# weiguangzhao/PBNet

Hardware: AMD Instinct MI355X
Metric: scenes/sec fwd+cluster (ScanNet ~150k pts/scene) (higher is better)
Workload: dtype bf16

## Files before the change

### include/pbnet_hip.h

```cpp
#ifndef PBNET_HIP_H
#define PBNET_HIP_H

#include <stddef.h>
#include <stdint.h>

#ifdef __cplusplus
extern "C" {
#endif

typedef void* pbn_stream_t;

enum {
    PBN_OK = 0,
    PBN_ERR_ARG = -1,
    PBN_ERR_WORKSPACE = -2,
    PBN_ERR_HIP = -3,
    PBN_ERR_RANGE = -4,
    PBN_ERR_UNSUPPORTED = -5
};

enum { PBN_F32 = 0, PBN_BF16 = 1, PBN_F16 = 2 };

#define PBN_MAX_SCENES 8

const char* pbn_version(void);
int pbn_last_hip_error(void);

size_t pbn_cluster_workspace_bytes(int n_points, int n_segments, int general_sem);

int pbn_binary_cluster(const float* off_xyz, const float* org_xyz, const int32_t* sem, const int32_t* seg_len,
                       int n_points, int n_segments, float radius, int min_pts, float para_f, int nv_flag,
                       int general_sem , int32_t* cluster_id, int32_t* cluster_num, int32_t* den, float* centers,
                       int32_t* clt_sem, int32_t* n_clusters, int32_t* member_start, int32_t* member_idx,
                       void* workspace, size_t workspace_bytes, pbn_stream_t stream);

int pbn_get_iou(const int32_t* proposals_idx, const int32_t* proposals_offset, const int64_t* instance_labels,
                const int32_t* instance_pointnum, float* proposals_iou, int n_instance, int n_proposal,
                pbn_stream_t stream);

int pbn_cal_iou_and_masklabel(const int32_t* proposals_idx, const int32_t* proposals_offset,
                              const int64_t* instance_labels, const int32_t* instance_pointnum,
                              float* proposals_iou, int n_instance, int n_proposal,
                              const float* mask_scores_sigmoid, float* mask_label, int mode, pbn_stream_t stream);


int pbn_hash_capacity(int n);
size_t pbn_coords_workspace_bytes(int n_max);

int pbn_coords_unique(const int32_t* coords, const int32_t* n_dev, int n_max, uint64_t* table_keys, int32_t* table_vals,
                      int capacity, int32_t* unique_index, int32_t* inverse, int32_t* unique_coords, int32_t* n_unique,
                      void* workspace, size_t workspace_bytes, pbn_stream_t stream);

int pbn_coords_stride(const int32_t* fine_coords, const int32_t* n_fine_dev, int n_fine_max, int stride_out,
                      uint64_t* table_keys, int32_t* table_vals, int capacity, int32_t* coarse_coords,
                      int32_t* parent_row, int32_t* child_k, int32_t* nbr_down, int32_t* n_coarse, void* workspace,
                      size_t workspace_bytes, pbn_stream_t stream);

int pbn_kernel_map(const int32_t* out_coords, const int32_t* n_out_dev, int n_out_max, const int32_t* offsets,
                   int n_offsets, const uint64_t* table_keys, const int32_t* table_vals, int capacity, int32_t* nbr,
                   pbn_stream_t stream);

int pbn_kernel_map_cube(const int32_t* out_coords, const int32_t* n_out_dev, int n_out_max, int kernel_size,
                        int tensor_stride, int x_fastest, const uint64_t* table_keys, const int32_t* table_vals,
                        int capacity, int32_t* nbr, pbn_stream_t stream);

int pbn_up_table(const int32_t* parent_row, const int32_t* child_k, const int32_t* n_fine_dev, int n_fine_max,
                 int32_t* nbr_up, pbn_stream_t stream);

int pbn_spconv_forward(const void* in_feat, int ld_in, int n_in, const int32_t* nbr, int n_offsets, const int32_t* row_perm,
                       const int32_t* n_out_dev, int n_out, const void* w_packed, int vecs_per_offset, int n_steps,
                       int cout_padded, const float* scale, const float* shift, const void* residual, int ld_res,
                       int relu, void* out_feat, int ld_out, int dtype, int rows_per_wave, void* workspace,
                       size_t workspace_bytes, pbn_stream_t stream);

int pbn_spconv_forward_dual(const void* in_feat, int ld_in, int n_in, const int32_t* nbr, int n_offsets,
                            const int32_t* n_out_dev, int n_out, const void* w_packed, int vecs_per_offset, int n_steps,
                            int cout_padded, const float* scale, const float* shift, const void* residual, int ld_res,
                            int relu, void* out_feat, int ld_out, int dtype, int rows_per_wave, void* workspace,
                            size_t workspace_bytes, const void* in2_feat, int ld_in2, int n_in2, int vecs_second,
                            pbn_stream_t stream);

int pbn_spconv_family(int n_out, int n_offsets, int vecs_per_offset, int n_steps, int cout_padded, int dtype, int has_map);

int pbn_gather_rows(const void* in, int ld_in_bytes, const int64_t* idx, int n, int row_bytes, void* out,
                    int ld_out_bytes, pbn_stream_t stream);

size_t pbn_segment_pool_workspace_bytes(int n_seg, int channels);
int pbn_segment_pool(const void* feats, int ld, int channels, int dtype, const int32_t* seg_start, int n_seg,
                     float* out_max, float* out_avg, void* workspace, size_t workspace_bytes, pbn_stream_t stream);

int pbn_local_scene_rows(const int32_t* ent_row_start, const int32_t* ent_member_start, const int32_t* ent_scene,
                         const float* ent_weight, int n_ent, int n_rows, const int32_t* member_idx,
                         const int64_t* ins_ind, const float* xyz, float inv_voxel, const void* point_feat, int ld_feat,
                         int channels, const void* sem_score, int ld_sem, const int64_t* sem_pred, int dtype,
                         int64_t* point_idx, int64_t* row_scene, int32_t* coords, void* feat_out, int ld_out,
                         pbn_stream_t stream);
int pbn_gather_pad_rows(const void* in, int ld_in_bytes, int row_bytes, const int64_t* idx, int n, void* out,
                        int ld_out_bytes, pbn_stream_t stream);

int pbn_pack_weight(const float* src, int n_offsets, int dim_a, int dim_b, int flip, int transpose, int dtype,
                    int vecs_per_offset, int n_steps, int cout_padded, void* out, pbn_stream_t stream);

typedef struct pbn_pack_job {
    const float* src;
    void* out;
    int32_t n_offsets, dim_a, dim_b, flip, transpose, cin, cout, cin_p, cout_p, n_steps;
    int32_t reserved[2];
} pbn_pack_job;
int pbn_pack_weights_batch(const pbn_pack_job* jobs, int n_jobs, int max_vectors, int dtype, pbn_stream_t stream);

int pbn_gather_rulebook_rows(const void* in, int ld_in_bytes, int row_bytes, const int32_t* nbr, int n_offsets, int k0,
                             int kc, int n, void* out, pbn_stream_t stream);

size_t pbn_bn_workspace_bytes(int channels);
int pbn_bn_train_forward(const void* x, int ld_x, int n, int channels, int dtype, const float* weight, const float* bias,
                         float eps, float momentum, float* running_mean, float* running_var, void* y, int ld_y,
                         float* save_mean, float* save_invstd, void* workspace, size_t workspace_bytes, pbn_stream_t stream);
int pbn_bn_train_backward(const void* x, int ld_x, const void* dy, int ld_dy, int n, int channels, int dtype,
                          const float* weight, const float* save_mean, const float* save_invstd, void* dx, int ld_dx,
                          float* dweight, float* dbias, void* workspace, size_t workspace_bytes, pbn_stream_t stream);

int pbn_bn_act_train_forward(const void* x, int ld_x, int n, int channels, int dtype, const float* weight, const float* bias,
                             float eps, float momentum, float* running_mean, float* running_var, const void* residual,
                             int ld_res, int relu, void* y, int ld_y, float* save_mean, float* save_invstd, void* workspace,
                             size_t workspace_bytes, pbn_stream_t stream);
int pbn_bn_act_train_backward(const void* x, int ld_x, const void* dy, int ld_dy, const void* y, int ld_y, int n, int channels,
                              int dtype, const float* weight, const float* save_mean, const float* save_invstd, void* dx,
                              int ld_dx, void* dres, int ld_dres, float* dweight, float* dbias, void* workspace,
                              size_t workspace_bytes, pbn_stream_t stream);

int pbn_rulebook_pair_blocks(int n);
int pbn_rulebook_pair_counts(const int32_t* nbr, int n, int n_offsets, int32_t* table, int32_t* totals, pbn_stream_t stream);
int pbn_rulebook_pair_fill(const int32_t* nbr, int n, int n_offsets, const int32_t* table, const int32_t* seg_start, int seg,
                           int n_segments, int32_t* in_idx, int32_t* out_idx, int64_t* seg_offset, pbn_stream_t stream);

int pbn_rulebook_pair_fill_dev(const int32_t* nbr, int n, int n_offsets, const int32_t* table, const int32_t* totals,
                               int segment, int32_t* seg_begin, int32_t* in_idx, int32_t* out_idx, int64_t* seg_offset,
                               pbn_stream_t stream);

typedef struct {
    const int32_t* nbr;
    int32_t n, n_offsets;
    int32_t* table;
    int32_t* totals;
    int32_t* seg_begin;
    int32_t* in_idx;
    int32_t* out_idx;
    int64_t* seg_offset;
} pbn_pair_job;
int pbn_rulebook_pairs_multi(const pbn_pair_job* jobs, int n_jobs, int segment, pbn_stream_t stream);

size_t pbn_spconv_wgrad_workspace_bytes(int n_offsets, int cin, int cout);
int pbn_spconv_wgrad(const void* x, int ld_x, const void* g, int ld_g, int dtype, const int32_t* in_idx,
                     const int32_t* out_idx, const int32_t* seg_begin, const int32_t* pair_counts, int segment,
                     int n_pairs_total, int n_offsets, int cin, int cout, float* dw, void* workspace, size_t workspace_bytes,
                     pbn_stream_t stream);
int pbn_spconv_wgrad_checked(const void* x, int ld_x, long long n_x_rows, const void* g, int ld_g, long long n_g_rows, int dtype,
                             const int32_t* in_idx, const int32_t* out_idx, const int32_t* seg_begin, const int32_t* pair_counts,
                             int lists_padded, int segment, int n_pairs_total, int n_offsets, int cin, int cout, float* dw,
                             void* workspace, size_t workspace_bytes, pbn_stream_t stream);
typedef struct {
    int32_t form, wa, wb, small_level, strips, co_groups, splits;
    int64_t grid;
} pbn_wgrad_plan;
int pbn_spconv_wgrad_plan(int dtype, int ld_x, int ld_g, int aligned16, int identity, int n_offsets, int n_pairs_total, int cin,
                          int cout, int has_workspace, size_t workspace_bytes, pbn_wgrad_plan* out);

enum {
    PBN_CNT_POINTS = 0, PBN_CNT_CLUSTERS = 1, PBN_CNT_ENTRIES = 2, PBN_CNT_ROWS = 3, PBN_CNT_SCENES = 4,
    PBN_CNT_PROPOSAL_ROWS = 5, PBN_CNT_PROPOSALS = 6, PBN_CNT_OVERFLOW = 7, PBN_CNT_WORDS = 16
};
enum {
    PBN_OVF_POINTS = 1, PBN_OVF_CLUSTERS = 2, PBN_OVF_ENTRIES = 4, PBN_OVF_ROWS = 8, PBN_OVF_SEGMENT = 16,
    PBN_OVF_BATCH = 32, PBN_OVF_LEVEL = 64,
    PBN_OVF_CDIST = 128
};
int pbn_class_gate(const int32_t* table, const float* thr05, int n_classes, int nb, int m_cap, int n_points,
                   int32_t* class_base, int32_t* seg_len, int32_t* counts, pbn_stream_t stream);
size_t pbn_local_plan_workspace_bytes(int c_cap);
int pbn_local_plan(const int32_t* cluster_num, int n_segments, int nb, const int32_t* member_start, const float* centers,
                   const int32_t* n_clusters, const float* thr02, const int32_t* kmax, int c_cap, int e_cap, int r_cap,
                   int32_t* ent_row_start, int32_t* ent_member_start, int32_t* ent_scene, float* ent_weight,
                   int32_t* counts, void* workspace, size_t workspace_bytes, pbn_stream_t stream);
int pbn_proposal_offsets(const int32_t* per_scene, int s_cap, int64_t* proposals_offset, int64_t* alive_ids,
                         int32_t* dense_of, int32_t* counts, pbn_stream_t stream);
int pbn_batch_starts(const int32_t* coords, const int32_t* n_dev, int n_cap, int n_segments, int32_t* seg_start,
                     pbn_stream_t stream);
int pbn_local_scene_rows_dev(const int32_t* ent_row_start, const int32_t* ent_member_start, const int32_t* ent_scene,
                             const float* ent_weight, int n_ent_cap, int n_rows_cap, const int32_t* n_ent_dev,
                             const int32_t* n_rows_dev, const int32_t* member_idx, const int64_t* ins_ind, const float* xyz,
                             float inv_voxel, const void* point_feat, int ld_feat, int channels, const void* sem_score,
                             int ld_sem, const int64_t* sem_pred, int dtype, int64_t* point_idx, int64_t* row_scene,
                             int32_t* coords, void* feat_out, int ld_out, pbn_stream_t stream);
int pbn_gather_pad_rows_dev(const void* in, int ld_in_bytes, int row_bytes, const int64_t* idx, const int64_t* idx2,
                            int n_cap, const int32_t* n_dev, void* out, int ld_out_bytes, pbn_stream_t stream);
int pbn_mlp_rows_dev(const void* in, int ld_in, int in_rows, int channels, const int64_t* idx_a, const int64_t* idx_b, int n_cap,
                     const int32_t* n_dev, const float* w1, const float* scale, const float* shift, const float* slope,
                     int hidden, const float* w2, const float* b2, int n_out, int sigmoid, void* out, int ld_out, int dtype,
                     pbn_stream_t stream);
int pbn_mask_count_dev(const void* mask_score, int ld, float thd, const int64_t* row_scene, int n_cap, const int32_t* n_dev,
                       int n_scenes_cap, int dtype, int32_t* per_scene, int32_t* block_cnt, pbn_stream_t stream);
int pbn_proposal_rows_dev(const void* mask_score, int ld, float thd, const int64_t* row_scene, const int64_t* point_idx,
                          int n_cap, const int32_t* n_dev, const int32_t* dense_of, const int32_t* block_cnt,
                          const float* xyz, float scale, float inv_voxel, const void* point_feat, int ld_feat, int channels,
                          int dtype, int64_t* proposals_idx, void* proposals_ms, int32_t* coords, void* feat_out,
                          pbn_stream_t stream);

int pbn_mlp_rows(const void* in, int ld_in, int channels, const int64_t* idx_a, const int64_t* idx_b, int n,
                 const float* w1, const float* scale, const float* shift, const float* slope, int hidden, const float* w2,
                 const float* b2, int n_out, int sigmoid, void* out, int ld_out, int dtype, pbn_stream_t stream);

int pbn_select_blocks(int n);
int pbn_sem_argmax_table(const void* score, int ld, int n_cls, const int32_t* batch, int nb, int n, int dtype,
                         int64_t* sem_pred, void* sem_prob, int32_t* table, int32_t* block_hist, pbn_stream_t stream);
int pbn_select_points(const int64_t* sem_pred, int n, int n_cls, const int32_t* class_base, const int32_t* block_hist,
                      const float* xyz, const void* offset, int ld_off, int dtype, int64_t* ins_ind, float* ins_orig,
                      float* ins_off, int32_t* ins_sem, pbn_stream_t stream);

int pbn_mask_count(const void* mask_score, int ld, float thd, const int64_t* row_scene, int n, int n_scenes, int dtype,
                   int32_t* per_scene, int32_t* block_cnt, pbn_stream_t stream);
int pbn_proposal_rows(const void* mask_score, int ld, float thd, const int64_t* row_scene, const int64_t* point_idx, int n,
                      const int32_t* dense_of, const int32_t* block_cnt, const float* xyz, float scale, float inv_voxel,
                      const void* point_feat, int ld_feat, int channels, int dtype, int64_t* proposals_idx,
                      void* proposals_ms, int32_t* coords, void* feat_out, pbn_stream_t stream);

int pbn_post_words(int n_fold);
int pbn_proposal_bitmask(const int64_t* proposals_idx, int n_entries, int n_fold, int n_prop, uint32_t* masks,
                         int32_t* counts, pbn_stream_t stream);
int pbn_mask_iou(const uint32_t* masks, const int32_t* rows, int n_rows, int n_fold, const int32_t* counts, float* iou,
                 pbn_stream_t stream);
int pbn_superpoint_refine(const uint32_t* masks, const int32_t* pick, int n_pick, int n_fold, const int64_t* superpoint,
                          int n_sp, int64_t* seg, int32_t* hist, int64_t* sp_label, int64_t* seg_refined,
                          uint32_t* masks_out, int32_t* counts_out, pbn_stream_t stream);
int pbn_bitmask_to_dense(const uint32_t* masks, const int32_t* rows, int n_rows, int n_fold, int32_t* dense,
                         pbn_stream_t stream);

int pbn_post_max_proposals(void);
int pbn_post_select(const float* clt_score, const int32_t* counts, int n_prop, float score_t, int npoint_t, int32_t* rows,
                    int32_t* n_rows, int32_t* status, pbn_stream_t stream);
int pbn_mask_iou_dev(const uint32_t* masks, const int32_t* rows, const int32_t* n_rows, int n_prop, int n_fold,
                     const int32_t* counts, float* iou, pbn_stream_t stream);
int pbn_post_nms(const float* clt_score, const int32_t* rows, const int32_t* n_rows, int n_prop, const float* iou, float nms_t,
                 int32_t* pick, int32_t* pick_rows, int32_t* n_pick, pbn_stream_t stream);
int pbn_superpoint_refine_dev(const uint32_t* masks, const int32_t* pick_rows, const int32_t* n_pick, int n_prop, int n_fold,
                              const int64_t* superpoint, int n_sp_cap, int64_t* seg, int32_t* hist, int64_t* sp_label,
                              int64_t* seg_refined, uint32_t* masks_out, int32_t* counts_out, int32_t* status,
                              pbn_stream_t stream);
int pbn_post_compact(const int32_t* counts2, const int32_t* pick_rows, const int32_t* n_pick, int n_prop, int n_fold,
                     const float* clt_score, const int64_t* proposals_idx, int n_entries, const void* proposals_offset,
                     int offset_i64, const void* pred_sem, int sem_i64, int64_t n_sem, const int64_t* label_table, int n_labels,
                     const uint32_t* masks2, int32_t* keep, float* scores_out, int64_t* semantic_id_out, int32_t* clusters,
                     int32_t* n_keep, int32_t* status, pbn_stream_t stream);

typedef struct pbn_scene_table {
    int32_t n_scenes;
    int32_t point_start[PBN_MAX_SCENES + 1];
    int32_t sp_start[PBN_MAX_SCENES + 1];
} pbn_scene_table;
typedef struct pbn_post_batch_layout {
    int64_t masks, counts, prop_scene, score, rows, pick_rows, n_rows, n_pick, iou, votes, sp_label, seg, seg_refined, counts2,
        renumber, total_bytes;
} pbn_post_batch_layout;
size_t pbn_post_batch_workspace_bytes(int n_prop, int n_points_total, int n_scenes, int n_sp_total, pbn_post_batch_layout* layout);
int pbn_post_batch(const int64_t* proposals_idx, int n_entries, const void* proposals_offset, int offset_i64, int n_prop,
                   const void* clt_score, int score_dtype, const void* pred_sem, int sem_i64, int n_points_total,
                   pbn_scene_table scenes, const int64_t* superpoint, float score_t, int npoint_t, float nms_t,
                   const int64_t* label_table, int n_labels, int32_t* point_instance, float* scores, int64_t* semantic_id,
                   int32_t* npoints, int32_t* scalars, void* workspace, size_t workspace_bytes, pbn_stream_t stream);

typedef struct pbn_tta_table {
    int32_t n_scenes;
    int32_t copies;
    int32_t point_start[PBN_MAX_SCENES + 1];
    int32_t sp_start[PBN_MAX_SCENES + 1];
} pbn_tta_table;
int pbn_post_batch_tta(const int64_t* proposals_idx, int n_entries, const void* proposals_offset, int offset_i64, int n_prop,
                       const void* clt_score, int score_dtype, const void* pred_sem, int sem_i64, int n_points_merged,
                       pbn_tta_table units, const int64_t* superpoint, float score_t, int npoint_t, float nms_t,
                       const int64_t* label_table, int n_labels, int32_t* point_instance, float* scores, int64_t* semantic_id,
                       int32_t* npoints, int32_t* scalars, void* workspace, size_t workspace_bytes, pbn_stream_t stream);

size_t pbn_scene_summary_workspace_bytes(int n_prop, int n_cls);
int pbn_scene_summary_lds_instances(int n_cls);
int pbn_scene_summary(const void* sem_score, int ld, int n_cls, int score_dtype, int n_points_merged, pbn_tta_table units,
                      const int32_t* point_instance, const int32_t* post_scalars, int n_prop, const float* xyz,
                      const int64_t* label_table, int n_labels, int32_t* sem_fold, int64_t* class_vote, int32_t* class_points,
                      float* box, float* centroid, int32_t* status, void* workspace, size_t workspace_bytes, pbn_stream_t stream);

int pbn_instance_overlap(const int32_t* masks, int n_pred, int n_pts, const int32_t* gt_index, int n_gt, int32_t* inter,
                         pbn_stream_t stream);

#define PBN_AP_RECORD_MAGIC 0x41504c47
#define PBN_AP_RECORD_HEADER 8
#define PBN_AP_STATUS_ID_RANGE 4
#define PBN_AP_STATUS_ID_COUNT 8
#define PBN_AP_STATUS_LABEL_RANGE 16
#define PBN_AP_STATUS_INSTANCE_CAP 32
#define PBN_AP_STATUS_SEMANTIC_RANGE 64
int pbn_gt_encode_dev(const void* sem, int sem_i64, const void* ins, int ins_i64, int n_pts, const int32_t* label_table,
                      int n_labels, int32_t* first, int n_inst_cap, int32_t* ids, int32_t* status, pbn_stream_t stream);
int pbn_gt_index_dev(const void* ids, int ids_i64, int n_pts, int32_t* table, int id_cap, int32_t* uid, int32_t* gt_vert,
                     int u_cap, int32_t* n_gt, int32_t* gt_index, int32_t* status, pbn_stream_t stream);
int pbn_instance_overlap_dev(const int32_t* clusters, const int32_t* n_keep, int p_cap, int n_pts, const int32_t* gt_index,
                             const int32_t* n_gt, int u_cap, int32_t* inter, pbn_stream_t stream);
int pbn_ap_record_append(int32_t* state, int32_t* log, int64_t log_words, int scene_tag, const int32_t* n_keep, int p_cap,
                         const int32_t* n_gt, int u_cap, int n_pts, const int32_t* post_status, int32_t* assoc_status,
                         const int32_t* uid, const int32_t* gt_vert, const int64_t* semantic_id, const float* conf,
                         const int32_t* inter, pbn_stream_t stream);

typedef struct pbn_ap_scene_tags {
    int32_t tag[PBN_MAX_SCENES];
} pbn_ap_scene_tags;
size_t pbn_ap_assoc_batch_workspace_bytes(int n_points_total, int n_scenes, int u_cap, int id_cap, int n_inst_cap);
int pbn_ap_assoc_batch_lds_counters(void);
int pbn_ap_assoc_batch(pbn_tta_table units, const int32_t* point_instance, const int32_t* post_scalars, const float* scores,
                       const int64_t* semantic_id, int n_prop, const void* ids, int ids_i64, const void* sem, int sem_i64,
                       const void* ins, int ins_i64, const int32_t* label_table, int n_labels, int u_cap, int id_cap,
                       int n_inst_cap, pbn_ap_scene_tags tags, int32_t* state, int32_t* log, int64_t log_words, void* workspace,
                       size_t workspace_bytes, pbn_stream_t stream);

#define PBN_AP_MAX_CLASSES 32
#define PBN_AP_MAX_OVERLAPS 16
#define PBN_AP_TABLE_SCALARS 16
typedef struct pbn_ap_class_ids {
    int32_t n;
    int32_t id[PBN_AP_MAX_CLASSES];
} pbn_ap_class_ids;
typedef struct pbn_ap_overlaps {
    int32_t n;
    int32_t _pad;
    double th[PBN_AP_MAX_OVERLAPS];
} pbn_ap_overlaps;
size_t pbn_ap_table_workspace_bytes(int rec_cap, int64_t entry_cap);
int pbn_ap_table_lds_entries(void);
int pbn_ap_table_reset(void* workspace, size_t workspace_bytes, int rec_cap, int64_t entry_cap, pbn_stream_t stream);
int pbn_ap_table_add_log(void* workspace, size_t workspace_bytes, int rec_cap, int64_t entry_cap, const int32_t* log_state,
                         const int32_t* log, int64_t log_words, int tag_base, pbn_ap_class_ids classes, pbn_ap_overlaps overlaps,
                         int min_region, pbn_stream_t stream);
int pbn_ap_table_finish(void* workspace, size_t workspace_bytes, int rec_cap, int64_t entry_cap, int n_classes, int n_overlaps,
                        float* ap, int32_t* cells, int32_t* flags, int32_t* directory, int32_t* scalars, pbn_stream_t stream);

typedef struct {
    int64_t counts, unique_index, inverse;
    int64_t keys[5], vals[5], coords[5], k3[5];
    int64_t parent_row[4], child_k[4], nbr_down[4], up[4];
    int64_t k5, workspace, workspace_bytes;
    int32_t capacity[5];
    int32_t _pad;
} pbn_coords_layout;

size_t pbn_coords_arena_bytes(int n, int want_k5, pbn_coords_layout* layout);
int pbn_coords_build(const int32_t* coords, const int32_t* n_dev, int n, int want_k5, int x_fastest, void* arena,
                     size_t arena_bytes, const pbn_coords_layout* layout, pbn_stream_t stream);

typedef struct {
    pbn_coords_layout pyramid;
    int64_t n_unique, unique_index, inverse, perm, inv_perm, ucoords;
    int64_t tmp_keys, tmp_vals, uidx32, inv32, sort_keys, sort_vals, sort_temp, sort_temp_bytes;
} pbn_prepare_layout;

size_t pbn_coords_prepare_bytes(int n, int want_k5, pbn_prepare_layout* layout);
int pbn_coords_prepare_dev(const int32_t* coords, const int32_t* n_dev, int n_cap, int want_k5, int x_fastest, void* arena,
                           size_t arena_bytes, const pbn_prepare_layout* layout, pbn_stream_t stream);
int pbn_coords_prepare(const int32_t* coords, int n, int want_k5, int x_fastest, void* arena, size_t arena_bytes,
                       const pbn_prepare_layout* layout, pbn_stream_t stream);
int pbn_coords_prepare_hash(const int32_t* coords, const int32_t* n_dev, int n_cap, int want_k5, int x_fastest, void* arena,
                            size_t arena_bytes, const pbn_prepare_layout* layout, pbn_stream_t stream);

int pbn_morton_keys(const int32_t* coords, const int32_t* n_dev, int n_max, int64_t* keys, pbn_stream_t stream);

typedef struct {
    int32_t map_kind, level_in, level_out;
    int32_t in_buf, in_col, res_buf, res_col, out_buf, out_col;
    int32_t vpo, n_steps, cout_p, relu;
    int32_t in2_buf;
    int32_t in2_col, vpo2;
    const void* w;
    const float* scale;
    const float* shift;
} pbn_unet_op;

typedef struct {
    int32_t level, width;
} pbn_unet_buf;

size_t pbn_unet_arena_bytes(const pbn_unet_buf* bufs, int n_bufs, const int32_t* n_rows, int dtype, int64_t* buf_offsets);
int pbn_unet_forward_dev(const pbn_unet_op* ops, int n_ops, const pbn_unet_buf* bufs, int n_bufs, const int32_t* n_rows_cap,
                         const int32_t* n_rows_dev, const int32_t* rows_expected, const void* input, int ld_input,
                         const int32_t* const* k3, const int32_t* k5, const int32_t* const* down, const int32_t* const* up,
                         void* arena, size_t arena_bytes, int dtype, void* splitk_ws, size_t splitk_bytes, pbn_stream_t stream);
int pbn_unet_forward(const pbn_unet_op* ops, int n_ops, const pbn_unet_buf* bufs, int n_bufs, const int32_t* n_rows,
                     const void* input, int ld_input, const int32_t* const* k3, const int32_t* k5,
                     const int32_t* const* down, const int32_t* const* up, void* arena, size_t arena_bytes, int dtype,
                     void* splitk_ws, size_t splitk_bytes, pbn_stream_t stream);

int pbn_unet_forward_timed(const pbn_unet_op* ops, int n_ops, const pbn_unet_buf* bufs, int n_bufs, const int32_t* n_rows,
                           const void* input, int ld_input, const int32_t* const* k3, const int32_t* k5,
                           const int32_t* const* down, const int32_t* const* up, void* arena, size_t arena_bytes,
                           int dtype, void* splitk_ws, size_t splitk_bytes, pbn_stream_t stream, float* op_ms);

typedef struct {
    int32_t map_kind, level_in, level_out;
    int32_t in_buf, in_col, pre_buf, res_buf, res_col, out_buf, out_col;
    int32_t relu, cin, cout;
    int32_t vpo, n_steps, cout_p;
    int32_t vpo_d, n_steps_d, cout_p_d;
    int32_t want_dx, dx_accumulate, _pad;
    const void* w;
    const void* w_d;
    const float* gamma;
    const float* beta;
    float* running_mean;
    float* running_var;
    float eps, momentum;
    int64_t stat_off, dw_off, dgamma_off, dbeta_off;
} pbn_train_op;

typedef struct {
    const int32_t* in_idx;
    const int32_t* out_idx;
    const int32_t* seg_begin;
    const int32_t* counts;
    int32_t segment, n_pairs_estimate;
} pbn_pair_lists;

int pbn_unet_train_forward(const pbn_train_op* ops, int n_ops, const pbn_unet_buf* bufs, int n_bufs, const int32_t* n_rows,
                           const void* input, int ld_input, const int32_t* const* k3, const int32_t* k5,
                           const int32_t* const* down, const int32_t* const* up, void* act_arena, size_t arena_bytes,
                           float* stats, int dtype, void* splitk_ws, size_t splitk_bytes, void* bn_ws, size_t bn_ws_bytes,
                           pbn_stream_t stream);
int pbn_unet_train_backward(const pbn_train_op* ops, int n_ops, const pbn_unet_buf* bufs, int n_bufs, const int32_t* n_rows,
                            const void* input, int ld_input, const int32_t* const* k3, const int32_t* k5,
                            const int32_t* const* down, const int32_t* const* up, const pbn_pair_lists* pairs,
                            const void* act_arena, void* grad_arena, size_t arena_bytes, const float* stats,
                            float* param_grads, void* dinput, int ld_dinput, int dtype, void* splitk_ws, size_t splitk_bytes,
                            void* bn_ws, size_t bn_ws_bytes, void* wgrad_ws, size_t wgrad_ws_bytes, pbn_stream_t stream);

int pbn_aug_chunks(int n_rows);
size_t pbn_aug_workspace_bytes(int n_segments);
int pbn_aug_affine(const float* xyz, const int32_t* unit_off, int n_units, int max_unit_rows, const int32_t* pre_min,
                   const double* mats, const double* scale, const int32_t* has_scale, double* out, double* ext,
                   void* workspace, pbn_stream_t stream);
int pbn_aug_elastic(double* xyz, const int32_t* unit_off, int n_units, int max_unit_rows, const int32_t* desc, int n_el,
                    int total_cells, float* noise, float* tmp, int gran, double mag, double* ext, void* workspace,
                    pbn_stream_t stream);
int pbn_aug_sub_min(double* xyz, const int32_t* unit_off, int n_units, int max_unit_rows, const int32_t* flags,
                    const double* ext, pbn_stream_t stream);
int pbn_aug_crop(const double* xyz, const int32_t* scene_off, int n_scenes, int max_scene_rows, const int32_t* mode,
                 const double* triples, const int32_t* n_triples, const double* levels, int max_crop_p, int min_crop_p,
                 int32_t* counts, int32_t* state, double* ext_pre, double* ext_post, void* workspace, pbn_stream_t stream);
int pbn_aug_compact(const double* xyz, const float* rgb, const float* nl, const int64_t* sem, const int32_t* ins,
                    const double* shift, const int32_t* ins_shift, const int32_t* unit_off, int n_units,
                    const int32_t* scene_off, int n_scenes, const int32_t* mode, const double* triples, const double* levels,
                    const int32_t* state, const double* ext_pre, const double* ext_post, const int32_t* label_off,
                    int32_t* label_map, int32_t* present, int32_t* scene_i32, int32_t* scan, double* xyz_out,
                    float* feat_out, int64_t* sem_out, int32_t* label_out, int32_t* scene_info, int n_rows, int n_labels,
                    pbn_stream_t stream);
int pbn_aug_instances(const double* xyz, const int32_t* label, const int32_t* out_start, int n_scenes,
                      const int32_t* inst_start, const int32_t* inst_off, int n_inst, int n_rows, int32_t* pointnum,
                      float* stats, float* inst_info, int64_t* ins, pbn_stream_t stream);
int pbn_aug_quantize(const double* xyz, const int32_t* out_start, int n_scenes, int n_rows, double voxel_size,
                     int32_t* coords, float* xyz_f32, pbn_stream_t stream);

enum { PBN_MESH_NORMALS = 0, PBN_MESH_SEGMENT = 1, PBN_MESH_SEGMENT_POINT = 2 };
size_t pbn_mesh_workspace_bytes(int mode, int n_vertices, int n_elems);
int pbn_mesh_vertex_normals(const float* xyz, int n_vertices, const void* faces, int faces_i64, int n_faces, float* nl,
                            int32_t* status, void* workspace, size_t workspace_bytes, pbn_stream_t stream);
int pbn_mesh_segment(const float* xyz, int n_vertices, const void* faces, int faces_i64, int n_faces, float k_thresh,
                     int seg_min_verts, int64_t* sup, float* nl, void* workspace, size_t workspace_bytes, float* times_ms,
                     pbn_stream_t stream);
int pbn_mesh_segment_point(const float* xyz, const float* normals, int n_points, const void* edges, int edges_i64, int n_edges,
                           float k_thresh, int seg_min_verts, int64_t* sup, void* workspace, size_t workspace_bytes,
                           pbn_stream_t stream);

int pbn_sem_confusion(const void* pred, int pred_i64, const void* target, int target_i64, int64_t n, int n_class,
                      int ignore_index, int64_t* acc3k, int64_t* conf_kk, pbn_stream_t stream);
int pbn_mask_accuracy(const void* pred_mask, int dtype, const void* gt_mask, int gt_i64, int64_t n, float threshold,
                      int64_t* row8, pbn_stream_t stream);

size_t pbn_losses_workspace_bytes(int64_t n_points, int64_t n_rows, int64_t n_prop);
int pbn_losses_forward(const void* sem_score, int sem_dtype, int sem_ld, const int64_t* sem_label, const void* offset_pred,
                       int offset_dtype, const float* inst_info, const float* xyz, const int64_t* ins_label, int64_t n_points,
                       int n_class, const void* pred_mask, int mask_dtype, int64_t* gt_mask, uint8_t* mask_weight,
                       int64_t n_rows, const float* iou, int n_inst, const void* clt_scores, int clt_dtype, int64_t n_prop,
                       double fg_thresh, double bg_thresh, float* gt_scores, float* terms, int64_t* counts, double* state,
                       void* workspace, size_t workspace_bytes, pbn_stream_t stream);
int pbn_losses_backward(const void* sem_score, int sem_dtype, int sem_ld, const int64_t* sem_label, const void* offset_pred,
                        int offset_dtype, const float* inst_info, const float* xyz, const int64_t* ins_label, int64_t n_points,
                        int n_class, const void* pred_mask, int mask_dtype, const int64_t* gt_mask, const uint8_t* mask_weight,
                        int64_t n_rows, const void* clt_scores, int clt_dtype, const float* gt_scores, int64_t n_prop,
                        const double* state, const float* grad_loss, void* g_sem, void* g_offset, void* g_mask, void* g_clt,
                        pbn_stream_t stream);

#define PBN_OPTIM_CHUNK 4096
typedef struct pbn_optim_chunk_rec {
    void* param;
    const void* grad;
    void* state0;
    void* state1;
    int32_t n;
    int32_t vec;
} pbn_optim_chunk_rec;
int pbn_optim_chunk(void);
int pbn_optim_adam(const void* table, int n_chunks, float lr, float beta1, float one_minus_beta1, float beta2,
                   float one_minus_beta2, float eps, float weight_decay, float step_size, float bc2_sqrt, int decoupled,
                   pbn_stream_t stream);
int pbn_optim_sgd(const void* table, int n_chunks, float lr, float momentum, float weight_decay, int first,
                  pbn_stream_t stream);
int pbn_loss_meter_update(const float* terms, const double* weights, double* acc, int k, pbn_stream_t stream);

#ifdef __cplusplus
}
#endif
#endif
```

### pbnet_amd/MinkowskiEngine/core.py

```python
import ctypes

import torch

from .. import _native as N
from . import conventions as CV


def _i32(n, dev, fill=None):
    if fill is None:
        return torch.empty(n, dtype=torch.int32, device=dev)
    return torch.full((n,), fill, dtype=torch.int32, device=dev)


_OFFSETS = {}
_RANGE_ERROR = ("coordinates cannot be indexed: batch must be in [0,65534], x/y/z in [-32768,32767], and the bounding box of one "
                "call must fit 44 Z-order key bits (3 x bits of the largest extent + bits of the batch range); also raised when a "
                "coordinate table was found full or corrupted")


def _device_offsets(kernel_size, stride, device):
    key = (int(kernel_size), int(stride), device)
    t = _OFFSETS.get(key)
    if t is None:
        t = CV.kernel_offsets(kernel_size, stride).to(device)
        _OFFSETS[key] = t
    return t


class _Level(object):
    __slots__ = ("stride", "coords", "n", "n_dev", "keys", "vals", "capacity", "parent_row", "child_k", "nbr_down")


class _Pyramid(object):
    _STRIDES = (1, 2, 4, 8, 16)

    def __init__(self, coords, n_dev, n_cap, _prepared=None):
        lib = N.lib()
        if _prepared is not None:
            self.arena, self.layout = _prepared
            self.device = self.arena.device
        else:
            self.device = coords.device
            self.layout = N.CoordsLayout()
            nbytes = lib.pbn_coords_arena_bytes(n_cap, 1, ctypes.byref(self.layout))
            self.arena = torch.empty(nbytes, dtype=torch.uint8, device=coords.device)
            rc = lib.pbn_coords_build(N.ptr(coords), None if n_dev is None else N.ptr(n_dev), n_cap, 1,
                                      int(CV.X_FASTEST), N.ptr(self.arena), nbytes, ctypes.byref(self.layout),
                                      N.current_stream())
            N.check(rc, "pbn_coords_build")
        self.counts_dev = self.view(self.layout.counts, 5, torch.int32)
        self.n = None

    def view(self, offset, count, dtype, shape=None):
        nbytes = count * torch.empty(0, dtype=dtype).element_size()
        t = self.arena[offset:offset + nbytes].view(dtype)
        return t if shape is None else t.view(shape)

    def ptr(self, offset):
        return self.arena.data_ptr() + offset

    def set_counts(self, counts):
        if min(counts) < 0:
            raise ValueError(_RANGE_ERROR)
        self.n = [int(c) for c in counts]

    def finalize(self):
        if self.n is None:
            self.set_counts(self.counts_dev.tolist())

    def level_index(self, stride):
        return self._STRIDES.index(stride)

    def coordinates(self, stride):
        self.finalize()
        l = self.level_index(stride)
        return self.view(self.layout.coords[l], self.n[l] * 4, torch.int32, (self.n[l], 4))

    def _map_view(self, key, make):
        views = self.__dict__.setdefault("_views", {})
        if key not in views:
            views[key] = make()
        return views[key]

    def kernel_map(self, stride, kernel_size):
        self.finalize()
        l = self.level_index(stride)
        if kernel_size == 3:
            return self._map_view(("k3", l), lambda: self.view(self.layout.k3[l], self.n[l] * 27, torch.int32, (self.n[l], 27)))
        assert kernel_size == 5 and stride == 1
        return self._map_view(("k5",), lambda: self.view(self.layout.k5, self.n[0] * 125, torch.int32, (self.n[0], 125)))

    def down_map(self, stride_in):
        self.finalize()
        l = self.level_index(stride_in)
        return self._map_view(("down", l), lambda: self.view(self.layout.nbr_down[l], self.n[l + 1] * 8, torch.int32,
                                                             (self.n[l + 1], 8)))

    def up_map(self, stride_in):
        self.finalize()
        l = self.level_index(stride_in) - 1
        return self._map_view(("up", l), lambda: self.view(self.layout.up[l], self.n[l] * 8, torch.int32, (self.n[l], 8)))

    def native_tables(self):
        self.finalize()
        return table_arrays(self.ptr(0), self.layout)


def table_arrays(base, L):
    vp = ctypes.c_void_p
    return ((vp * 5)(*[base + L.k3[l] for l in range(5)]), vp(base + L.k5),
            (vp * 4)(*[base + L.nbr_down[l] for l in range(4)]), (vp * 4)(*[base + L.up[l] for l in range(4)]))


class SortedView(object):
    __slots__ = ("pyramid", "perm", "inv_perm")


class CoordinateManager(object):

    MAX_STRIDE = 16
    _STRIDES = (1, 2, 4, 8, 16)

    def __init__(self, coordinates, build_maps=True, prepare=None):
        N.require_cuda(coordinates)
        coords = coordinates.to(torch.int32).contiguous()
        assert coords.dim() == 2 and coords.shape[1] == 4, "coordinates must be [N,4] (batch, x, y, z)"
        dev = coords.device
        lib = N.lib()
        n = int(coords.shape[0])
        self.device = dev
        self.n_input = n
        self._maps = {}
        self._plain = None
        self._sorted = None
        self._final = False
        self.unique_index = self.inverse_mapping = self.is_identity = None
        self._n1 = None
        if prepare is None:
            prepare = ("plain" if torch.is_grad_enabled() else "sorted") if build_maps else "unique"
        self._native = None
        if prepare == "sorted" and n > 0:
            P = N.PrepareLayout()
            nbytes = lib.pbn_coords_prepare_bytes(n, 1, ctypes.byref(P))
            arena = torch.empty(nbytes, dtype=torch.uint8, device=dev)
            rc = lib.pbn_coords_prepare(N.ptr(coords), n, 1, int(CV.X_FASTEST), N.ptr(arena), nbytes, ctypes.byref(P),
                                        N.current_stream())
            N.check(rc, "pbn_coords_prepare")
            self._native = (arena, P)
            self._prepare_input = coords
            sv = SortedView()
            sv.pyramid = _Pyramid(None, None, n, _prepared=(arena, P.pyramid))
            sv.perm = sv.inv_perm = None
            self._sorted = sv
            self._count = sv.pyramid.view(P.n_unique, 1, torch.int32)
            self._ucoords = sv.pyramid.view(P.ucoords, max(n, 1) * 4, torch.int32, (max(n, 1), 4))
            return
        cap = lib.pbn_hash_capacity(n)
        keys = torch.empty(cap, dtype=torch.int64, device=dev)
        vals = _i32(cap, dev)
        self._count = _i32(1, dev)
        self._uidx, self._inv = _i32(max(n, 1), dev), _i32(max(n, 1), dev)
        self._ucoords = torch.empty(max(n, 1), 4, dtype=torch.int32, device=dev)
        wsb = lib.pbn_coords_workspace_bytes(n)
        ws = torch.empty(wsb, dtype=torch.uint8, device=dev)
        rc = lib.pbn_coords_unique(N.ptr(coords), None, n, N.ptr(keys), N.ptr(vals), cap, N.ptr(self._uidx),
                                   N.ptr(self._inv), N.ptr(self._ucoords), N.ptr(self._count), N.ptr(ws), wsb,
                                   N.current_stream())
        N.check(rc, "pbn_coords_unique")
        if prepare == "plain":
            self._build_plain()
        elif prepare == "sorted":
            self._build_sorted()

    def _build_plain(self):
        if self._plain is None:
            self._plain = _Pyramid(self._ucoords, self._count, self.n_input)
        return self._plain

    def _build_sorted(self):
        if self._sorted is None:
            n = self.n_input
            keys = torch.empty(max(n, 1), dtype=torch.int64, device=self.device)
            rc = N.lib().pbn_morton_keys(N.ptr(self._ucoords), N.ptr(self._count), n, N.ptr(keys), N.current_stream())
            N.check(rc, "pbn_morton_keys")
            perm = torch.sort(keys[:n], stable=True)[1]
            sv = SortedView()
            sv.perm = perm
            sv.pyramid = _Pyramid(self._ucoords[perm].contiguous(), self._count, n)
            sv.inv_perm = None
            self._sorted = sv
        return self._sorted

    def _finalize(self):
        if self._final:
            return
        if self._native is not None:
            arena, P = self._native
            pyr = self._sorted.pyramid
            counts = pyr.counts_dev.tolist()
            if min(counts) < 0 and self.__dict__.get("_prepare_input") is not None:
                coords = self._prepare_input
                rc = N.lib().pbn_coords_prepare_hash(N.ptr(coords), None, self.n_input, 1, int(CV.X_FASTEST), N.ptr(arena),
                                                     arena.numel(), ctypes.byref(P), N.current_stream())
                N.check(rc, "pbn_coords_prepare_hash")
                counts = pyr.counts_dev.tolist()
            self._prepare_input = None
            pyr.set_counts(counts)
            n1 = self._n1 = int(counts[0])
            n = self.n_input
            self.unique_index = pyr.view(P.unique_index, n, torch.int64)[:n1]
            self.inverse_mapping = pyr.view(P.inverse, n, torch.int64)
            self.is_identity = (n1 == n)
            self._sorted.perm = pyr.view(P.perm, n, torch.int64)[:n1]
            self._sorted.inv_perm = pyr.view(P.inv_perm, n, torch.int64)[:n1]
            self._final = True
            return
        pending = [p for p in (self._plain, self._sorted.pyramid if self._sorted else None) if p is not None and p.n is None]
        counts = torch.cat([self._count] + [p.counts_dev for p in pending]).tolist()
        if min(counts) < 0:
            raise ValueError(_RANGE_ERROR)
        self._n1 = int(counts[0])
        for i, p in enumerate(pending):
            p.set_counts(counts[1 + 5 * i:6 + 5 * i])
        n1 = self._n1
        self.unique_index = self._uidx[:n1].long()
        self.inverse_mapping = self._inv[:self.n_input].long()
        self.is_identity = (n1 == self.n_input)
        if self._sorted is not None:
            sv = self._sorted
            sv.perm = sv.perm[:n1]
            sv.inv_perm = torch.empty_like(sv.perm)
            sv.inv_perm[sv.perm] = torch.arange(n1, device=self.device)
        self._final = True

    def plain(self):
        self._finalize()
        if self._plain is None:
            self._build_plain()
        self._plain.finalize()
        return self._plain

    def sorted(self):
        self._finalize()
        if self._sorted is None:
            self._build_sorted()
            sv = self._sorted
            sv.pyramid.finalize()
            sv.perm = sv.perm[:self._n1]
            sv.inv_perm = torch.empty_like(sv.perm)
            sv.inv_perm[sv.perm] = torch.arange(self._n1, device=self.device)
        return self._sorted

    def num_rows(self, stride):
        self._finalize()
        if stride == 1:
            return self._n1
        pyr = self._plain if self._plain is not None else (self._sorted.pyramid if self._sorted else self.plain())
        pyr.finalize()
        return pyr.n[self._STRIDES.index(stride)]

    def row_counts(self):
        return [self.num_rows(s) for s in self._STRIDES]

    def coordinates(self, stride):
        self._finalize()
        if stride == 1:
            return self._ucoords[:self._n1]
        return self.plain().coordinates(stride)

    def kernel_map(self, stride, kernel_size):
        pyr = self.plain()
        if kernel_size == 3 or (kernel_size == 5 and stride == 1):
            return pyr.kernel_map(stride, kernel_size)
        key = ("k", stride, kernel_size)
        if key not in self._maps:
            l = pyr.level_index(stride)
            n = pyr.n[l]
            L = pyr.layout
            nbr = torch.empty(max(n, 1), kernel_size ** 3, dtype=torch.int32, device=self.device)
            rc = N.lib().pbn_kernel_map_cube(N.c_vp(pyr.ptr(L.coords[l])), None, n, kernel_size, stride,
                                             int(CV.X_FASTEST), N.c_vp(pyr.ptr(L.keys[l])), N.c_vp(pyr.ptr(L.vals[l])),
                                             L.capacity[l], N.ptr(nbr), N.current_stream())
            N.check(rc, "pbn_kernel_map_cube")
            self._maps[key] = nbr[:n]
        return self._maps[key]

    def down_map(self, stride_in):
        return self.plain().down_map(stride_in)

    def up_map(self, stride_in):
        return self.plain().up_map(stride_in)


class SparseTensor(object):

    def __init__(self, features, coordinates=None, tensor_stride=1, coordinate_manager=None, device=None,
                 quantization_mode=None, _slab=None):
        if device is not None:
            dev = torch.device(device) if not isinstance(device, int) else torch.device("cuda", device)
            features = features.to(dev)
            if coordinates is not None:
                coordinates = coordinates.to(dev)
        if coordinate_manager is None:
            assert coordinates is not None
            N.require_cuda(features, coordinates)
            cm = CoordinateManager(coordinates)
            cm.num_rows(1)
            if not cm.is_identity:
                features = features[cm.unique_index]
            coordinate_manager = cm
            tensor_stride = 1
        self._F = features
        self._stored = None
        self.coordinate_manager = coordinate_manager
        self.tensor_stride = int(tensor_stride)

    @classmethod
    def _from_stored_rows(cls, stored, row_index, coordinate_manager, tensor_stride=1):
        self = cls.__new__(cls)
        self._F = None
        self._stored = (stored, row_index)
        self.coordinate_manager = coordinate_manager
        self.tensor_stride = int(tensor_stride)
        return self

    def rows(self):
        if self._F is None:
            return self._stored
        return self._F, None

    @property
    def F(self):
        if self._F is None:
            stored, row_index = self._stored
            self._F = stored[row_index]
        return self._F

    @property
    def C(self):
        return self.coordinate_manager.coordinates(self.tensor_stride)

    @property
    def inverse_mapping(self):
        return self.coordinate_manager.inverse_mapping

    @property
    def device(self):
        return self.rows()[0].device

    @property
    def dtype(self):
        return self.rows()[0].dtype

    @property
    def shape(self):
# ... 18 lines not shown
```

### pbnet_amd/_native.py

```python
import ctypes
import os

import torch

_HERE = os.path.dirname(os.path.abspath(__file__))
LIB_PATH = os.environ.get("PBNET_HIP_LIB") or os.path.join(_HERE, "libpbnet_hip.so")

_lib = None

c_f32p = ctypes.c_void_p
c_i32p = ctypes.c_void_p
c_vp = ctypes.c_void_p
c_int = ctypes.c_int
c_float = ctypes.c_float
c_size = ctypes.c_size_t

c_i64 = ctypes.c_int64
c_i32 = ctypes.c_int32

DT = {torch.float32: 0, torch.bfloat16: 1, torch.float16: 2}


class CoordsLayout(ctypes.Structure):
    _fields_ = [("counts", c_i64), ("unique_index", c_i64), ("inverse", c_i64),
                ("keys", c_i64 * 5), ("vals", c_i64 * 5), ("coords", c_i64 * 5), ("k3", c_i64 * 5),
                ("parent_row", c_i64 * 4), ("child_k", c_i64 * 4), ("nbr_down", c_i64 * 4), ("up", c_i64 * 4),
                ("k5", c_i64), ("workspace", c_i64), ("workspace_bytes", c_i64),
                ("capacity", c_i32 * 5), ("_pad", c_i32)]


class PrepareLayout(ctypes.Structure):
    _fields_ = [("pyramid", CoordsLayout), ("n_unique", c_i64), ("unique_index", c_i64), ("inverse", c_i64),
                ("perm", c_i64), ("inv_perm", c_i64), ("ucoords", c_i64), ("tmp_keys", c_i64), ("tmp_vals", c_i64),
                ("uidx32", c_i64), ("inv32", c_i64), ("sort_keys", c_i64), ("sort_vals", c_i64), ("sort_temp", c_i64),
                ("sort_temp_bytes", c_i64)]


class UnetOp(ctypes.Structure):
    _fields_ = [("map_kind", c_i32), ("level_in", c_i32), ("level_out", c_i32),
                ("in_buf", c_i32), ("in_col", c_i32), ("res_buf", c_i32), ("res_col", c_i32), ("out_buf", c_i32),
                ("out_col", c_i32), ("vpo", c_i32), ("n_steps", c_i32), ("cout_p", c_i32), ("relu", c_i32),
                ("in2_buf", c_i32), ("in2_col", c_i32), ("vpo2", c_i32),
                ("w", ctypes.c_void_p), ("scale", ctypes.c_void_p), ("shift", ctypes.c_void_p)]


class WgradPlan(ctypes.Structure):
    _fields_ = [("form", c_i32), ("wa", c_i32), ("wb", c_i32), ("small_level", c_i32), ("strips", c_i32),
                ("co_groups", c_i32), ("splits", c_i32), ("grid", c_i64)]


class UnetBuf(ctypes.Structure):
    _fields_ = [("level", c_i32), ("width", c_i32)]


class TrainOp(ctypes.Structure):
    _fields_ = [("map_kind", c_i32), ("level_in", c_i32), ("level_out", c_i32),
                ("in_buf", c_i32), ("in_col", c_i32), ("pre_buf", c_i32), ("res_buf", c_i32), ("res_col", c_i32),
                ("out_buf", c_i32), ("out_col", c_i32), ("relu", c_i32), ("cin", c_i32), ("cout", c_i32),
                ("vpo", c_i32), ("n_steps", c_i32), ("cout_p", c_i32), ("vpo_d", c_i32), ("n_steps_d", c_i32),
                ("cout_p_d", c_i32), ("want_dx", c_i32), ("dx_accumulate", c_i32), ("_pad", c_i32),
                ("w", ctypes.c_void_p), ("w_d", ctypes.c_void_p), ("gamma", ctypes.c_void_p), ("beta", ctypes.c_void_p),
                ("running_mean", ctypes.c_void_p), ("running_var", ctypes.c_void_p), ("eps", ctypes.c_float),
                ("momentum", ctypes.c_float), ("stat_off", ctypes.c_int64), ("dw_off", ctypes.c_int64),
                ("dgamma_off", ctypes.c_int64), ("dbeta_off", ctypes.c_int64)]


class PairJob(ctypes.Structure):
    _fields_ = [("nbr", ctypes.c_void_p), ("n", c_i32), ("n_offsets", c_i32), ("table", ctypes.c_void_p),
                ("totals", ctypes.c_void_p), ("seg_begin", ctypes.c_void_p), ("in_idx", ctypes.c_void_p),
                ("out_idx", ctypes.c_void_p), ("seg_offset", ctypes.c_void_p)]


class PairLists(ctypes.Structure):
    _fields_ = [("in_idx", ctypes.c_void_p), ("out_idx", ctypes.c_void_p), ("seg_begin", ctypes.c_void_p),
                ("counts", ctypes.c_void_p), ("segment", c_i32), ("n_pairs_estimate", c_i32)]


MAX_SCENES = 8


class SceneTable(ctypes.Structure):
    _fields_ = [("n_scenes", c_i32), ("point_start", c_i32 * (MAX_SCENES + 1)), ("sp_start", c_i32 * (MAX_SCENES + 1))]


class TtaTable(ctypes.Structure):
    _fields_ = [("n_scenes", c_i32), ("copies", c_i32), ("point_start", c_i32 * (MAX_SCENES + 1)),
                ("sp_start", c_i32 * (MAX_SCENES + 1))]


class SceneTags(ctypes.Structure):
    _fields_ = [("tag", c_i32 * MAX_SCENES)]


AP_MAX_CLASSES, AP_MAX_OVERLAPS, AP_TABLE_SCALARS = 32, 16, 16


class ApClassIds(ctypes.Structure):
    _fields_ = [("n", c_i32), ("id", c_i32 * AP_MAX_CLASSES)]


class ApOverlaps(ctypes.Structure):
    _fields_ = [("n", c_i32), ("_pad", c_i32), ("th", ctypes.c_double * AP_MAX_OVERLAPS)]


class PostBatchLayout(ctypes.Structure):
    _fields_ = [(k, c_i64) for k in ("masks", "counts", "prop_scene", "score", "rows", "pick_rows", "n_rows", "n_pick", "iou",
                                     "votes", "sp_label", "seg", "seg_refined", "counts2", "renumber", "total_bytes")]


SIGNATURES = {
    "pbn_version": (ctypes.c_char_p, []),
    "pbn_last_hip_error": (c_int, []),
    "pbn_cluster_workspace_bytes": (c_size, [c_int, c_int, c_int]),
    "pbn_binary_cluster": (c_int, [c_f32p, c_f32p, c_i32p, c_i32p, c_int, c_int, c_float, c_int, c_float, c_int, c_int,
                                   c_i32p, c_i32p, c_i32p, c_f32p, c_i32p, c_i32p, c_i32p, c_i32p, c_vp, c_size, c_vp]),
    "pbn_get_iou": (c_int, [c_i32p, c_i32p, c_vp, c_i32p, c_f32p, c_int, c_int, c_vp]),
    "pbn_cal_iou_and_masklabel": (c_int, [c_i32p, c_i32p, c_vp, c_i32p, c_f32p, c_int, c_int, c_f32p, c_f32p, c_int,
                                          c_vp]),
    "pbn_hash_capacity": (c_int, [c_int]),
    "pbn_coords_workspace_bytes": (c_size, [c_int]),
    "pbn_coords_unique": (c_int, [c_i32p, c_i32p, c_int, c_vp, c_i32p, c_int, c_i32p, c_i32p, c_i32p, c_i32p, c_vp,
                                  c_size, c_vp]),
    "pbn_coords_stride": (c_int, [c_i32p, c_i32p, c_int, c_int, c_vp, c_i32p, c_int, c_i32p, c_i32p, c_i32p, c_i32p,
                                  c_i32p, c_vp, c_size, c_vp]),
    "pbn_kernel_map": (c_int, [c_i32p, c_i32p, c_int, c_i32p, c_int, c_vp, c_i32p, c_int, c_i32p, c_vp]),
    "pbn_up_table": (c_int, [c_i32p, c_i32p, c_i32p, c_int, c_i32p, c_vp]),
    "pbn_spconv_forward": (c_int, [c_vp, c_int, c_int, c_i32p, c_int, c_i32p, c_i32p, c_int, c_vp, c_int, c_int, c_int,
                                   c_f32p, c_f32p, c_vp, c_int, c_int, c_vp, c_int, c_int, c_int, c_vp, c_size, c_vp]),
    "pbn_spconv_forward_dual": (c_int, [c_vp, c_int, c_int, c_i32p, c_int, c_i32p, c_int, c_vp, c_int, c_int, c_int, c_f32p, c_f32p,
                                        c_vp, c_int, c_int, c_vp, c_int, c_int, c_int, c_vp, c_size, c_vp, c_int, c_int, c_int, c_vp]),
    "pbn_spconv_family": (c_int, [c_int, c_int, c_int, c_int, c_int, c_int, c_int]),
    "pbn_spconv_wgrad_workspace_bytes": (c_size, [c_int, c_int, c_int]),
    "pbn_spconv_wgrad": (c_int, [c_vp, c_int, c_vp, c_int, c_int, c_vp, c_vp, c_i32p, c_i32p, c_int, c_int, c_int, c_int, c_int,
                                 c_f32p, c_vp, c_size, c_vp]),
    "pbn_spconv_wgrad_checked": (c_int, [c_vp, c_int, ctypes.c_longlong, c_vp, c_int, ctypes.c_longlong, c_int, c_vp, c_vp, c_i32p,
                                         c_i32p, c_int, c_int, c_int, c_int, c_int, c_int, c_f32p, c_vp, c_size, c_vp]),
    "pbn_spconv_wgrad_plan": (c_int, [c_int, c_int, c_int, c_int, c_int, c_int, c_int, c_int, c_int, c_int, c_size,
                                      ctypes.POINTER(WgradPlan)]),
    "pbn_gather_rows": (c_int, [c_vp, c_int, c_vp, c_int, c_int, c_vp, c_int, c_vp]),
    "pbn_segment_pool_workspace_bytes": (c_size, [c_int, c_int]),
    "pbn_segment_pool": (c_int, [c_vp, c_int, c_int, c_int, c_i32p, c_int, c_f32p, c_f32p, c_vp, c_size, c_vp]),
    "pbn_local_scene_rows": (c_int, [c_i32p, c_i32p, c_i32p, c_f32p, c_int, c_int, c_i32p, c_vp, c_f32p, c_float, c_vp,
                                     c_int, c_int, c_vp, c_int, c_vp, c_int, c_vp, c_vp, c_i32p, c_vp, c_int, c_vp]),
    "pbn_gather_pad_rows": (c_int, [c_vp, c_int, c_int, c_vp, c_int, c_vp, c_int, c_vp]),
    "pbn_mlp_rows": (c_int, [c_vp, c_int, c_int, c_vp, c_vp, c_int, c_f32p, c_f32p, c_f32p, c_f32p, c_int, c_f32p, c_f32p,
                             c_int, c_int, c_vp, c_int, c_int, c_vp]),
    "pbn_select_blocks": (c_int, [c_int]),
    "pbn_sem_argmax_table": (c_int, [c_vp, c_int, c_int, c_i32p, c_int, c_int, c_int, c_vp, c_vp, c_i32p, c_i32p, c_vp]),
    "pbn_select_points": (c_int, [c_vp, c_int, c_int, c_i32p, c_i32p, c_f32p, c_vp, c_int, c_int, c_vp, c_f32p, c_f32p,
                                  c_i32p, c_vp]),
    "pbn_mask_count": (c_int, [c_vp, c_int, c_float, c_vp, c_int, c_int, c_int, c_i32p, c_i32p, c_vp]),
    "pbn_proposal_rows": (c_int, [c_vp, c_int, c_float, c_vp, c_vp, c_int, c_i32p, c_i32p, c_f32p, c_float, c_float, c_vp,
                                  c_int, c_int, c_int, c_vp, c_vp, c_i32p, c_vp, c_vp]),
    "pbn_post_words": (c_int, [c_int]),
    "pbn_proposal_bitmask": (c_int, [c_vp, c_int, c_int, c_int, c_vp, c_i32p, c_vp]),
    "pbn_mask_iou": (c_int, [c_vp, c_i32p, c_int, c_int, c_i32p, c_f32p, c_vp]),
    "pbn_superpoint_refine": (c_int, [c_vp, c_i32p, c_int, c_int, c_vp, c_int, c_vp, c_i32p, c_vp, c_vp, c_vp, c_i32p,
                                      c_vp]),
    "pbn_bitmask_to_dense": (c_int, [c_vp, c_i32p, c_int, c_int, c_i32p, c_vp]),
    "pbn_post_max_proposals": (c_int, []),
    "pbn_post_select": (c_int, [c_f32p, c_i32p, c_int, c_float, c_int, c_i32p, c_i32p, c_i32p, c_vp]),
    "pbn_mask_iou_dev": (c_int, [c_vp, c_i32p, c_i32p, c_int, c_int, c_i32p, c_f32p, c_vp]),
    "pbn_post_nms": (c_int, [c_f32p, c_i32p, c_i32p, c_int, c_f32p, c_float, c_i32p, c_i32p, c_i32p, c_vp]),
    "pbn_superpoint_refine_dev": (c_int, [c_vp, c_i32p, c_i32p, c_int, c_int, c_vp, c_int, c_vp, c_i32p, c_vp, c_vp, c_vp, c_i32p,
                                          c_i32p, c_vp]),
    "pbn_post_compact": (c_int, [c_i32p, c_i32p, c_i32p, c_int, c_int, c_f32p, c_vp, c_int, c_vp, c_int, c_vp, c_int, c_i64, c_vp,
                                 c_int, c_vp, c_i32p, c_f32p, c_vp, c_i32p, c_i32p, c_i32p, c_vp]),
    "pbn_post_batch_workspace_bytes": (c_size, [c_int, c_int, c_int, c_int, ctypes.POINTER(PostBatchLayout)]),
    "pbn_post_batch": (c_int, [c_vp, c_int, c_vp, c_int, c_int, c_vp, c_int, c_vp, c_int, c_int, SceneTable, c_vp, c_float, c_int,
                               c_float, c_vp, c_int, c_i32p, c_f32p, c_vp, c_i32p, c_i32p, c_vp, c_size, c_vp]),
    "pbn_post_batch_tta": (c_int, [c_vp, c_int, c_vp, c_int, c_int, c_vp, c_int, c_vp, c_int, c_int, TtaTable, c_vp, c_float, c_int,
                                   c_float, c_vp, c_int, c_i32p, c_f32p, c_vp, c_i32p, c_i32p, c_vp, c_size, c_vp]),
    "pbn_scene_summary_workspace_bytes": (c_size, [c_int, c_int]),
    "pbn_scene_summary_lds_instances": (c_int, [c_int]),
    "pbn_scene_summary": (c_int, [c_vp, c_int, c_int, c_int, c_int, TtaTable, c_i32p, c_i32p, c_int, c_f32p, c_vp, c_int, c_i32p,
                                  c_vp, c_i32p, c_f32p, c_f32p, c_i32p, c_vp, c_size, c_vp]),
    "pbn_instance_overlap": (c_int, [c_i32p, c_int, c_int, c_i32p, c_int, c_i32p, c_vp]),
    "pbn_gt_encode_dev": (c_int, [c_vp, c_int, c_vp, c_int, c_int, c_i32p, c_int, c_i32p, c_int, c_i32p, c_i32p, c_vp]),
    "pbn_gt_index_dev": (c_int, [c_vp, c_int, c_int, c_i32p, c_int, c_i32p, c_i32p, c_int, c_i32p, c_i32p, c_i32p, c_vp]),
    "pbn_instance_overlap_dev": (c_int, [c_i32p, c_i32p, c_int, c_int, c_i32p, c_i32p, c_int, c_i32p, c_vp]),
    "pbn_ap_record_append": (c_int, [c_i32p, c_i32p, c_i64, c_int, c_i32p, c_int, c_i32p, c_int, c_int, c_i32p, c_i32p, c_i32p,
                                     c_i32p, c_vp, c_f32p, c_i32p, c_vp]),
    "pbn_ap_assoc_batch_workspace_bytes": (c_size, [c_int, c_int, c_int, c_int, c_int]),
    "pbn_ap_assoc_batch_lds_counters": (c_int, []),
    "pbn_ap_assoc_batch": (c_int, [TtaTable, c_i32p, c_i32p, c_f32p, c_vp, c_int, c_vp, c_int, c_vp, c_int, c_vp, c_int, c_i32p,
                                   c_int, c_int, c_int, c_int, SceneTags, c_i32p, c_i32p, c_i64, c_vp, c_size, c_vp]),
    "pbn_ap_table_workspace_bytes": (c_size, [c_int, c_i64]),
    "pbn_ap_table_lds_entries": (c_int, []),
    "pbn_ap_table_reset": (c_int, [c_vp, c_size, c_int, c_i64, c_vp]),
    "pbn_ap_table_add_log": (c_int, [c_vp, c_size, c_int, c_i64, c_i32p, c_i32p, c_i64, c_int, ApClassIds, ApOverlaps, c_int,
                                     c_vp]),
    "pbn_ap_table_finish": (c_int, [c_vp, c_size, c_int, c_i64, c_int, c_int, c_f32p, c_i32p, c_i32p, c_i32p, c_i32p, c_vp]),
    "pbn_rulebook_pair_blocks": (c_int, [c_int]),
    "pbn_bn_workspace_bytes": (c_size, [c_int]),
    "pbn_bn_train_forward": (c_int, [c_vp, c_int, c_int, c_int, c_int, c_f32p, c_f32p, ctypes.c_float, ctypes.c_float, c_f32p,
                                     c_f32p, c_vp, c_int, c_f32p, c_f32p, c_vp, c_size, c_vp]),
    "pbn_bn_train_backward": (c_int, [c_vp, c_int, c_vp, c_int, c_int, c_int, c_int, c_f32p, c_f32p, c_f32p, c_vp, c_int,
                                      c_f32p, c_f32p, c_vp, c_size, c_vp]),
    "pbn_bn_act_train_forward": (c_int, [c_vp, c_int, c_int, c_int, c_int, c_f32p, c_f32p, ctypes.c_float, ctypes.c_float,
                                         c_f32p, c_f32p, c_vp, c_int, c_int, c_vp, c_int, c_f32p, c_f32p, c_vp, c_size, c_vp]),
    "pbn_bn_act_train_backward": (c_int, [c_vp, c_int, c_vp, c_int, c_vp, c_int, c_int, c_int, c_int, c_f32p, c_f32p, c_f32p,
                                          c_vp, c_int, c_vp, c_int, c_f32p, c_f32p, c_vp, c_size, c_vp]),
    "pbn_rulebook_pair_counts": (c_int, [c_i32p, c_int, c_int, c_i32p, c_i32p, c_vp]),
    "pbn_rulebook_pair_fill_dev": (c_int, [c_i32p, c_int, c_int, c_i32p, c_i32p, c_int, c_i32p, c_vp, c_vp, c_vp, c_vp]),
    "pbn_rulebook_pair_fill": (c_int, [c_i32p, c_int, c_int, c_i32p, c_i32p, c_int, c_int, c_vp, c_vp, c_vp, c_vp]),
    "pbn_gather_rulebook_rows": (c_int, [c_vp, c_int, c_int, c_i32p, c_int, c_int, c_int, c_int, c_vp, c_vp]),
    "pbn_pack_weights_batch": (c_int, [c_vp, c_int, c_int, c_int, c_vp]),
    "pbn_pack_weight": (c_int, [c_f32p, c_int, c_int, c_int, c_int, c_int, c_int, c_int, c_int, c_int, c_vp, c_vp]),
    "pbn_kernel_map_cube": (c_int, [c_i32p, c_i32p, c_int, c_int, c_int, c_int, c_vp, c_i32p, c_int, c_i32p, c_vp]),
    "pbn_coords_arena_bytes": (c_size, [c_int, c_int, ctypes.POINTER(CoordsLayout)]),
    "pbn_coords_build": (c_int, [c_i32p, c_i32p, c_int, c_int, c_int, c_vp, c_size, ctypes.POINTER(CoordsLayout), c_vp]),
    "pbn_coords_prepare_bytes": (c_size, [c_int, c_int, ctypes.POINTER(PrepareLayout)]),
    "pbn_coords_prepare": (c_int, [c_i32p, c_int, c_int, c_int, c_vp, c_size, ctypes.POINTER(PrepareLayout), c_vp]),
    "pbn_coords_prepare_dev": (c_int, [c_i32p, c_i32p, c_int, c_int, c_int, c_vp, c_size, ctypes.POINTER(PrepareLayout), c_vp]),
    "pbn_coords_prepare_hash": (c_int, [c_i32p, c_i32p, c_int, c_int, c_int, c_vp, c_size, ctypes.POINTER(PrepareLayout), c_vp]),
    "pbn_unet_forward_dev": (c_int, [ctypes.POINTER(UnetOp), c_int, ctypes.POINTER(UnetBuf), c_int, ctypes.POINTER(c_i32),
                                     c_i32p, ctypes.POINTER(c_i32), c_vp, c_int, ctypes.POINTER(ctypes.c_void_p), c_vp,
                                     ctypes.POINTER(ctypes.c_void_p), ctypes.POINTER(ctypes.c_void_p), c_vp, c_size, c_int,
                                     c_vp, c_size, c_vp]),
    "pbn_class_gate": (c_int, [c_i32p, c_f32p, c_int, c_int, c_int, c_int, c_i32p, c_i32p, c_i32p, c_vp]),
    "pbn_local_plan_workspace_bytes": (c_size, [c_int]),
    "pbn_local_plan": (c_int, [c_i32p, c_int, c_int, c_i32p, c_f32p, c_i32p, c_f32p, c_i32p, c_int, c_int, c_int, c_i32p,
                               c_i32p, c_i32p, c_f32p, c_i32p, c_vp, c_size, c_vp]),
    "pbn_proposal_offsets": (c_int, [c_i32p, c_int, c_vp, c_vp, c_i32p, c_i32p, c_vp]),
    "pbn_batch_starts": (c_int, [c_i32p, c_i32p, c_int, c_int, c_i32p, c_vp]),
    "pbn_local_scene_rows_dev": (c_int, [c_i32p, c_i32p, c_i32p, c_f32p, c_int, c_int, c_i32p, c_i32p, c_i32p, c_vp, c_f32p,
                                         c_float, c_vp, c_int, c_int, c_vp, c_int, c_vp, c_int, c_vp, c_vp, c_i32p, c_vp,
                                         c_int, c_vp]),
    "pbn_gather_pad_rows_dev": (c_int, [c_vp, c_int, c_int, c_vp, c_vp, c_int, c_i32p, c_vp, c_int, c_vp]),
    "pbn_mlp_rows_dev": (c_int, [c_vp, c_int, c_int, c_int, c_vp, c_vp, c_int, c_i32p, c_f32p, c_f32p, c_f32p, c_f32p, c_int,
                                 c_f32p, c_f32p, c_int, c_int, c_vp, c_int, c_int, c_vp]),
    "pbn_mask_count_dev": (c_int, [c_vp, c_int, c_float, c_vp, c_int, c_i32p, c_int, c_int, c_i32p, c_i32p, c_vp]),
    "pbn_proposal_rows_dev": (c_int, [c_vp, c_int, c_float, c_vp, c_vp, c_int, c_i32p, c_i32p, c_i32p, c_f32p, c_float,
                                      c_float, c_vp, c_int, c_int, c_int, c_vp, c_vp, c_i32p, c_vp, c_vp]),
    "pbn_morton_keys": (c_int, [c_i32p, c_i32p, c_int, c_vp, c_vp]),
    "pbn_unet_arena_bytes": (c_size, [ctypes.POINTER(UnetBuf), c_int, ctypes.POINTER(c_i32), c_int,
                                      ctypes.POINTER(c_i64)]),
    "pbn_unet_forward": (c_int, [ctypes.POINTER(UnetOp), c_int, ctypes.POINTER(UnetBuf), c_int, ctypes.POINTER(c_i32),
                                 c_vp, c_int, ctypes.POINTER(ctypes.c_void_p), c_vp, ctypes.POINTER(ctypes.c_void_p),
                                 ctypes.POINTER(ctypes.c_void_p), c_vp, c_size, c_int, c_vp, c_size, c_vp]),
    "pbn_rulebook_pairs_multi": (c_int, [ctypes.POINTER(PairJob), c_int, c_int, c_vp]),
    "pbn_unet_train_forward": (c_int, [ctypes.POINTER(TrainOp), c_int, ctypes.POINTER(UnetBuf), c_int, ctypes.POINTER(c_i32),
                                       c_vp, c_int, ctypes.POINTER(ctypes.c_void_p), c_vp, ctypes.POINTER(ctypes.c_void_p),
                                       ctypes.POINTER(ctypes.c_void_p), c_vp, c_size, c_vp, c_int, c_vp, c_size, c_vp, c_size,
                                       c_vp]),
    "pbn_unet_train_backward": (c_int, [ctypes.POINTER(TrainOp), c_int, ctypes.POINTER(UnetBuf), c_int, ctypes.POINTER(c_i32),
                                        c_vp, c_int, ctypes.POINTER(ctypes.c_void_p), c_vp, ctypes.POINTER(ctypes.c_void_p),
                                        ctypes.POINTER(ctypes.c_void_p), ctypes.POINTER(PairLists), c_vp, c_vp, c_size, c_vp,
                                        c_vp, c_vp, c_int, c_int, c_vp, c_size, c_vp, c_size, c_vp, c_size, c_vp]),
    "pbn_unet_forward_timed": (c_int, [ctypes.POINTER(UnetOp), c_int, ctypes.POINTER(UnetBuf), c_int,
                                       ctypes.POINTER(c_i32), c_vp, c_int, ctypes.POINTER(ctypes.c_void_p), c_vp,
                                       ctypes.POINTER(ctypes.c_void_p), ctypes.POINTER(ctypes.c_void_p), c_vp, c_size,
                                       c_int, c_vp, c_size, c_vp, ctypes.POINTER(ctypes.c_float)]),
    "pbn_aug_chunks": (c_int, [c_int]),
    "pbn_aug_workspace_bytes": (c_size, [c_int]),
    "pbn_aug_affine": (c_int, [c_f32p, c_i32p, c_int, c_int, c_i32p, c_vp, c_vp, c_i32p, c_vp, c_vp, c_vp, c_vp]),
    "pbn_aug_elastic": (c_int, [c_vp, c_i32p, c_int, c_int, c_i32p, c_int, c_int, c_f32p, c_f32p, c_int, ctypes.c_double, c_vp,
                                c_vp, c_vp]),
    "pbn_aug_sub_min": (c_int, [c_vp, c_i32p, c_int, c_int, c_i32p, c_vp, c_vp]),
    "pbn_aug_crop": (c_int, [c_vp, c_i32p, c_int, c_int, c_i32p, c_vp, c_i32p, c_vp, c_int, c_int, c_i32p, c_i32p, c_vp, c_vp,
                             c_vp, c_vp]),
    "pbn_aug_compact": (c_int, [c_vp, c_f32p, c_f32p, c_vp, c_i32p, c_vp, c_i32p, c_i32p, c_int, c_i32p, c_int, c_i32p, c_vp,
                                c_vp, c_i32p, c_vp, c_vp, c_i32p, c_i32p, c_i32p, c_i32p, c_i32p, c_vp, c_f32p, c_vp, c_i32p,
                                c_i32p, c_int, c_int, c_vp]),
    "pbn_aug_instances": (c_int, [c_vp, c_i32p, c_i32p, c_int, c_i32p, c_i32p, c_int, c_int, c_i32p, c_f32p, c_f32p, c_vp,
                                  c_vp]),
    "pbn_aug_quantize": (c_int, [c_vp, c_i32p, c_int, c_int, ctypes.c_double, c_i32p, c_f32p, c_vp]),
    "pbn_mesh_workspace_bytes": (c_size, [c_int, c_int, c_int]),
    "pbn_mesh_vertex_normals": (c_int, [c_f32p, c_int, c_vp, c_int, c_int, c_f32p, c_i32p, c_vp, c_size, c_vp]),
    "pbn_mesh_segment": (c_int, [c_f32p, c_int, c_vp, c_int, c_int, c_float, c_int, c_vp, c_f32p, c_vp, c_size,
                                 ctypes.POINTER(ctypes.c_float), c_vp]),
    "pbn_mesh_segment_point": (c_int, [c_f32p, c_f32p, c_int, c_vp, c_int, c_int, c_float, c_int, c_vp, c_vp, c_size, c_vp]),
    "pbn_sem_confusion": (c_int, [c_vp, c_int, c_vp, c_int, c_i64, c_int, c_int, c_vp, c_vp, c_vp]),
    "pbn_mask_accuracy": (c_int, [c_vp, c_int, c_vp, c_int, c_i64, c_float, c_vp, c_vp]),
    "pbn_losses_workspace_bytes": (c_size, [c_i64, c_i64, c_i64]),
    "pbn_losses_forward": (c_int, [c_vp, c_int, c_int, c_vp, c_vp, c_int, c_f32p, c_f32p, c_vp, c_i64, c_int, c_vp, c_int, c_vp,
                                   c_vp, c_i64, c_f32p, c_int, c_vp, c_int, c_i64, ctypes.c_double, ctypes.c_double, c_f32p,
                                   c_f32p, c_vp, c_vp, c_vp, c_size, c_vp]),
    "pbn_losses_backward": (c_int, [c_vp, c_int, c_int, c_vp, c_vp, c_int, c_f32p, c_f32p, c_vp, c_i64, c_int, c_vp, c_int, c_vp,
                                    c_vp, c_i64, c_vp, c_int, c_f32p, c_i64, c_vp, c_f32p, c_vp, c_vp, c_vp, c_vp, c_vp]),
    "pbn_optim_chunk": (c_int, []),
    "pbn_optim_adam": (c_int, [c_vp, c_int, c_float, c_float, c_float, c_float, c_float, c_float, c_float, c_float, c_float,
                               c_int, c_vp]),
# ... 58 lines not shown
```

### pbnet_amd/csrc/executor.hip

```cpp
#include <cstdlib>
#include "pbn_common.h"
#include "spconv_common.h"
#include "unet_plan.h"

using namespace pbn;

static inline size_t a256(size_t x) { return align_up(x, 256); }

extern "C" size_t pbn_coords_arena_bytes(int n, int want_k5, pbn_coords_layout* L) {
    if (n < 0 || !L) return 0;
    const size_t N = (size_t)(n > 0 ? n : 1);
    const int cap = pbn_hash_capacity(n);
    size_t off = 0;
    auto take = [&](size_t bytes) { size_t o = off; off = a256(off + bytes); return (int64_t)o; };
    L->counts = take(16 * sizeof(int));
    for (int l = 0; l < 5; ++l) { L->capacity[l] = cap; L->keys[l] = take((size_t)cap * 8); }
    for (int l = 0; l < 4; ++l) L->nbr_down[l] = take(N * 8 * 4);
    for (int l = 0; l < 5; ++l) L->vals[l] = take((size_t)cap * 4);
    const int64_t fill_end = (int64_t)off;
    (void)fill_end;
    L->unique_index = take(N * 4);
    L->inverse = take(N * 4);
    for (int l = 0; l < 5; ++l) {
        L->coords[l] = take(N * 16);
// ... 5 lines not shown
        L->up[l] = take(N * 8 * 4);
    }
    L->k5 = want_k5 ? take(N * 125 * 4) : -1;
    L->workspace = take(pbn_coords_workspace_bytes(n));
    L->workspace_bytes = (int64_t)pbn_coords_workspace_bytes(n);
    return off;
}

extern "C" int pbn_coords_build(const int32_t* coords, const int32_t* n_dev, int n, int want_k5, int x_fastest, void* arena,
                                size_t arena_bytes, const pbn_coords_layout* L, pbn_stream_t stream) {
    if (n < 0 || !arena || !L) return PBN_ERR_ARG;
    pbn_coords_layout chk;
    if (pbn_coords_arena_bytes(n, want_k5, &chk) > arena_bytes) return PBN_ERR_WORKSPACE;
    char* A = (char*)arena;
    auto I = [&](int64_t o) { return (int32_t*)(A + o); };
    int32_t* counts = I(L->counts);
    void* ws = A + L->workspace;
    const size_t wsb = (size_t)L->workspace_bytes;
    hipStream_t st = (hipStream_t)stream;
    {
        const FillRange fr[3] = {{A + L->counts, 16 * sizeof(int), 0}, {A + L->keys[0], (size_t)(L->vals[0] - L->keys[0]), 0xff},
                                 {A + L->vals[0], (size_t)(L->unique_index - L->vals[0]), 0x7f}};
        const int frc = fill_ranges(fr, 3, st);
        if (frc != PBN_OK) return frc;
    }
    int rc = coords_unique_impl(coords, n_dev, n, (uint64_t*)(A + L->keys[0]), I(L->vals[0]), L->capacity[0],
                                I(L->unique_index), I(L->inverse), I(L->coords[0]), counts + 0, ws, wsb, counts + 8, false,
                                st);
    if (rc != PBN_OK) return rc;
    return coords_build_upper(n, want_k5, x_fastest, arena, L, st);
}

int pbn::coords_build_upper(int n, int want_k5, int x_fastest, void* arena, const pbn_coords_layout* L, hipStream_t st) {
    char* A = (char*)arena;
    auto I = [&](int64_t o) { return (int32_t*)(A + o); };
    int32_t* counts = I(L->counts);
    void* ws = A + L->workspace;
    const size_t wsb = (size_t)L->workspace_bytes;
    int rc = PBN_OK;
    for (int l = 0; l < 4; ++l) {
        rc = coords_stride_impl(I(L->coords[l]), counts + l, n, 2 << l, (uint64_t*)(A + L->keys[l + 1]), I(L->vals[l + 1]),
                                L->capacity[l + 1], I(L->coords[l + 1]), I(L->parent_row[l]), I(L->child_k[l]),
                                I(L->nbr_down[l]), I(L->up[l]), counts + l + 1, ws, wsb, counts + 8, false, st);
        if (rc != PBN_OK) return rc;
    }
    {
        MapJobs jb;
        jb.n_jobs = 0; jb.n_max = n; jb.x_fastest = x_fastest;
        long long total = 0;
        auto add = [&](int l, int ksize, int32_t* out) {
            const int j = jb.n_jobs++;
            jb.coords[j] = I(L->coords[l]); jb.n_dev[j] = counts + l; jb.keys[j] = (const unsigned long long*)(A + L->keys[l]);
            jb.vals[j] = I(L->vals[l]); jb.nbr[j] = out; jb.mask[j] = (unsigned)L->capacity[l] - 1; jb.ksize[j] = ksize;
            jb.stride[j] = 1 << l;
            total += (long long)n * ksize * ksize * ksize;
        };
        for (int l = 0; l < 5; ++l) add(l, 3, I(L->k3[l]));
        if (want_k5) add(0, 5, I(L->k5));
        rc = kernel_maps_multi(jb, total, st);
        if (rc != PBN_OK) return rc;
    }
    return PBN_OK;
}

extern "C" size_t pbn_coords_prepare_bytes(int n, int want_k5, pbn_prepare_layout* P) {
    if (n < 0 || !P) return 0;
    const size_t N = (size_t)(n > 0 ? n : 1);
    const size_t pyr = pbn_coords_arena_bytes(n, want_k5, &P->pyramid);
    if (!pyr) return 0;
    size_t off = a256(pyr);
    auto take = [&](size_t bytes) { size_t o = off; off = a256(off + bytes); return (int64_t)o; };
    const int cap = pbn_hash_capacity(n);
    P->n_unique = take(16 * sizeof(int));
    P->tmp_keys = take((size_t)cap * 8);
    P->tmp_vals = take((size_t)cap * 4);
    P->unique_index = take(N * 8);
    P->inverse = take(N * 8);
    P->perm = take(N * 8);
    P->inv_perm = take(N * 8);
    P->ucoords = take(N * 16);
    P->uidx32 = take(N * 4);
    P->inv32 = take(N * 4);
    P->sort_keys = take(2 * N * 8);
    P->sort_vals = take(2 * N * 4);
    {
        const size_t a = sort_pairs_temp_bytes(n), b = pyramid_scratch_bytes(n);
        P->sort_temp_bytes = (int64_t)(a > b ? a : b);
    }
    P->sort_temp = take((size_t)P->sort_temp_bytes);
    return off;
}

static int coords_prepare_impl(const int32_t* coords, const int32_t* n_dev, int n, int want_k5, int x_fastest, void* arena,
                               size_t arena_bytes, const pbn_prepare_layout* P, pbn_stream_t stream, bool force_hash = false) {
    if (n < 0 || !arena || !P) return PBN_ERR_ARG;
    pbn_prepare_layout chk;
    if (pbn_coords_prepare_bytes(n, want_k5, &chk) > arena_bytes) return PBN_ERR_WORKSPACE;
    hipStream_t st = (hipStream_t)stream;
    static const int hash_env = getenv("PBN_PREPARE_HASH") ? atoi(getenv("PBN_PREPARE_HASH")) : 0;
    if (!hash_env && !force_hash) return coords_prepare_sorted(coords, n_dev, n, want_k5, x_fastest, arena, P, st);
    char* A = (char*)arena;
    const pbn_coords_layout* L = &P->pyramid;
    auto I = [&](int64_t o) { return (int32_t*)(A + o); };
    const size_t N = (size_t)(n > 0 ? n : 1);
    {
        const FillRange fr[6] = {{A + P->n_unique, 16 * sizeof(int), 0},
                                 {A + P->tmp_keys, (size_t)(P->tmp_vals - P->tmp_keys), 0xff},
                                 {A + P->tmp_vals, (size_t)(P->unique_index - P->tmp_vals), 0x7f},
                                 {A + L->counts, 16 * sizeof(int), 0},
                                 {A + L->keys[0], (size_t)(L->vals[0] - L->keys[0]), 0xff},
                                 {A + L->vals[0], (size_t)(L->unique_index - L->vals[0]), 0x7f}};
        const int frc = fill_ranges(fr, 6, st);
        if (frc != PBN_OK) return frc;
    }
    if (n == 0) return PBN_OK;
    if (!coords) return PBN_ERR_ARG;
    int32_t* n_unique = I(P->n_unique);
    int rc = coords_unique_impl(coords, n_dev, n, (uint64_t*)(A + P->tmp_keys), I(P->tmp_vals), pbn_hash_capacity(n),
                                I(P->uidx32), I(P->inv32), I(P->ucoords), n_unique, A + L->workspace,
                                (size_t)L->workspace_bytes, n_unique + 8, false, st);
    if (rc != PBN_OK) return rc;
    uint64_t* keys = (uint64_t*)(A + P->sort_keys);
    int32_t* vals = I(P->sort_vals);
    rc = coords_morton_iota(I(P->ucoords), n_unique, n, keys, vals, st);
    if (rc != PBN_OK) return rc;
    rc = sort_pairs_u64_i32(keys, keys + N, vals, vals + N, n, A + P->sort_temp, (size_t)P->sort_temp_bytes, st);
    if (rc != PBN_OK) return rc;
    rc = coords_apply_perm(I(P->ucoords), vals + N, I(P->uidx32), I(P->inv32), n, I(L->coords[0]),
                           (int64_t*)(A + P->perm), (int64_t*)(A + P->inv_perm), (int64_t*)(A + P->unique_index),
                           (int64_t*)(A + P->inverse), st);
    if (rc != PBN_OK) return rc;
    rc = coords_insert_identity(I(L->coords[0]), n_unique, n, (uint64_t*)(A + L->keys[0]), I(L->vals[0]), L->capacity[0],
                                I(L->coords[0]), I(L->counts), I(L->counts) + 8, st);
    if (rc != PBN_OK) return rc;
    return coords_build_upper(n, want_k5, x_fastest, arena, L, st);
}

extern "C" int pbn_coords_prepare(const int32_t* coords, int n, int want_k5, int x_fastest, void* arena, size_t arena_bytes,
                                  const pbn_prepare_layout* P, pbn_stream_t stream) {
    return coords_prepare_impl(coords, nullptr, n, want_k5, x_fastest, arena, arena_bytes, P, stream);
}

extern "C" int pbn_coords_prepare_dev(const int32_t* coords, const int32_t* n_dev, int n_cap, int want_k5, int x_fastest,
                                      void* arena, size_t arena_bytes, const pbn_prepare_layout* P, pbn_stream_t stream) {
    if (!n_dev) return PBN_ERR_ARG;
    return coords_prepare_impl(coords, n_dev, n_cap, want_k5, x_fastest, arena, arena_bytes, P, stream);
}

extern "C" int pbn_coords_prepare_hash(const int32_t* coords, const int32_t* n_dev, int n_cap, int want_k5, int x_fastest,
                                       void* arena, size_t arena_bytes, const pbn_prepare_layout* P, pbn_stream_t stream) {
    return coords_prepare_impl(coords, n_dev, n_cap, want_k5, x_fastest, arena, arena_bytes, P, stream, true);
}

extern "C" size_t pbn_unet_arena_bytes(const pbn_unet_buf* bufs, int n_bufs, const int32_t* n_rows, int dtype,
                                       int64_t* buf_offsets) {
    if (!bufs || !n_rows || n_bufs < 1) return 0;
    size_t off = 0;
    for (int b = 0; b < n_bufs; ++b) {
        if (b == 0) { if (buf_offsets) buf_offsets[0] = -1; continue; }
        const size_t bytes = (size_t)n_rows[bufs[b].level] * bufs[b].width * esize(dtype);
        if (buf_offsets) buf_offsets[b] = (int64_t)off;
        off = a256(off + (bytes ? bytes : 16));
    }
    return off;
}

static NextWeights next_weights(const pbn_unet_op& q, int n_bufs, const MapTables& T, const int32_t* n_rows, const PlanArena& B,
                                int dtype, int mode) {
    if (!op_index_ok(q.in_buf, q.res_buf, q.out_buf, q.level_in, q.level_out, n_bufs) || !q.w) return {};
    const OpTables m = op_tables(q.map_kind, q.level_in, q.level_out, T);
    const ConvArgs nx = shape_args(n_rows[q.level_out], m.K, q.vpo, q.n_steps, q.cout_p, m.fwd != nullptr,
                                   (unsigned)((unsigned long long)q.n_steps * (q.cout_p / 16) * 1024ull),
                                   (unsigned)((unsigned long long)n_rows[q.level_in] * B.ld(q.in_buf) * esize(dtype)));
    LaunchDesc d;
    describe_launch(nx, dtype, &d);
    return {q.w, q.n_steps, q.cout_p / 16, d.wave_family ? d.nt : 0, (mode == 1 && d.wmajor) ? d.groups : 0};
}

static int unet_forward_impl(const pbn_unet_op* ops, int n_ops, const pbn_unet_buf* bufs, int n_bufs,
                             const int32_t* n_rows, const void* input, int ld_input, const int32_t* const* k3,
                             const int32_t* k5, const int32_t* const* down, const int32_t* const* up, void* arena,
                             size_t arena_bytes, int dtype, void* splitk_ws, size_t splitk_bytes, pbn_stream_t stream,
                             hipEvent_t* events, const int32_t* n_rows_dev = nullptr, const int32_t* rows_expected = nullptr) {
    if (!ops || !bufs || !n_rows || !input || !arena || n_ops < 1 || n_bufs < 2 || n_bufs > 512) return PBN_ERR_ARG;
    int64_t offs[512];
    if (pbn_unet_arena_bytes(bufs, n_bufs, n_rows, dtype, offs) > arena_bytes) return PBN_ERR_WORKSPACE;
    static const int pf_env = getenv("PBN_CONV_PREFETCH") ? atoi(getenv("PBN_CONV_PREFETCH")) : 0;
    const PlanArena B(arena, offs, bufs, input, ld_input, esize(dtype));
    const MapTables T{k3, k5, down, up};
    for (int i = 0; i < n_ops; ++i) {
        const pbn_unet_op& o = ops[i];
        if (!op_index_ok(o.in_buf, o.res_buf, o.out_buf, o.level_in, o.level_out, n_bufs)) return PBN_ERR_ARG;
        const OpTables m = op_tables(o.map_kind, o.level_in, o.level_out, T);
        if (!m.ok) return PBN_ERR_ARG;
        const bool dual = o.in2_buf >= 0;
        ConvHints hints;
        if (rows_expected && n_rows_dev) hints.rows_expected = rows_expected[o.level_out];
        if (pf_env && i + 1 < n_ops) hints.next = next_weights(ops[i + 1], n_bufs, T, n_rows, B, dtype, pf_env);
        if (events) PBN_HIP_CHECK(hipEventRecord(events[2 * i], (hipStream_t)stream));
        if (o.in2_buf >= n_bufs) return PBN_ERR_ARG;
        const int rc = spconv_launch({.in_feat = B.at(o.in_buf, o.in_col), .ld_in = B.ld(o.in_buf), .n_in = n_rows[o.level_in],
                                      .nbr = m.fwd, .n_offsets = m.K,
                                      .n_out_dev = n_rows_dev ? n_rows_dev + o.level_out : nullptr, .n_out = n_rows[o.level_out],
                                      .w_packed = o.w, .vecs_per_offset = o.vpo, .n_steps = o.n_steps, .cout_padded = o.cout_p,
                                      .scale = o.scale, .shift = o.shift,
                                      .residual = o.res_buf >= 0 ? B.at(o.res_buf, o.res_col) : nullptr,
                                      .ld_res = o.res_buf >= 0 ? B.ld(o.res_buf) : 0, .relu = o.relu,
                                      .out_feat = B.at(o.out_buf, o.out_col), .ld_out = B.ld(o.out_buf), .dtype = dtype,
                                      .workspace = splitk_ws, .workspace_bytes = splitk_bytes,
                                      .in2_feat = dual ? B.at(o.in2_buf, o.in2_col) : nullptr, .ld_in2 = dual ? B.ld(o.in2_buf) : 0,
                                      .n_in2 = dual ? n_rows[o.level_out] : 0, .vecs_second = dual ? o.vpo2 : 0},
                                     hints, (hipStream_t)stream);
        if (rc != PBN_OK) return rc;
        if (events) PBN_HIP_CHECK(hipEventRecord(events[2 * i + 1], (hipStream_t)stream));
    }
    return PBN_OK;
}

extern "C" int pbn_unet_forward(const pbn_unet_op* ops, int n_ops, const pbn_unet_buf* bufs, int n_bufs,
                                const int32_t* n_rows, const void* input, int ld_input, const int32_t* const* k3,
                                const int32_t* k5, const int32_t* const* down, const int32_t* const* up, void* arena,
                                size_t arena_bytes, int dtype, void* splitk_ws, size_t splitk_bytes, pbn_stream_t stream) {
    return unet_forward_impl(ops, n_ops, bufs, n_bufs, n_rows, input, ld_input, k3, k5, down, up, arena, arena_bytes, dtype,
                             splitk_ws, splitk_bytes, stream, nullptr);
}

extern "C" int pbn_unet_forward_dev(const pbn_unet_op* ops, int n_ops, const pbn_unet_buf* bufs, int n_bufs,
                                    const int32_t* n_rows_cap, const int32_t* n_rows_dev, const int32_t* rows_expected,
                                    const void* input, int ld_input, const int32_t* const* k3, const int32_t* k5,
                                    const int32_t* const* down, const int32_t* const* up, void* arena, size_t arena_bytes,
                                    int dtype, void* splitk_ws, size_t splitk_bytes, pbn_stream_t stream) {
    if (!n_rows_dev) return PBN_ERR_ARG;
    return unet_forward_impl(ops, n_ops, bufs, n_bufs, n_rows_cap, input, ld_input, k3, k5, down, up, arena, arena_bytes, dtype,
                             splitk_ws, splitk_bytes, stream, nullptr, n_rows_dev, rows_expected);
}

extern "C" int pbn_unet_forward_timed(const pbn_unet_op* ops, int n_ops, const pbn_unet_buf* bufs, int n_bufs,
                                      const int32_t* n_rows, const void* input, int ld_input, const int32_t* const* k3,
                                      const int32_t* k5, const int32_t* const* down, const int32_t* const* up,
                                      void* arena, size_t arena_bytes, int dtype, void* splitk_ws, size_t splitk_bytes,
                                      pbn_stream_t stream, float* op_ms) {
    if (!op_ms || n_ops < 1 || n_ops > 4096) return PBN_ERR_ARG;
    hipEvent_t* ev = new hipEvent_t[2 * (size_t)n_ops];
    int made = 0, rc = PBN_OK;
    for (; made < 2 * n_ops; ++made)
        if (hipEventCreate(&ev[made]) != hipSuccess) { rc = PBN_ERR_HIP; break; }
    if (rc == PBN_OK)
        rc = unet_forward_impl(ops, n_ops, bufs, n_bufs, n_rows, input, ld_input, k3, k5, down, up, arena, arena_bytes,
                               dtype, splitk_ws, splitk_bytes, stream, ev);
    if (rc == PBN_OK && hipStreamSynchronize((hipStream_t)stream) != hipSuccess) rc = PBN_ERR_HIP;
    if (rc == PBN_OK)
        for (int i = 0; i < n_ops; ++i)
            if (hipEventElapsedTime(&op_ms[i], ev[2 * i], ev[2 * i + 1]) != hipSuccess) { rc = PBN_ERR_HIP; break; }
    for (int i = 0; i < made; ++i) (void)hipEventDestroy(ev[i]);
    delete[] ev;
    return rc;
}
```

### pbnet_amd/csrc/pbn_common.h

```cpp
#pragma once
#include <hip/hip_runtime.h>
#include <stdint.h>
#include "../../include/pbnet_hip.h"

namespace pbn {

constexpr int WAVE = 64;
constexpr int SEL_MAX_CLASSES = 32;

extern thread_local int g_last_hip_error;

#define PBN_HIP_CHECK(expr)                                  \
    do {                                                     \
        hipError_t _e = (expr);                              \
        if (_e != hipSuccess) {                              \
            pbn::g_last_hip_error = (int)_e;                 \
            return PBN_ERR_HIP;                              \
        }                                                    \
    } while (0)

#define PBN_LAUNCH_CHECK() PBN_HIP_CHECK(hipGetLastError())

static inline int cdiv(long long a, long long b) { return (int)((a + b - 1) / b); }
static inline size_t align_up(size_t x, size_t a) { return (x + a - 1) / a * a; }

struct Carver {
    char* base;
    size_t off;
    size_t cap;
    bool ok;
    Carver(void* p, size_t bytes) : base((char*)p), off(0), cap(bytes), ok(true) {}
    template <typename T>
    T* take(size_t n) {
        size_t start = align_up(off, 256);
        size_t end = start + n * sizeof(T);
        if (base != nullptr && end > cap) ok = false;
        off = end;
        return base ? (T*)(base + start) : (T*)nullptr;
    }
};

__device__ __forceinline__ int lane_id() { return (int)(threadIdx.x & 63); }

__device__ __forceinline__ int wave_reduce_add(int v) {
#pragma unroll
    for (int o = 32; o > 0; o >>= 1) v += __shfl_xor(v, o, 64);
    return v;
}

__device__ __forceinline__ uint32_t hash64(uint64_t k) {
    k ^= k >> 30;
    k *= 0xbf58476d1ce4e5b9ULL;
    k ^= k >> 27;
    k *= 0x94d049bb133111ebULL;
    k ^= k >> 31;
    return (uint32_t)k;
}

constexpr int SCAN_THREADS = 256;
constexpr int SCAN_ITEMS = 8;
constexpr int SCAN_TILE = SCAN_THREADS * SCAN_ITEMS;

static inline size_t scan_tmp_ints(long long n) { return (size_t)cdiv(n, SCAN_TILE) + 2; }

int scan_exclusive_i32(const int* in, int* out, int n, int* tmp, int* total, hipStream_t stream);
size_t scan_chained_state_words(long long n);
int scan_exclusive_i32_chained(const int* in, int* out, int n, unsigned long long* state_zeroed, int* total, int* status,
                               hipStream_t stream);

struct MapJobs {
    const int* coords[6]; const int* n_dev[6]; const unsigned long long* keys[6]; const int* vals[6]; int* nbr[6];
    unsigned mask[6]; int ksize[6], stride[6];
    int n_jobs, n_max, x_fastest;
};
int kernel_maps_multi(const MapJobs& jobs, long long total_max, hipStream_t stream);

struct FillRange { void* p; size_t bytes; unsigned char value; };
int fill_ranges(const FillRange* ranges, int n, hipStream_t stream);
static inline int fill_bytes(void* p, unsigned char value, size_t bytes, hipStream_t stream) {
    const FillRange r{p, bytes, value};
    return fill_ranges(&r, 1, stream);
}

int coords_unique_impl(const int32_t* coords, const int32_t* n_dev, int n_max, uint64_t* table_keys, int32_t* table_vals,
                       int capacity, int32_t* unique_index, int32_t* inverse, int32_t* unique_coords, int32_t* n_unique,
                       void* workspace, size_t workspace_bytes, int32_t* status, bool clear, hipStream_t stream);
int coords_stride_impl(const int32_t* fine_coords, const int32_t* n_fine_dev, int n_fine_max, int stride_out,
                       uint64_t* table_keys, int32_t* table_vals, int capacity, int32_t* coarse_coords,
                       int32_t* parent_row, int32_t* child_k, int32_t* nbr_down, int32_t* nbr_up, int32_t* n_coarse,
                       void* workspace, size_t workspace_bytes, int32_t* status, bool clear, hipStream_t stream);

int coords_insert_identity(const int32_t* coords, const int32_t* n_dev, int n_max, uint64_t* keys, int32_t* vals,
                           int capacity, int32_t* out_coords, int32_t* n_out, int32_t* status, hipStream_t stream);
int coords_morton_iota(const int32_t* coords, const int32_t* n_dev, int n_max, uint64_t* keys, int32_t* iota,
                       hipStream_t stream);
int coords_apply_perm(const int32_t* ucoords, const int32_t* perm32, const int32_t* uidx32, const int32_t* inv32, int n_max,
                      int32_t* sorted_coords, int64_t* perm64, int64_t* inv_perm64, int64_t* uidx64, int64_t* inv64,
                      hipStream_t stream);
int coords_build_upper(int n, int want_k5, int x_fastest, void* arena, const pbn_coords_layout* L, hipStream_t stream);
int coords_number_first(const int32_t* slot_of_row, const int32_t* table_vals, const int32_t* n_dev, int n_max, int32_t* scan_tmp,
                        int32_t* newid, int32_t* first_row, int32_t* n_out, const int32_t* status, hipStream_t stream);
size_t pyramid_scratch_bytes(int n);
int coords_prepare_sorted(const int32_t* coords, const int32_t* n_dev, int n, int want_k5, int x_fastest, void* arena,
                          const pbn_prepare_layout* P, hipStream_t stream);
constexpr int RADIX_U32_DIGIT_BITS = 11, RADIX_U32_PASSES = 3;
size_t radix_sort_u32_scratch_bytes(int n);
int radix_sort_u32(unsigned long long* keys_a, unsigned long long* keys_b, int32_t* vals_a, int32_t* vals_b, int n,
                   const unsigned* ghist, int32_t* status, void* scratch, size_t scratch_bytes, hipStream_t stream);
size_t sort_pairs_temp_bytes(int n);
int sort_pairs_u64_i32(const uint64_t* keys_in, uint64_t* keys_out, const int32_t* vals_in, int32_t* vals_out, int n,
                       void* temp, size_t temp_bytes, hipStream_t stream);

}
```

### pbnet_amd/csrc/pyramid.hip

```cpp
#include "coords_dev.h"

namespace pbn {
namespace {

typedef unsigned long long u64;

constexpr int RADIX_BITS = 11, RADIX = 1 << RADIX_BITS, MAX_PASSES = 4;
#ifndef PBN_SORT_ITEMS
#define PBN_SORT_ITEMS 8
#endif
constexpr int SORT_ITEMS = PBN_SORT_ITEMS, SORT_TILE = TPB * SORT_ITEMS;
constexpr int PYR_ITEMS = 4, PYR_TILE = TPB * PYR_ITEMS;
constexpr unsigned SPIN_LIMIT = 1u << 24;
constexpr size_t SORT_LDS_BYTES = (size_t)SORT_TILE * 12 + (size_t)(TPB / 64 + 2) * RADIX * 4;

enum { PL_BMIN = 0, PL_XMIN, PL_YMIN, PL_ZMIN, PL_BMAX, PL_XMAX, PL_YMAX, PL_ZMAX, PL_TICKET0 = 8, PL_TICKET_PYR = 12,
       PL_ERROR = 13, PL_STAMPS = 16, PL_WORDS = 64 };
constexpr int PBN_STATUS_KEY_BITS = 4;
constexpr int PBN_STATUS_SPIN = 8;

struct KeyPlan { int b0, x0, y0, z0, e, nbits; };
__device__ __forceinline__ KeyPlan key_plan(const int* __restrict__ plan) {
    KeyPlan k;
    k.b0 = plan[PL_BMIN];
// ... 346 lines not shown
}

__global__ __launch_bounds__(TPB) void k_pyramid(const u64* __restrict__ keys_a, const u64* __restrict__ keys_b,
                                                const int* __restrict__ vals_a, const int* __restrict__ vals_b,
                                                const int* __restrict__ ucoords, const int* n_dev, int n_max,
                                                int* __restrict__ plan, int* __restrict__ status,
                                                u64* __restrict__ state, const PyrOut o) {
    __shared__ int s_wtot[TPB / 64][4];
    __shared__ int s_ex[4];
    __shared__ int s_blk;
    const int n = real_n(n_dev, n_max);
    const int tid = threadIdx.x, lane = tid & 63, wave = tid >> 6;
    if (tid == 0) s_blk = atomicAdd(&plan[PL_TICKET_PYR], 1);
    __syncthreads();
    const int blk = s_blk;
    const bool bad = *status != 0;
    if (blk == 0 && tid == 0 && (n <= 0 || bad)) {
        for (int l = 0; l < 5; ++l) o.counts[l] = bad ? -1 : 0;
    }
    if (n <= 0 || bad) return;
    const int base = blk * PYR_TILE;
    if (base >= n) return;
    const KeyPlan kp = key_plan(plan);
    const int passes = sort_plan(kp.nbits).passes;
    const u64* keys = (passes & 1) ? keys_b : keys_a;
    const int* vals = (passes & 1) ? vals_b : vals_a;

    int r[PYR_ITEMS], rp = 0;
    int4 c[PYR_ITEMS];
    u64 key[PYR_ITEMS];
#pragma unroll
    for (int k = 0; k < PYR_ITEMS; ++k) {
        const int i = base + k * TPB + tid;
        r[k] = i < n ? vals[i] : 0;
        key[k] = i < n ? keys[i] : 0ull;
    }
    const int ip = base + wave * 64 - 1;
    int rpk[PYR_ITEMS];
#pragma unroll
    for (int k = 0; k < PYR_ITEMS; ++k) rpk[k] = (lane == 0 && ip + k * TPB >= 0 && ip + k * TPB < n) ? vals[ip + k * TPB] : -1;
    (void)rp;
#pragma unroll
    for (int k = 0; k < PYR_ITEMS; ++k) c[k] = reinterpret_cast<const int4*>(ucoords)[r[k]];
    int4 cp[PYR_ITEMS];
#pragma unroll
    for (int k = 0; k < PYR_ITEMS; ++k)
        cp[k] = rpk[k] >= 0 ? reinterpret_cast<const int4*>(ucoords)[rpk[k]] : make_int4(-1, 0, 0, 0);
    int f[PYR_ITEMS], wid[PYR_ITEMS][4], carry[4] = {0, 0, 0, 0};
#pragma unroll
    for (int k = 0; k < PYR_ITEMS; ++k) {
        const int i = base + k * TPB + tid;
        int4 p;
        p.x = __shfl_up(c[k].x, 1, 64); p.y = __shfl_up(c[k].y, 1, 64); p.z = __shfl_up(c[k].z, 1, 64); p.w = __shfl_up(c[k].w, 1, 64);
        if (lane == 0) p = cp[k];
        f[k] = 0;
        int inc[4];
#pragma unroll
        for (int l = 1; l <= 4; ++l) {
            const bool first = i < n && (i == 0 || p.x != c[k].x || (p.y >> l) != (c[k].y >> l) || (p.z >> l) != (c[k].z >> l) ||
                                         (p.w >> l) != (c[k].w >> l));
            f[k] |= first ? (1 << (l - 1)) : 0;
            inc[l - 1] = wave_incl_scan_i(first ? 1 : 0);
            if (lane == 63) s_wtot[wave][l - 1] = inc[l - 1];
        }
        __syncthreads();
#pragma unroll
        for (int l = 0; l < 4; ++l) {
            int woff = 0, tot = 0;
            for (int w = 0; w < TPB / 64; ++w) { const int t = s_wtot[w][l]; if (w < wave) woff += t; tot += t; }
            wid[k][l] = carry[l] + woff + inc[l];
            carry[l] += tot;
        }
        __syncthreads();
    }
    const int* tot = carry;
    if (wave == 0) {
        u64* mine = state + (size_t)blk * 2;
        if (lane == 0) {
            const u64 fl = blk == 0 ? 2ull : 1ull;
            st_state(mine + 0, fl << 62 | (u64)(unsigned)tot[0] << 31 | (u64)(unsigned)tot[1]);
            st_state(mine + 1, fl << 62 | (u64)(unsigned)tot[2] << 31 | (u64)(unsigned)tot[3]);
        }
        int ex[4] = {0, 0, 0, 0};
        unsigned spins = 0;
        int p = blk - 1;
        while (p >= 0) {
            const int pp = p - lane;
            u64 a = 0, b = 0;
            if (pp >= 0) { a = ld_state(state + (size_t)pp * 2); b = ld_state(state + (size_t)pp * 2 + 1); }
            const bool ready = pp < 0 || ((a >> 62) != 0 && (a >> 62) == (b >> 62));
            const u64 not_ready = __ballot(!ready);
            const u64 is_prefix = __ballot(pp >= 0 && ready && (a >> 62) == 2);
            int upto = not_ready ? __ffsll((long long)not_ready) - 1 : 64;
            int stop = 64;
            if (is_prefix) { const int fp = __ffsll((long long)is_prefix) - 1; if (fp < upto) { stop = fp; upto = fp + 1; } }
            const bool take = lane < upto && pp >= 0;
            int v[4] = {take ? (int)((a >> 31) & 0x7fffffffu) : 0, take ? (int)(a & 0x7fffffffu) : 0,
                        take ? (int)((b >> 31) & 0x7fffffffu) : 0, take ? (int)(b & 0x7fffffffu) : 0};
#pragma unroll
            for (int l = 0; l < 4; ++l) ex[l] += wave_reduce_add(v[l]);
            if (stop < 64) break;
            if (upto == 0) {
                if (++spins > SPIN_LIMIT) { if (lane == 0) atomicOr(status, PBN_STATUS_SPIN); break; }
                __builtin_amdgcn_s_sleep(1);
            }
            p -= upto;
        }
        if (lane == 0) {
            if (blk > 0) {
                st_state(mine + 0, 2ull << 62 | (u64)(unsigned)(ex[0] + tot[0]) << 31 | (u64)(unsigned)(ex[1] + tot[1]));
                st_state(mine + 1, 2ull << 62 | (u64)(unsigned)(ex[2] + tot[2]) << 31 | (u64)(unsigned)(ex[3] + tot[3]));
            }
            for (int l = 0; l < 4; ++l) s_ex[l] = ex[l];
            if (base + PYR_TILE >= n) {
                o.counts[0] = n;
                for (int l = 0; l < 4; ++l) o.counts[l + 1] = ex[l] + tot[l];
            }
        }
    }
    __syncthreads();
#pragma unroll
    for (int k = 0; k < PYR_ITEMS; ++k) {
        const int i = base + k * TPB + tid;
        if (i >= n) continue;
        int id[4];
#pragma unroll
        for (int l = 0; l < 4; ++l) id[l] = s_ex[l] + wid[k][l] - 1;
        const int4 cc = c[k];
        reinterpret_cast<int4*>(o.coords[0])[i] = cc;
        o.perm[i] = r[k];
        o.inv_perm[r[k]] = i;
        int row = i;
#pragma unroll
        for (int l = 1; l <= 4; ++l) {
            const bool mine = l == 1 || ((f[k] >> (l - 2)) & 1);
            if (mine) {
                const int kk = ((cc.y >> (l - 1)) & 1) + 2 * ((cc.z >> (l - 1)) & 1) + 4 * ((cc.w >> (l - 1)) & 1);
                const int par = id[l - 1];
                o.parent_row[l - 1][row] = par;
                o.child_k[l - 1][row] = kk;
                o.nbr_down[l - 1][(size_t)par * 8 + kk] = row;
                write_up_row(o.up[l - 1], row, kk, par);
            }
            if ((f[k] >> (l - 1)) & 1) {
                const int m = ~((1 << l) - 1);
                reinterpret_cast<int4*>(o.coords[l])[id[l - 1]] = make_int4(cc.x, cc.y & m, cc.z & m, cc.w & m);
                if (l >= 2) o.lkeys[l - 2][id[l - 1]] = key[k] >> (3 * l);
            }
            row = id[l - 1];
        }
    }
}

__device__ __forceinline__ void cube_offset(int k, int ksize, int x_fastest, int& dx, int& dy, int& dz) {
    const int c0 = (ksize & 1) ? ksize / 2 : 0;
    const int a = k % ksize - c0, b = (k / ksize) % ksize - c0, c = k / (ksize * ksize) - c0;
    dx = x_fastest ? a : c; dy = b; dz = x_fastest ? c : a;
}

struct TopJobs { const int* coords[3]; const u64* lkeys[3]; int* nbr[3]; const int* counts; int n_max, x_fastest; };
__global__ __launch_bounds__(TPB) void k_maps_top(const TopJobs jb, const int* __restrict__ plan) {
    const KeyPlan kp = key_plan(plan);
    long long first[4];
    first[0] = 0;
#pragma unroll
    for (int j = 0; j < 3; ++j) { const int c = jb.counts[2 + j]; first[j + 1] = first[j] + (long long)(c > 0 ? min(c, jb.n_max) : 0) * 27; }
    for (long long g = (long long)blockIdx.x * TPB + threadIdx.x; g < first[3]; g += (long long)gridDim.x * TPB) {
        const int j = (g >= first[1]) + (g >= first[2]);
        const int l = 2 + j;
        const long long e = g - first[j];
        const int row = (int)(e / 27), k = (int)(e % 27);
        int dx, dy, dz;
        cube_offset(k, 3, jb.x_fastest, dx, dy, dz);
        const int4 cc = reinterpret_cast<const int4*>(jb.coords[j])[row];
        const int x = cc.y + (dx << l) - kp.x0, y = cc.z + (dy << l) - kp.y0, z = cc.w + (dz << l) - kp.z0;
        int res = -1;
        const int lim = 1 << kp.e;
        if (x >= 0 && y >= 0 && z >= 0 && x < lim && y < lim && z < lim) {
            const u64 want = (((u64)(unsigned)(cc.x - kp.b0) << (3 * kp.e)) | spread3((unsigned)x) | (spread3((unsigned)y) << 1) |
                              (spread3((unsigned)z) << 2)) >> (3 * l);
            const u64* keys = jb.lkeys[j];
            int lo = 0, hi = min(jb.counts[l], jb.n_max);
            while (lo < hi) {
                const int mid = (lo + hi) >> 1;
                if (keys[mid] < want) lo = mid + 1; else hi = mid;
            }
            if (lo < min(jb.counts[l], jb.n_max) && keys[lo] == want) res = lo;
        }
        jb.nbr[j][e] = res;
    }
}

struct DownJob {
    const int* nbr_down; const int* k3_up;
    const int* n_parents_dev; int* k3; int* k5; int n_max, x_fastest;
};
__global__ __launch_bounds__(TPB) void k_maps_down(const DownJob jb) {
    __shared__ int s_tab[TPB / 64][27 * 8];
    const int lane = threadIdx.x & 63, wave = threadIdx.x >> 6;
    const int n_par = real_n(jb.n_parents_dev, jb.n_max);
    int* tab = s_tab[wave];
    for (int par = blockIdx.x * (TPB / 64) + wave; par < n_par; par += gridDim.x * (TPB / 64)) {
        const int q = lane < 27 ? jb.k3_up[(size_t)par * 27 + lane] : -1;
#pragma unroll
        for (int e0 = 0; e0 < 27 * 8; e0 += 64) {
            const int e = e0 + lane;
            const int qq = __shfl(q, (e >> 3) < 27 ? (e >> 3) : 0, 64);
            if (e < 27 * 8) tab[e] = qq >= 0 ? jb.nbr_down[(size_t)qq * 8 + (e & 7)] : -1;
        }
        __builtin_amdgcn_fence(__ATOMIC_RELEASE, "wavefront");
        __builtin_amdgcn_wave_barrier();
        int first = -1, nchild = 0;
        unsigned cks = 0;
#pragma unroll
        for (int ck = 0; ck < 8; ++ck) {
            const int row = tab[13 * 8 + ck];
            if (row >= 0) { if (first < 0) first = row; cks |= (unsigned)ck << (3 * nchild); ++nchild; }
        }
        auto entry = [&](int j, int k, int ksize) -> int {
            const int ck = (int)(cks >> (3 * j)) & 7;
            int dx, dy, dz;
            cube_offset(k, ksize, jb.x_fastest, dx, dy, dz);
            const int tx = (ck & 1) + dx, ty = ((ck >> 1) & 1) + dy, tz = ((ck >> 2) & 1) + dz;
            const int px = tx >> 1, py = ty >> 1, pz = tz >> 1;
            const int kp3 = jb.x_fastest ? (px + 1) + 3 * (py + 1) + 9 * (pz + 1) : (pz + 1) + 3 * (py + 1) + 9 * (px + 1);
            return tab[kp3 * 8 + ((tx & 1) + 2 * (ty & 1) + 4 * (tz & 1))];
        };
        for (int e = lane; e < nchild * 27; e += 64) {
            const int j = e / 27;
            jb.k3[(size_t)first * 27 + e] = entry(j, e - j * 27, 3);
        }
        if (jb.k5)
            for (int e = lane; e < nchild * 125; e += 64) {
                const int j = e / 125;
                jb.k5[(size_t)first * 125 + e] = entry(j, e - j * 125, 5);
            }
        __builtin_amdgcn_wave_barrier();
    }
}

}

size_t pyramid_scratch_bytes(int n) {
    const size_t N = (size_t)(n > 0 ? n : 1);
    const size_t sort_blocks = (size_t)cdiv((long long)N, SORT_TILE), pyr_blocks = (size_t)cdiv((long long)N, PYR_TILE);
    size_t b = 0;
    b += align_up(PL_WORDS * sizeof(int), 256);
    b += align_up((size_t)MAX_PASSES * RADIX * sizeof(unsigned), 256);
    b += align_up((size_t)MAX_PASSES * sort_blocks * (RADIX / 2) * sizeof(u64), 256);
    b += align_up(pyr_blocks * 2 * sizeof(u64), 256);
    b += 3 * align_up(N * sizeof(u64), 256);
    return b + 256;
}

int coords_prepare_sorted(const int32_t* coords, const int32_t* n_dev, int n, int want_k5, int x_fastest, void* arena,
                          const pbn_prepare_layout* P, hipStream_t st) {
    char* A = (char*)arena;
    const pbn_coords_layout* L = &P->pyramid;
    auto I = [&](int64_t o) { return (int32_t*)(A + o); };
    const size_t N = (size_t)(n > 0 ? n : 1);
    const size_t sort_blocks = (size_t)cdiv((long long)N, SORT_TILE), pyr_blocks = (size_t)cdiv((long long)N, PYR_TILE);
    char* S = A + P->sort_temp;
    size_t off = 0;
    auto take = [&](size_t bytes) { char* p = S + off; off += align_up(bytes, 256); return p; };
    int* plan = (int*)take(PL_WORDS * sizeof(int));
    unsigned* ghist = (unsigned*)take((size_t)MAX_PASSES * RADIX * sizeof(unsigned));
    u64* sort_state = (u64*)take((size_t)MAX_PASSES * sort_blocks * (RADIX / 2) * sizeof(u64));
    u64* pyr_state = (u64*)take(pyr_blocks * 2 * sizeof(u64));
    u64* lkeys[3];
    for (int j = 0; j < 3; ++j) lkeys[j] = (u64*)take(N * sizeof(u64));
    if (off > (size_t)P->sort_temp_bytes) return PBN_ERR_WORKSPACE;
    int32_t* n_unique = I(P->n_unique);
    int32_t* status = n_unique + 8;
    int32_t* counts = I(L->counts);
    {
        const FillRange fr[] = {{A + P->n_unique, 16 * sizeof(int), 0},
                                {A + P->tmp_keys, (size_t)(P->tmp_vals - P->tmp_keys), 0xff},
                                {A + P->tmp_vals, (size_t)(P->unique_index - P->tmp_vals), 0x7f},
                                {A + L->counts, 16 * sizeof(int), 0},
                                {A + L->nbr_down[0], (size_t)(L->vals[0] - L->nbr_down[0]), 0xff},
                                {plan + PL_BMIN, 4 * sizeof(int), 0x7f},
                                {plan + PL_BMAX, 4 * sizeof(int), 0x80},
                                {plan + PL_TICKET0, (PL_WORDS - PL_TICKET0) * sizeof(int), 0},
                                {ghist, (size_t)((char*)lkeys[0] - (char*)ghist), 0}};
        const int frc = fill_ranges(fr, 9, st);
        if (frc != PBN_OK) return frc;
    }
    if (n == 0) return PBN_OK;
    if (!coords) return PBN_ERR_ARG;
    Carver cv(A + L->workspace, (size_t)L->workspace_bytes);
    int* slot_of_row = cv.take<int>(N);
    int* first_row = cv.take<int>(N);
    int* newid = cv.take<int>(N);
    int* scan_tmp = cv.take<int>(scan_tmp_ints((long long)N));
    if (!cv.ok) return PBN_ERR_WORKSPACE;
    const int cap = pbn_hash_capacity(n);
    const int gb = (int)(cdiv(n, TPB * 4) < 2048 ? cdiv(n, TPB * 4) : 2048);
    const int gi = (int)(cdiv(n, TPB) < 8192 ? cdiv(n, TPB) : 8192);
    hipLaunchKernelGGL(k_insert_bbox, dim3(gi), dim3(TPB), 0, st, coords, n_dev, n, (u64*)(A + P->tmp_keys), I(P->tmp_vals),
                       (unsigned)cap - 1, slot_of_row, status, plan);
    int rc = coords_number_first(slot_of_row, I(P->tmp_vals), n_dev, n, scan_tmp, newid, first_row, n_unique, status, st);
    if (rc != PBN_OK) return rc;
    u64* keys_a = (u64*)(A + P->sort_keys);
    u64* keys_b = keys_a + N;
    int* vals_a = I(P->sort_vals);
    int* vals_b = vals_a + N;
    hipLaunchKernelGGL(k_unique_keys, dim3(gb), dim3(TPB), 0, st, coords, slot_of_row, first_row, newid, n_dev, n, I(P->uidx32),
                       I(P->inv32), (long long*)(A + P->unique_index), (long long*)(A + P->inverse), I(P->ucoords), plan, status,
                       keys_a, vals_a, ghist);
    static const bool lds_attr = (hipFuncSetAttribute((const void*)k_sort_pass, hipFuncAttributeMaxDynamicSharedMemorySize,
                                                      (int)SORT_LDS_BYTES) == hipSuccess);
    if (!lds_attr) return PBN_ERR_HIP;
    for (int p = 0; p < MAX_PASSES; ++p)
        hipLaunchKernelGGL(k_sort_pass, dim3((unsigned)sort_blocks), dim3(TPB), SORT_LDS_BYTES, st, (p & 1) ? keys_b : keys_a,
                           (p & 1) ? keys_a : keys_b, (p & 1) ? vals_b : vals_a, (p & 1) ? vals_a : vals_b, n_unique, n, p, plan,
                           status, ghist, sort_state + (size_t)p * sort_blocks * (RADIX / 2));
    PyrOut o;
    for (int l = 0; l < 5; ++l) o.coords[l] = I(L->coords[l]);
    for (int l = 0; l < 4; ++l) {
        o.parent_row[l] = I(L->parent_row[l]); o.child_k[l] = I(L->child_k[l]); o.nbr_down[l] = I(L->nbr_down[l]);
        o.up[l] = I(L->up[l]);
    }
    for (int j = 0; j < 3; ++j) o.lkeys[j] = lkeys[j];
    o.counts = counts;
    o.perm = (long long*)(A + P->perm);
    o.inv_perm = (long long*)(A + P->inv_perm);
    hipLaunchKernelGGL(k_pyramid, dim3((unsigned)pyr_blocks), dim3(TPB), 0, st, keys_a, keys_b, vals_a, vals_b, I(P->ucoords),
                       n_unique, n, plan, status, pyr_state, o);
    {
        TopJobs tj;
        for (int j = 0; j < 3; ++j) { tj.coords[j] = I(L->coords[2 + j]); tj.lkeys[j] = lkeys[j]; tj.nbr[j] = I(L->k3[2 + j]); }
        tj.counts = counts; tj.n_max = n; tj.x_fastest = x_fastest;
        long long blocks = cdiv((long long)n * 27 / 4 + 1, TPB);
        if (blocks > 2048) blocks = 2048;
        hipLaunchKernelGGL(k_maps_top, dim3((unsigned)blocks), dim3(TPB), 0, st, tj, plan);
        for (int l = 1; l >= 0; --l) {
            DownJob dj;
            dj.nbr_down = I(L->nbr_down[l]); dj.k3_up = I(L->k3[l + 1]); dj.n_parents_dev = counts + l + 1; dj.k3 = I(L->k3[l]);
            dj.k5 = (l == 0 && want_k5) ? I(L->k5) : nullptr; dj.n_max = n; dj.x_fastest = x_fastest;
            long long bl = cdiv((long long)n, (TPB / 64) * 2);
            if (bl > 8192) bl = 8192;
            if (bl < 1) bl = 1;
            hipLaunchKernelGGL(k_maps_down, dim3((unsigned)bl), dim3(TPB), 0, st, dj);
        }
    }
    PBN_LAUNCH_CHECK();
    return PBN_OK;
}

static_assert(RADIX_U32_DIGIT_BITS == RADIX_BITS, "radix_sort_u32 runs sort_pass_body<8>: 11-bit digits");

size_t radix_sort_u32_scratch_bytes(int n) {
    const size_t sort_blocks = (size_t)cdiv(n > 0 ? n : 1, SORT_TILE);
    return align_up(PL_WORDS * sizeof(int), 256) + align_up((size_t)RADIX_U32_PASSES * sort_blocks * (RADIX / 2) * sizeof(u64), 256);
}

int radix_sort_u32(unsigned long long* keys_a, unsigned long long* keys_b, int32_t* vals_a, int32_t* vals_b, int n,
                   const unsigned* ghist, int32_t* status, void* scratch, size_t scratch_bytes, hipStream_t st) {
    if (n <= 0) return PBN_OK;
    if (scratch_bytes < radix_sort_u32_scratch_bytes(n)) return PBN_ERR_WORKSPACE;
    const size_t sort_blocks = (size_t)cdiv(n, SORT_TILE);
    int* words = (int*)scratch;
    u64* state = (u64*)((char*)scratch + align_up(PL_WORDS * sizeof(int), 256));
    const int frc = fill_bytes(scratch, 0, radix_sort_u32_scratch_bytes(n), st);
    if (frc != PBN_OK) return frc;
    static const bool lds_attr = (hipFuncSetAttribute((const void*)k_sort_pass_u32, hipFuncAttributeMaxDynamicSharedMemorySize,
                                                      (int)SORT_LDS_BYTES) == hipSuccess);
    if (!lds_attr) return PBN_ERR_HIP;
    for (int p = 0; p < RADIX_U32_PASSES; ++p)
        hipLaunchKernelGGL(k_sort_pass_u32, dim3((unsigned)sort_blocks), dim3(TPB), SORT_LDS_BYTES, st, (p & 1) ? keys_b : keys_a,
                           (p & 1) ? keys_a : keys_b, (p & 1) ? vals_b : vals_a, (p & 1) ? vals_a : vals_b, n, p, words, status,
                           ghist, state + (size_t)p * sort_blocks * (RADIX / 2));
    PBN_LAUNCH_CHECK();
    return PBN_OK;
}

}
```

### pbnet_amd/csrc/spconv.hip

```cpp
#include <cmath>
#include <cstdlib>
#include "spconv_common.h"

namespace pbn {
namespace {

constexpr int CGMAX = 4;


#define PBN_LDS_ADDR(p) ((unsigned)(uintptr_t)((__attribute__((address_space(3))) void*)(p)))

#ifdef PBN_CONV_TIMING
__device__ unsigned g_conv_timing[4 * 64 * 8 + 8];
#define PBN_STAMP(POS, I)                                                                                             \
    if (timed_ && lane == 0 && (POS) - g_lo < 64)                                                                     \
        s_time[(wave * 64 + ((POS) - g_lo)) * 8 + (I)] = (unsigned)__builtin_readcyclecounter();
#define PBN_TIMING_SKIP_DMA if (a.dbg & 64) continue
#else
#define PBN_STAMP(POS, I)
#define PBN_TIMING_SKIP_DMA
#endif

template <typename T, int NF, int NT, int RING, int NW = 4>
__global__ __launch_bounds__(NW * 64) void k_spconv(const ConvArgs a) {
// ... 332 lines not shown
__global__ __launch_bounds__(256) void k_spconv_reduce(const ConvArgs a) {
    const int ldp = a.ntiles_total * 16;
    const int vec_per_row = ldp >> 2;
    const int n = a.n_out_dev ? min(*a.n_out_dev, a.n_out) : a.n_out;
    const long long e = (long long)blockIdx.x * 256 + threadIdx.x;
    if (e >= (long long)n * vec_per_row) return;
    const int p = (int)(e / vec_per_row), c0 = (int)(e - (long long)p * vec_per_row) * 4;
    f32x4 v = f32x4{0.f, 0.f, 0.f, 0.f};
    for (int z = 0; z < a.ksplit; ++z) {
        const float4 t = *reinterpret_cast<const float4*>(a.partial + ((size_t)z * a.n_out_pad + p) * ldp + c0);
        v[0] += t.x; v[1] += t.y; v[2] += t.z; v[3] += t.w;
    }
    const int orow = a.row_perm ? a.row_perm[p] : p;
    if (a.scale) {
        const float4 sc = *reinterpret_cast<const float4*>(a.scale + c0);
        v[0] *= sc.x; v[1] *= sc.y; v[2] *= sc.z; v[3] *= sc.w;
    }
    if (a.shift) {
        const float4 sh = *reinterpret_cast<const float4*>(a.shift + c0);
        v[0] += sh.x; v[1] += sh.y; v[2] += sh.z; v[3] += sh.w;
    }
    if (a.residual) v += load4<T>(reinterpret_cast<const T*>(a.residual) + (size_t)orow * a.ld_res + c0);
    if (a.relu) {
        v[0] = fmaxf(v[0], 0.f); v[1] = fmaxf(v[1], 0.f); v[2] = fmaxf(v[2], 0.f); v[3] = fmaxf(v[3], 0.f);
    }
    store4<T>(reinterpret_cast<T*>(a.out) + (size_t)orow * a.ld_out + c0, v);
}

template <typename T, int NF, int NT, int RING, int NW = 4>
int launch_ring(ConvArgs a, int ngroups, float* workspace, size_t workspace_bytes, hipStream_t stream) {
    constexpr int TM = 16 * NW * NF;
    constexpr int CONV_TPB = NW * 64;
    const int KS = a.K | 1;
    a.cg = 1;
    if ((a.vpo & 3) == 0) {
        const int spo = a.vpo >> 2;
        for (int c = CGMAX; c >= 1; --c)
            if (spo % c == 0) { a.cg = c; break; }
    }
    const int n_groups = a.n_steps / a.cg;
    const size_t lds = (size_t)RING * a.cg * NT * 1024 +
                       sizeof(int) * ((size_t)TM * KS + ((a.K + 4) & ~3) + 3 * ((size_t)n_groups + 4) + 2 * NT * 16 + 4);
    if (lds > 160 * 1024) return PBN_ERR_UNSUPPORTED;
    auto kern = k_spconv<T, NF, NT, RING, NW>;
    if (lds > 64 * 1024)
        PBN_HIP_CHECK(hipFuncSetAttribute((const void*)kern, hipFuncAttributeMaxDynamicSharedMemorySize, (int)lds));
    const int tiles = cdiv(a.n_out, TM);
    a.ksplit = 1;
    a.partial = nullptr;
    a.n_out_pad = tiles * TM;
    const long long wgs = (long long)cdiv(a.n_sel, TM) * ngroups;
    static const float t_group = getenv("PBN_CONV_TGROUP") ? (float)atof(getenv("PBN_CONV_TGROUP")) : 1.5f;
    static const int max_wgs = getenv("PBN_CONV_SPLIT") ? atoi(getenv("PBN_CONV_SPLIT")) : 512;
    if (workspace && wgs < 256 && n_groups >= 8) {
        const float slab_us = 2.0f * (float)a.n_out_pad * (float)(a.ntiles_total * 16) * 4.0f / 3.0e6f;
        long long want = (long long)(sqrtf((float)n_groups * t_group / (slab_us > 0.05f ? slab_us : 0.05f)) + 0.5f);
        const long long by_steps = n_groups / 2;
        const long long by_ws = (long long)(workspace_bytes / ((size_t)a.n_out_pad * a.ntiles_total * 16 * sizeof(float)));
        const long long by_wgs = (RING == 3 ? 256 : max_wgs) / wgs;
        if (want > by_wgs) want = by_wgs;
        if (want > by_steps) want = by_steps;
        if (want > by_ws) want = by_ws;
        if (want > 32) want = 32;
        if (want > 1) { a.ksplit = (int)want; a.partial = workspace; }
    }
    hipLaunchKernelGGL(kern, dim3(tiles, ngroups, a.ksplit), dim3(CONV_TPB), lds, stream, a);
    if (a.ksplit > 1) {
        const long long total = (long long)a.n_out * (a.ntiles_total * 4);
        hipLaunchKernelGGL(k_spconv_reduce<T>, dim3(cdiv(total, 256)), dim3(256), 0, stream, a);
    }
    PBN_LAUNCH_CHECK();
    return PBN_OK;
}

template <typename T, int NF, int NT>
int launch_one(const ConvArgs& a, int ngroups, float* ws, size_t wsb, hipStream_t stream) {
    static const int ring_env = getenv("PBN_CONV_RING") ? atoi(getenv("PBN_CONV_RING")) : 2;
    static const long long w8_env = getenv("PBN_CONV_WAVES8") ? atoll(getenv("PBN_CONV_WAVES8")) : 0;
    if constexpr (NF == 2) {
        if (a.K <= 32 && (w8_env == 1 || (w8_env > 1 && a.n_out >= w8_env))) {
            const int rc = launch_ring<T, NF, NT, 2, 8>(a, ngroups, ws, wsb, stream);
            if (rc != PBN_ERR_UNSUPPORTED) return rc;
        }
    }
    if constexpr (NF == 1) {
        if (ring_env == 3 && a.n_out < 8192) {
            const int rc = launch_ring<T, NF, NT, 3>(a, ngroups, ws, wsb, stream);
            if (rc != PBN_ERR_UNSUPPORTED) return rc;
        }
    }
    return launch_ring<T, NF, NT, 2>(a, ngroups, ws, wsb, stream);
}

template <typename T, int NF>
int launch_nt(const ConvArgs& a, float* ws, size_t wsb, hipStream_t stream) {
    const int ntt = a.ntiles_total;
    if (ntt % 8 == 0) return launch_one<T, NF, 8>(a, ntt / 8, ws, wsb, stream);
    if (ntt % 6 == 0) return launch_one<T, NF, 6>(a, ntt / 6, ws, wsb, stream);
    if (ntt % 4 == 0) return launch_one<T, NF, 4>(a, ntt / 4, ws, wsb, stream);
    if (ntt % 2 == 0) return launch_one<T, NF, 2>(a, ntt / 2, ws, wsb, stream);
    return launch_one<T, NF, 1>(a, ntt, ws, wsb, stream);
}

template <typename T>
int launch_t(const ConvArgs& a, int rows_per_wave, float* ws, size_t wsb, hipStream_t stream) {
    if (rows_per_wave == 64) return launch_nt<T, 4>(a, ws, wsb, stream);
    if (rows_per_wave == 32) return launch_nt<T, 2>(a, ws, wsb, stream);
    return launch_nt<T, 1>(a, ws, wsb, stream);
}

__global__ __launch_bounds__(256) void k_gather_rows(const uint4* __restrict__ in, const long long* __restrict__ idx,
                                                    int n, int vec_per_row, int ld_in_vec, int ld_out_vec,
                                                    uint4* __restrict__ out) {
    const long long e = (long long)blockIdx.x * 256 + threadIdx.x;
    if (e >= (long long)n * vec_per_row) return;
    const int i = (int)(e / vec_per_row), v = (int)(e % vec_per_row);
    const long long r = idx[i];
    out[(size_t)i * ld_out_vec + v] = r >= 0 ? in[(size_t)r * ld_in_vec + v] : make_uint4(0u, 0u, 0u, 0u);
}

}
}

using namespace pbn;

namespace {

struct Family { int id; bool (*wanted)(const ConvArgs&, int dtype); int (*launch)(const ConvArgs&, int dtype, int cfg, hipStream_t); };

int launch_wave_auto(const ConvArgs& a, int dtype, int, hipStream_t stream) {
    static const int force_cfg = getenv("PBN_WAVE_CFG") ? atoi(getenv("PBN_WAVE_CFG")) : 0;
    return launch_wave(a, dtype, force_cfg, stream);
}

const Family FAMILIES[] = {
#ifdef PBN_EXPERIMENTS
    {3, pc_family_wanted, launch_pc},
#endif
    {2, rs_family_wanted, launch_rs},
    {1, wave_family_wanted, launch_wave_auto},
};

}

int pbn::spconv_launch(const ConvCall& c, const ConvHints& hints, hipStream_t stream) {
    if (c.n_out < 0 || c.n_in < 0 || c.n_offsets < 1 || c.vecs_per_offset < 1 || c.n_steps < 1 || c.cout_padded < 16 || (c.cout_padded & 15))
        return PBN_ERR_ARG;
    if (!(c.vecs_per_offset == 1 || c.vecs_per_offset == 2 || (c.vecs_per_offset & 3) == 0)) return PBN_ERR_ARG;
    const int n_main = (c.n_offsets * c.vecs_per_offset + 3) / 4;
    if (c.in2_feat) {
        if ((c.vecs_per_offset & 3) || c.vecs_second < 4 || (c.vecs_second & 3) || !c.nbr || c.row_perm || c.n_in2 < c.n_out) return PBN_ERR_ARG;
        if (c.n_steps < n_main + (c.vecs_second >> 2) || c.n_steps > n_main + (c.vecs_second >> 2) + 3) return PBN_ERR_ARG;
    } else if (c.n_steps != n_main) return PBN_ERR_ARG;
    if (!c.nbr && c.n_offsets != 1) return PBN_ERR_ARG;
    if (c.n_out == 0) return PBN_OK;
    if (!c.in_feat || !c.w_packed || !c.out_feat) return PBN_ERR_ARG;
    const int dtype = c.dtype, esz = dtype == PBN_F32 ? 4 : 2;
    if ((c.ld_in * esz) % 16 || (c.ld_out * esz) % 8 || (c.residual && (c.ld_res * esz) % 8)) return PBN_ERR_ARG;
    if (((uintptr_t)c.in_feat | (uintptr_t)c.w_packed) & 15) return PBN_ERR_ARG;
    if (c.in2_feat && ((c.ld_in2 * esz) % 16 || ((uintptr_t)c.in2_feat & 15))) return PBN_ERR_ARG;
    const unsigned long long in2_extent = c.in2_feat ? (unsigned long long)c.n_in2 * (unsigned long long)c.ld_in2 * (unsigned long long)esz : 0ull;
    if (in2_extent >= 0x80000000ull) return PBN_ERR_RANGE;
    const unsigned long long in_extent = (unsigned long long)c.n_in * (unsigned long long)c.ld_in * (unsigned long long)esz;
    const unsigned long long w_extent = (unsigned long long)c.n_steps * (unsigned long long)(c.cout_padded / 16) * 1024ull;
    if (in_extent >= 0x80000000ull || w_extent >= 0x80000000ull) return PBN_ERR_RANGE;
    if (!c.nbr && c.n_in < c.n_out) return PBN_ERR_ARG;
    ConvArgs a;
    a.in_bytes = (unsigned)in_extent; a.w_bytes = (unsigned)w_extent;
    a.in = c.in_feat; a.nbr = c.nbr; a.row_perm = c.row_perm; a.n_out_dev = c.n_out_dev; a.w = c.w_packed; a.scale = c.scale;
    a.shift = c.shift; a.residual = c.residual; a.out = c.out_feat; a.ld_in = c.ld_in; a.ld_res = c.ld_res; a.ld_out = c.ld_out;
    a.K = c.n_offsets; a.vpo = c.vecs_per_offset; a.n_steps = c.n_steps; a.ntiles_total = c.cout_padded / 16; a.n_out = c.n_out;
    a.relu = c.relu;
    a.n_sel = (hints.rows_expected > 0 && c.n_out_dev) ? (hints.rows_expected < c.n_out ? hints.rows_expected : c.n_out) : c.n_out;
    a.ksplit = 1; a.partial = nullptr; a.n_out_pad = 0; a.cg = 1; a.wmajor = 0;
    a.in2 = c.in2_feat; a.ld_in2 = c.ld_in2; a.vpo2 = c.vecs_second; a.n_main = n_main; a.in2_bytes = (unsigned)in2_extent;
    a.pf_w = hints.next.w; a.pf_steps = hints.next.steps; a.pf_ntt = hints.next.ntt; a.pf_nt = hints.next.nt; a.pf_groups = hints.next.groups;
    static const int dbg_env = getenv("PBN_CONV_DBG") ? atoi(getenv("PBN_CONV_DBG")) : 0;
    a.dbg = dbg_env;
    int rows_per_wave = c.rows_per_wave;
    if (rows_per_wave >= 10000) {
        const int cfg = rows_per_wave - 10000;
#ifdef PBN_EXPERIMENTS
        if ((cfg % 100000) / 1000 == 3) return launch_pc(a, dtype, (cfg / 100000) * 16, stream);
#endif
        return launch_rs(a, dtype, cfg, stream);
    }
    if (rows_per_wave >= 100) return launch_wave(a, dtype, rows_per_wave, stream);
    if (rows_per_wave == 0)
        for (const Family& f : FAMILIES)
            if (f.wanted(a, dtype)) {
                const int rc = f.launch(a, dtype, 0, stream);
                if (rc != PBN_ERR_UNSUPPORTED) return rc;
            }
    float* ws = reinterpret_cast<float*>(c.workspace);
    if (((uintptr_t)c.workspace) & 15) ws = nullptr;
    if (rows_per_wave != 16 && rows_per_wave != 32 && rows_per_wave != 64) rows_per_wave = (a.n_sel > 64) ? 32 : 16;
    switch (dtype) {
        case PBN_F32: return launch_t<float>(a, rows_per_wave, ws, c.workspace_bytes, stream);
        case PBN_BF16: return launch_t<__hip_bfloat16>(a, rows_per_wave, ws, c.workspace_bytes, stream);
        case PBN_F16: return launch_t<__half>(a, rows_per_wave, ws, c.workspace_bytes, stream);
        default: return PBN_ERR_ARG;
    }
}

extern "C" int pbn_spconv_forward(const void* in_feat, int ld_in, int n_in, const int32_t* nbr, int n_offsets,
                                  const int32_t* row_perm, const int32_t* n_out_dev, int n_out, const void* w_packed,
                                  int vecs_per_offset, int n_steps, int cout_padded, const float* scale,
                                  const float* shift, const void* residual, int ld_res, int relu, void* out_feat,
                                  int ld_out, int dtype, int rows_per_wave, void* workspace, size_t workspace_bytes,
                                  pbn_stream_t stream) {
    return spconv_launch({.in_feat = in_feat, .ld_in = ld_in, .n_in = n_in, .nbr = nbr, .n_offsets = n_offsets, .row_perm = row_perm,
                          .n_out_dev = n_out_dev, .n_out = n_out, .w_packed = w_packed, .vecs_per_offset = vecs_per_offset,
                          .n_steps = n_steps, .cout_padded = cout_padded, .scale = scale, .shift = shift, .residual = residual,
                          .ld_res = ld_res, .relu = relu, .out_feat = out_feat, .ld_out = ld_out, .dtype = dtype,
                          .rows_per_wave = rows_per_wave, .workspace = workspace, .workspace_bytes = workspace_bytes},
                         ConvHints{}, (hipStream_t)stream);
}

extern "C" int pbn_spconv_family(int n_out, int n_offsets, int vecs_per_offset, int n_steps, int cout_padded, int dtype, int has_map) {
    if (n_out < 0 || n_offsets < 1 || vecs_per_offset < 1 || n_steps < 1 || cout_padded < 16 || (cout_padded & 15)) return PBN_ERR_ARG;
    const ConvArgs a = shape_args(n_out, n_offsets, vecs_per_offset, n_steps, cout_padded, has_map != 0, 0, 0);
    for (const Family& f : FAMILIES)
        if (f.wanted(a, dtype)) return f.id;
    return 0;
}

extern "C" int pbn_spconv_forward_dual(const void* in_feat, int ld_in, int n_in, const int32_t* nbr, int n_offsets,
                                       const int32_t* n_out_dev, int n_out, const void* w_packed, int vecs_per_offset,
                                       int n_steps, int cout_padded, const float* scale, const float* shift,
                                       const void* residual, int ld_res, int relu, void* out_feat, int ld_out, int dtype,
                                       int rows_per_wave, void* workspace, size_t workspace_bytes, const void* in2_feat,
                                       int ld_in2, int n_in2, int vecs_second, pbn_stream_t stream) {
    if (!in2_feat) return PBN_ERR_ARG;
    return spconv_launch({.in_feat = in_feat, .ld_in = ld_in, .n_in = n_in, .nbr = nbr, .n_offsets = n_offsets, .n_out_dev = n_out_dev,
                          .n_out = n_out, .w_packed = w_packed, .vecs_per_offset = vecs_per_offset, .n_steps = n_steps,
                          .cout_padded = cout_padded, .scale = scale, .shift = shift, .residual = residual, .ld_res = ld_res,
                          .relu = relu, .out_feat = out_feat, .ld_out = ld_out, .dtype = dtype, .rows_per_wave = rows_per_wave,
                          .workspace = workspace, .workspace_bytes = workspace_bytes, .in2_feat = in2_feat, .ld_in2 = ld_in2,
                          .n_in2 = n_in2, .vecs_second = vecs_second},
                         ConvHints{}, (hipStream_t)stream);
}

#ifdef PBN_CONV_TIMING
extern "C" int pbn_conv_timing_read(unsigned* host) {
    PBN_HIP_CHECK(hipDeviceSynchronize());
    PBN_HIP_CHECK(hipMemcpyFromSymbol(host, HIP_SYMBOL(pbn::g_conv_timing), sizeof(unsigned) * (4 * 64 * 8 + 8)));
    return PBN_OK;
}
#endif

extern "C" int pbn_gather_rows(const void* in, int ld_in_bytes, const int64_t* idx, int n, int row_bytes, void* out,
                               int ld_out_bytes, pbn_stream_t stream_) {
    hipStream_t stream = (hipStream_t)stream_;
    if (n < 0 || row_bytes <= 0 || (row_bytes & 15) || (ld_in_bytes & 15) || (ld_out_bytes & 15)) return PBN_ERR_ARG;
    if (n == 0) return PBN_OK;
    if (!in || !idx || !out) return PBN_ERR_ARG;
    const int vpr = row_bytes / 16;
    const long long total = (long long)n * vpr;
    hipLaunchKernelGGL(k_gather_rows, dim3(cdiv(total, 256)), dim3(256), 0, stream, (const uint4*)in,
                       (const long long*)idx, n, vpr, ld_in_bytes / 16, ld_out_bytes / 16, (uint4*)out);
    PBN_LAUNCH_CHECK();
    return PBN_OK;
}
```

### pbnet_amd/csrc/spconv_common.h

```cpp
#pragma once
#include <hip/hip_bf16.h>
#include <hip/hip_fp16.h>
#include "pbn_common.h"

namespace pbn {

typedef float f32x4 __attribute__((ext_vector_type(4)));
typedef unsigned u32x4 __attribute__((ext_vector_type(4)));
typedef int i32x4 __attribute__((ext_vector_type(4)));
typedef __bf16 bf16x8 __attribute__((ext_vector_type(8)));
typedef _Float16 f16x8 __attribute__((ext_vector_type(8)));

struct ConvArgs {
    const void* in;
    const int* nbr;
    const int* row_perm;
    const int* n_out_dev;
    const void* w;
    const float* scale;
    const float* shift;
    const void* residual;
    void* out;
    int ld_in, ld_res, ld_out;
    unsigned in_bytes, w_bytes;
    int K, vpo, n_steps, ntiles_total;
    int n_out, relu;
    int n_sel;
    int ksplit;
    float* partial;
    int n_out_pad;
    int cg;
    int wmajor;
    int dbg;
    const void* in2;
    int ld_in2, vpo2, n_main;
    unsigned in2_bytes;
    const void* pf_w;
    int pf_steps, pf_ntt, pf_nt, pf_groups;
};

struct LaunchDesc { int wave_family, nt, groups, wmajor; };
struct NextWeights { const void* w; int steps, ntt, nt, groups; };
struct ConvCall {
    const void* in_feat; int ld_in; int n_in;
    const int32_t* nbr; int n_offsets;
    const int32_t* row_perm = nullptr; const int32_t* n_out_dev = nullptr; int n_out;
    const void* w_packed; int vecs_per_offset; int n_steps; int cout_padded;
    const float* scale = nullptr; const float* shift = nullptr; const void* residual = nullptr; int ld_res = 0; int relu = 0;
    void* out_feat; int ld_out; int dtype; int rows_per_wave = 0;
    void* workspace = nullptr; size_t workspace_bytes = 0;
    const void* in2_feat = nullptr; int ld_in2 = 0; int n_in2 = 0; int vecs_second = 0;
};
struct ConvHints { int rows_expected = 0; NextWeights next = {}; };
int spconv_launch(const ConvCall& c, const ConvHints& hints, hipStream_t stream);
inline ConvArgs shape_args(int n_sel, int K, int vpo, int n_steps, int cout_p, bool has_map, unsigned w_bytes, unsigned in_bytes) {
    static const int no_neighbour = -1;
    ConvArgs a{};
    a.nbr = has_map ? &no_neighbour : nullptr;
    a.K = K; a.vpo = vpo; a.n_steps = n_steps; a.ntiles_total = cout_p / 16; a.n_out = a.n_sel = n_sel;
    a.w_bytes = w_bytes; a.in_bytes = in_bytes;
    return a;
}

namespace {

template <typename T> struct Tr;
template <> struct Tr<float> { static constexpr int ELEMS = 4; };
template <> struct Tr<__hip_bfloat16> { static constexpr int ELEMS = 8; };
template <> struct Tr<__half> { static constexpr int ELEMS = 8; };

template <typename T>
__device__ __forceinline__ void mfma_step(const u32x4& w, const u32x4& x, f32x4& acc);

template <>
__device__ __forceinline__ void mfma_step<float>(const u32x4& w, const u32x4& x, f32x4& acc) {
    acc = __builtin_amdgcn_mfma_f32_16x16x4f32(__uint_as_float(w[0]), __uint_as_float(x[0]), acc, 0, 0, 0);
    acc = __builtin_amdgcn_mfma_f32_16x16x4f32(__uint_as_float(w[1]), __uint_as_float(x[1]), acc, 0, 0, 0);
    acc = __builtin_amdgcn_mfma_f32_16x16x4f32(__uint_as_float(w[2]), __uint_as_float(x[2]), acc, 0, 0, 0);
    acc = __builtin_amdgcn_mfma_f32_16x16x4f32(__uint_as_float(w[3]), __uint_as_float(x[3]), acc, 0, 0, 0);
}
template <>
__device__ __forceinline__ void mfma_step<__hip_bfloat16>(const u32x4& w, const u32x4& x, f32x4& acc) {
    acc = __builtin_amdgcn_mfma_f32_16x16x32_bf16(__builtin_bit_cast(bf16x8, w), __builtin_bit_cast(bf16x8, x), acc, 0, 0, 0);
}
template <>
__device__ __forceinline__ void mfma_step<__half>(const u32x4& w, const u32x4& x, f32x4& acc) {
    acc = __builtin_amdgcn_mfma_f32_16x16x32_f16(__builtin_bit_cast(f16x8, w), __builtin_bit_cast(f16x8, x), acc, 0, 0, 0);
}

template <typename T> __device__ __forceinline__ f32x4 load4(const T* p);
template <> __device__ __forceinline__ f32x4 load4<float>(const float* p) {
    const float4 v = *reinterpret_cast<const float4*>(p);
    return f32x4{v.x, v.y, v.z, v.w};
}
template <> __device__ __forceinline__ f32x4 load4<__hip_bfloat16>(const __hip_bfloat16* p) {
    const uint2 v = *reinterpret_cast<const uint2*>(p);
    return f32x4{__uint_as_float(v.x << 16), __uint_as_float(v.x & 0xffff0000u), __uint_as_float(v.y << 16),
                 __uint_as_float(v.y & 0xffff0000u)};
}
template <> __device__ __forceinline__ f32x4 load4<__half>(const __half* p) {
    const uint2 v = *reinterpret_cast<const uint2*>(p);
    const __half2 a = __builtin_bit_cast(__half2, v.x), b = __builtin_bit_cast(__half2, v.y);
    const float2 fa = __half22float2(a), fb = __half22float2(b);
    return f32x4{fa.x, fa.y, fb.x, fb.y};
}
__device__ __forceinline__ unsigned bf16_rne(float f) {
    unsigned u = __float_as_uint(f);
    if ((u & 0x7fffffffu) > 0x7f800000u) return (u >> 16) | 0x40u;
    return (u + 0x7fffu + ((u >> 16) & 1u)) >> 16;
}
template <typename T> __device__ __forceinline__ void store4(T* p, const f32x4& v);
template <> __device__ __forceinline__ void store4<float>(float* p, const f32x4& v) {
    *reinterpret_cast<float4*>(p) = make_float4(v[0], v[1], v[2], v[3]);
}
template <> __device__ __forceinline__ void store4<__hip_bfloat16>(__hip_bfloat16* p, const f32x4& v) {
    uint2 o;
    o.x = bf16_rne(v[0]) | (bf16_rne(v[1]) << 16);
    o.y = bf16_rne(v[2]) | (bf16_rne(v[3]) << 16);
    *reinterpret_cast<uint2*>(p) = o;
}
template <> __device__ __forceinline__ void store4<__half>(__half* p, const f32x4& v) {
    const __half2 a = __floats2half2_rn(v[0], v[1]), b = __floats2half2_rn(v[2], v[3]);
    uint2 o;
    o.x = __builtin_bit_cast(unsigned, a);
    o.y = __builtin_bit_cast(unsigned, b);
    *reinterpret_cast<uint2*>(p) = o;
}

__device__ __forceinline__ void prefetch_drain(u32x4& sink) { asm volatile("s_waitcnt vmcnt(0)" : "+v"(sink)); }
__device__ __forceinline__ u32x4 prefetch_next_weights(const ConvArgs& a, int block, int n_blocks, int tid, int tpb) {
    u32x4 sink = {0u, 0u, 0u, 0u};
    if (!a.pf_w) return sink;
    const int lane = tid & 63, wave = tid >> 6, waves = tpb >> 6;
    int owners = 1, xcd = 0, n_owned = a.pf_ntt / (a.pf_nt > 0 ? a.pf_nt : 1), g0 = 0, gstride = 1;
    if (a.pf_groups > 0) {
        xcd = block & 7;
        owners = 8;
        if (a.pf_groups >= 8) { g0 = xcd; gstride = 8; n_owned = (a.pf_groups - xcd + 7) >> 3; }
        else { g0 = xcd % a.pf_groups; gstride = a.pf_groups; n_owned = 1; }
    } else {
        n_owned = 1;
    }
    const int nt = a.pf_groups > 0 ? a.pf_nt : a.pf_ntt;
    const int rank = a.pf_groups > 0 ? (block >> 3) : block;
    const int nrank = a.pf_groups > 0 ? (n_blocks + 7 - xcd) >> 3 : n_blocks;
    const long long pieces = (long long)a.pf_steps * n_owned * nt;
    const long long per = (pieces + (nrank > 0 ? nrank : 1) - 1) / (nrank > 0 ? nrank : 1);
    const long long lo = (long long)rank * per, hi = lo + per < pieces ? lo + per : pieces;
    (void)owners;
    const unsigned char* base = reinterpret_cast<const unsigned char*>(a.pf_w);
    for (long long q = lo + wave; q < hi; q += waves) {
        const int s = (int)(q / (n_owned * nt));
        const int rem = (int)(q - (long long)s * (n_owned * nt));
        const int gi = rem / nt, t = rem - gi * nt;
        const int tile = (g0 + gi * gstride) * nt + t;
        const u32x4* src = reinterpret_cast<const u32x4*>(base + ((size_t)s * a.pf_ntt + tile) * 1024) + lane;
        asm volatile("global_load_dwordx4 %0, %1, off" : "+v"(sink) : "v"(src) : "memory");
    }
    return sink;
}

__device__ __forceinline__ int xcd_tile(int b, int nt) {
    const int q = nt >> 3, r = nt & 7, xcd = b & 7, idx = b >> 3;
    return (xcd < r ? xcd * (q + 1) : r * (q + 1) + (xcd - r) * q) + idx;
}

}

int launch_wave(const ConvArgs& a, int dtype, int force_cfg, hipStream_t stream);
bool wave_family_wanted(const ConvArgs& a, int dtype);
void describe_launch(const ConvArgs& a, int dtype, LaunchDesc* d);

bool rs_family_wanted(const ConvArgs& a, int dtype);
int launch_rs(const ConvArgs& a, int dtype, int cfg, hipStream_t stream);


#ifdef PBN_EXPERIMENTS
int launch_pc(const ConvArgs& a, int dtype, int rows, hipStream_t stream);
bool pc_family_wanted(const ConvArgs& a, int dtype);
#endif

}
```

### pbnet_amd/csrc/spconv_wave.hip

```cpp
#include <cstdlib>
#include <cstring>
#include "spconv_common.h"

namespace pbn {
namespace {

constexpr unsigned OOB = 0x80000000u;
constexpr unsigned UNIT_NONE = 0xffffu;

constexpr int MAX_DEPTH = 8;

#ifdef PBN_CONV_TIMING
constexpr int WT_BLOCKS = 1024;
__device__ unsigned long long g_wave_timing[WT_BLOCKS * 8 * 8 + 8];
#define PBN_WSTAMP(I)                                                                                                 \
    if (lane == 0 && wt_blk < WT_BLOCKS && wave < 8)                                                                  \
        g_wave_timing[(wt_blk * 8 + wave) * 8 + (I)] = (I) == 7 ? wall_clock64() : __builtin_readcyclecounter();
#else
#define PBN_WSTAMP(I)
#endif
#ifndef PBN_WAVE_DEPTH
#define PBN_WAVE_DEPTH 2
#endif
#ifndef PBN_WAVE_XCOAL
#define PBN_WAVE_XCOAL 1
#endif
constexpr int pipe_depth(int nf, int nt) {
    (void)nf; (void)nt;
    return PBN_WAVE_DEPTH;
}

template <int NF, int NT>
struct Stage {
    u32x4 w[NT];
    u32x4 x[NF];
};

__device__ __forceinline__ void buf_load_asm(u32x4& dst, const i32x4& rs, unsigned voff, unsigned soff) {
    asm volatile("buffer_load_dwordx4 %0, %1, %2, %3 offen" : "+v"(dst) : "v"(voff), "s"(rs), "s"(soff) : "memory");
}

template <typename T>
__device__ __forceinline__ void epilogue_store(const ConvArgs& a, f32x4 v, int orow, int c0) {
    if (a.scale) {
        const float4 sc = *reinterpret_cast<const float4*>(a.scale + c0);
        v[0] *= sc.x; v[1] *= sc.y; v[2] *= sc.z; v[3] *= sc.w;
    }
    if (a.shift) {
        const float4 sh = *reinterpret_cast<const float4*>(a.shift + c0);
        v[0] += sh.x; v[1] += sh.y; v[2] += sh.z; v[3] += sh.w;
    }
    if (a.residual) v += load4<T>(reinterpret_cast<const T*>(a.residual) + (size_t)orow * a.ld_res + c0);
    if (a.relu) {
        v[0] = fmaxf(v[0], 0.f); v[1] = fmaxf(v[1], 0.f); v[2] = fmaxf(v[2], 0.f); v[3] = fmaxf(v[3], 0.f);
    }
    store4<T>(reinterpret_cast<T*>(a.out) + (size_t)orow * a.ld_out + c0, v);
}

#ifndef PBN_WAVE_RED_KB
#define PBN_WAVE_RED_KB 64
#endif
constexpr int ksplit_round_tiles(int kw, int tm, int nt) {
    return (kw * tm * nt * 64 <= PBN_WAVE_RED_KB * 1024) ? nt : (nt < 2 ? nt : 2);
}
constexpr int ksplit_red_pitch(int ntb) { return ntb * 16 + 4; }

struct TileMap { int row_tile, group; bool valid; };
__device__ __forceinline__ TileMap map_block(const ConvArgs& a, int n_row_tiles, int n_groups) {
    TileMap m;
    const int b = blockIdx.x;
    if (!a.wmajor) {
        m.group = b / n_row_tiles;
        m.row_tile = xcd_tile(b - m.group * n_row_tiles, n_row_tiles);
        m.valid = m.group < n_groups;
        return m;
    }
    const int xcd = b & 7, idx = b >> 3;
    if (n_groups >= 8) {
        const int gl = idx / n_row_tiles;
        m.group = xcd + 8 * gl;
        m.row_tile = idx - gl * n_row_tiles;
        m.valid = m.group < n_groups;
    } else {
        const int share = 8 / n_groups;
        m.group = xcd % n_groups;
        m.row_tile = (xcd / n_groups) + share * idx;
        m.valid = m.row_tile < n_row_tiles;
    }
    return m;
}

template <typename T, int NF, int NT, int KW, bool KSPLIT, bool KLIST = false>
__global__ __launch_bounds__(KW * 64) void k_spconv_wave(const ConvArgs a) {
    static_assert(!KLIST || KSPLIT, "the shared step list is a K-split feature");
    static_assert(Tr<T>::ELEMS * sizeof(T) == 16, "one gather vector is 16 bytes");
    constexpr int RW = NF * 16;
    constexpr int TM = KSPLIT ? RW : KW * RW;
    constexpr int NTB = ksplit_round_tiles(KW, TM, NT);
    constexpr int TPB = KW * 64;
    constexpr int B = pipe_depth(NF, NT);
    extern __shared__ __attribute__((aligned(16))) unsigned char smem[];
    const int K = a.K;
    const int KS = K | 1;
    int* s_nbr = reinterpret_cast<int*>(smem);
    unsigned* s_units = reinterpret_cast<unsigned*>(s_nbr + ((TM * KS + 3) & ~3));
    const int units_pitch = (KSPLIT && !KLIST) ? 0 : a.n_steps + 2 * MAX_DEPTH + (KLIST ? 64 : 0);
    int* s_none = reinterpret_cast<int*>(s_units + ((KW * units_pitch + 3) & ~3));
    float* s_ss = reinterpret_cast<float*>(s_none + 4);
    float* s_red = s_ss + 2 * NT * 16;

    const int tid = threadIdx.x, lane = tid & 63;
    const int wave = __builtin_amdgcn_readfirstlane(tid >> 6);
#ifdef PBN_CONV_TIMING
    const int wt_blk = blockIdx.x;
    if (tid == 0 && wt_blk == 0) { g_wave_timing[WT_BLOCKS * 64] = gridDim.x; g_wave_timing[WT_BLOCKS * 64 + 1] = gridDim.y; }
#endif
    PBN_WSTAMP(7);
    PBN_WSTAMP(0);
    const int n_groups = a.ntiles_total / NT;
    u32x4 pf_sink = prefetch_next_weights(a, blockIdx.x, gridDim.x, tid, TPB);
    const int n_rows_now = a.n_out_dev ? min(*a.n_out_dev, a.n_out) : a.n_out;
    if (n_rows_now <= 0) { prefetch_drain(pf_sink); return; }
    const TileMap tm = map_block(a, (n_rows_now + TM - 1) / TM, n_groups);
    if (!tm.valid) { prefetch_drain(pf_sink); return; }
    const int row0 = tm.row_tile * TM;
    const int tile0 = tm.group * NT;
    const int g = lane >> 4, rl = lane & 15;

    const unsigned long long in_addr = (unsigned long long)a.in, w_addr = (unsigned long long)a.w;
    const i32x4 rs_in = {(int)(unsigned)in_addr, (int)(unsigned)(in_addr >> 32), (int)a.in_bytes, 0x00020000};
    const i32x4 rs_w = {(int)(unsigned)w_addr, (int)(unsigned)(w_addr >> 32), (int)a.w_bytes, 0x00020000};
    const unsigned ld_bytes = (unsigned)a.ld_in * (unsigned)sizeof(T);
    const unsigned long long in2_addr = (unsigned long long)a.in2;
    const i32x4 rs_in2 = {(int)(unsigned)in2_addr, (int)(unsigned)(in2_addr >> 32), (int)a.in2_bytes, 0x00020000};
    const unsigned ld2_bytes = (unsigned)a.ld_in2 * (unsigned)sizeof(T);
    const int n_main = a.in2 ? a.n_main : a.n_steps;
    const unsigned w_lane = (unsigned)lane * 16u;
    const unsigned w_tile0 = (unsigned)tile0 * 1024u;
    const unsigned w_step_bytes = (unsigned)a.ntiles_total * 1024u;
    const int vpo = a.vpo;
    const bool wide = (vpo & 3) == 0;
    const int spo = wide ? (vpo >> 2) : 1;
    const int vshift = (vpo == 2) ? 1 : 0;
    const float inv_vpo = 1.0f / (float)vpo;
    const int n_steps = a.n_steps;
    unsigned* my_units = s_units + wave * units_pitch;

    auto step_of = [&](int i) -> int {
        if constexpr (KLIST) return __builtin_amdgcn_readfirstlane((int)my_units[i * KW + wave]);
        else if constexpr (KSPLIT) return i * KW + wave;
        else return __builtin_amdgcn_readfirstlane((int)my_units[i]);
    };
    auto issue_w = [&](Stage<NF, NT>& st, int step) {
        const unsigned w_soff = (unsigned)(step < n_steps ? step : 0) * w_step_bytes + w_tile0;
#ifdef PBN_CONV_TIMING
        if (a.dbg & 2) return;
        const unsigned w_lane = (a.dbg & 16) ? OOB : (unsigned)lane * 16u;
#endif
#pragma unroll
        for (int t = 0; t < NT; ++t) buf_load_asm(st.w[t], rs_w, w_lane, w_soff + (unsigned)t * 1024u);
    };

    Stage<NF, NT> st[B];
#pragma unroll
    for (int s = 0; s < B; ++s) {
#pragma unroll
        for (int t = 0; t < NT; ++t) st[s].w[t] = u32x4{0u, 0u, 0u, 0u};
#pragma unroll
        for (int f = 0; f < NF; ++f) st[s].x[f] = u32x4{0u, 0u, 0u, 0u};
    }
    if constexpr (KSPLIT) {
        if (tid < NT * 32) {
            const int c = tile0 * 16 + (tid < NT * 16 ? tid : tid - NT * 16);
            const float* src = tid < NT * 16 ? a.scale : a.shift;
            s_ss[tid] = src ? src[c] : (tid < NT * 16 ? 1.0f : 0.0f);
        }
    }
    const int n = a.n_out_dev ? min(*a.n_out_dev, a.n_out) : a.n_out;
    if (row0 >= n) { prefetch_drain(pf_sink); return; }
    if (tid == 0) *s_none = -1;

    if (a.nbr && !a.row_perm && row0 + TM <= n && KS == K && ((TM * K) & 3) == 0) {
        const int4* src = reinterpret_cast<const int4*>(a.nbr + (size_t)row0 * K);
        int4* dst = reinterpret_cast<int4*>(s_nbr);
        for (int e = tid; e < (TM * K) >> 2; e += TPB) dst[e] = src[e];
    } else {
        const float inv_k = 1.0f / (float)K;
        for (int e = tid; e < TM * K; e += TPB) {
            const int r = (int)(((float)e + 0.5f) * inv_k), k = e - r * K;
            const int p = row0 + r;
            int v = -1;
            if (p < n) {
                const int row = a.row_perm ? a.row_perm[p] : p;
                v = a.nbr ? a.nbr[(size_t)row * K + k] : row;
            }
            s_nbr[r * KS + k] = v;
        }
    }
    prefetch_drain(pf_sink);
    __syncthreads();
    PBN_WSTAMP(1);

    const int wrow0 = KSPLIT ? 0 : wave * RW;
    int n_units;
    if constexpr (KSPLIT && !KLIST) {
        n_units = a.n_steps > wave ? (a.n_steps - wave + KW - 1) / KW : 0;
    } else {
        constexpr int SCAN = KSPLIT ? TM : RW;
        bool any0 = false, any1 = false;
        if (lane < K)
            for (int r = 0; r < SCAN; ++r) any0 |= s_nbr[(wrow0 + r) * KS + lane] >= 0;
        if (64 + lane < K)
            for (int r = 0; r < SCAN; ++r) any1 |= s_nbr[(wrow0 + r) * KS + 64 + lane] >= 0;
        const unsigned long long pop0 = __ballot(any0), pop1 = __ballot(any1);
        auto populated = [&](int k) -> bool { return ((k < 64 ? pop0 >> k : pop1 >> (k - 64)) & 1ull) != 0ull; };
        int base = 0;
        for (int s0 = 0; s0 < a.n_steps; s0 += 64) {
            const int s = s0 + lane;
            bool ok = false;
            int ko = 0;
            if (s < a.n_steps) {
                if (s >= n_main) {
                    ok = true;
                } else if (wide) {
                    ko = s / spo;
                    ok = populated(ko);
                } else {
                    ko = (s * 4) >> vshift;
                    const int span = 4 >> vshift;
                    for (int q = 0; q < span; ++q)
                        if (ko + q < K) ok |= populated(ko + q);
                }
            }
            const unsigned long long m = __ballot(ok);
            if (ok) my_units[base + __popcll(m & ((1ULL << lane) - 1ULL))] = (unsigned)s;
            base += __popcll(m);
        }
        constexpr int NSENT = (2 * B + 2) * (KLIST ? KW : 1);
        static_assert(NSENT <= 64, "one store per lane writes the sentinels");
        if (lane < NSENT) my_units[base + lane] = UNIT_NONE;
        if constexpr (KLIST) n_units = base > wave ? (base - wave + KW - 1) / KW : 0;
        else n_units = base;
        __builtin_amdgcn_fence(__ATOMIC_RELEASE, "wavefront");
        __builtin_amdgcn_wave_barrier();
    }
    PBN_WSTAMP(2);

    f32x4 acc[NF][NT];
#pragma unroll
    for (int f = 0; f < NF; ++f)
#pragma unroll
        for (int t = 0; t < NT; ++t) acc[f][t] = f32x4{0.f, 0.f, 0.f, 0.f};

    const int my_row = wrow0 + (PBN_WAVE_XCOAL ? (lane >> 2) : rl);
    const int my_chunk = PBN_WAVE_XCOAL ? (lane & 3) : g;
    const int xpose_addr = (4 * (lane & 15) + (lane >> 4)) * 4;
    struct Idx { int src[NF]; unsigned cvb; bool second; };
    auto fetch_idx = [&](int step) -> Idx {
        const int v = step * 4 + my_chunk;
        Idx ix;
        ix.second = __builtin_amdgcn_readfirstlane((int)(step >= n_main && step < n_steps)) != 0;
        if (ix.second) {
            const int cv = v - n_main * 4;
            ix.cvb = (unsigned)cv * 16u;
#pragma unroll
            for (int f = 0; f < NF; ++f) {
                const int p = row0 + my_row + f * 16;
                ix.src[f] = (p < n && cv < a.vpo2) ? p : -1;
            }
            return ix;
        }
        const int ko = (int)(((float)v + 0.5f) * inv_vpo);
        const bool live = step < n_steps && ko < K;
        ix.cvb = (unsigned)(v - ko * vpo) * 16u;
#pragma unroll
        for (int f = 0; f < NF; ++f) ix.src[f] = *(live ? s_nbr + (my_row + f * 16) * KS + ko : s_none);
        return ix;
    };
    auto issue_x = [&](Stage<NF, NT>& st, const Idx& ix) {
#ifdef PBN_CONV_TIMING
        if (a.dbg & 1) return;
#endif
        const i32x4 rs = {__builtin_amdgcn_readfirstlane(ix.second ? rs_in2[0] : rs_in[0]),
                          __builtin_amdgcn_readfirstlane(ix.second ? rs_in2[1] : rs_in[1]),
                          __builtin_amdgcn_readfirstlane(ix.second ? rs_in2[2] : rs_in[2]), 0x00020000};
        const unsigned ldb = ix.second ? ld2_bytes : ld_bytes;
#pragma unroll
        for (int f = 0; f < NF; ++f) {
            const unsigned voff = ix.src[f] >= 0 ? (unsigned)ix.src[f] * ldb + ix.cvb : OOB;
            buf_load_asm(st.x[f], rs, voff, 0u);
        }
    };
    auto compute = [&](const Stage<NF, NT>& st) {
#ifdef PBN_CONV_TIMING
        if (a.dbg & 4) return;
#endif
#if PBN_WAVE_XCOAL
        u32x4 xo[NF];
#pragma unroll
        for (int f = 0; f < NF; ++f)
#pragma unroll
            for (int d = 0; d < 4; ++d) xo[f][d] = (unsigned)__builtin_amdgcn_ds_bpermute(xpose_addr, (int)st.x[f][d]);
#pragma unroll
        for (int t = 0; t < NT; ++t)
#pragma unroll
            for (int f = 0; f < NF; ++f) mfma_step<T>(st.w[t], xo[f], acc[f][t]);
#else
#pragma unroll
        for (int t = 0; t < NT; ++t)
#pragma unroll
            for (int f = 0; f < NF; ++f) mfma_step<T>(st.w[t], st.x[f], acc[f][t]);
#endif
    };

    {
        constexpr int BEHIND = (B - 1) * (NT + NF);
        auto wait_unit = [&](Stage<NF, NT>& u) {
            asm volatile("s_waitcnt vmcnt(%1)" : "+v"(u.w[0]) : "n"(BEHIND));
#pragma unroll
            for (int t = 1; t < NT; ++t) asm volatile("" : "+v"(u.w[t]));
#pragma unroll
            for (int f = 0; f < NF; ++f) asm volatile("" : "+v"(u.x[f]));
        };
        int step = step_of(0);
        Idx ix = fetch_idx(step);
        int raw_next = 0;
        if constexpr (KLIST) raw_next = (int)my_units[KW + wave];
        else if constexpr (!KSPLIT) raw_next = (int)my_units[1];
        auto slot = [&](Stage<NF, NT>& u, int k) {
            issue_w(u, step);
            issue_x(u, ix);
            if constexpr (KLIST) {
                step = __builtin_amdgcn_readfirstlane(raw_next);
                raw_next = (int)my_units[(k + 2) * KW + wave];
            } else if constexpr (KSPLIT) {
                step = step_of(k + 1);
            } else {
                step = __builtin_amdgcn_readfirstlane(raw_next);
                raw_next = (int)my_units[k + 2];
            }
            ix = fetch_idx(step);
        };
#pragma unroll
        for (int s = 0; s < B; ++s) slot(st[s], s);
        PBN_WSTAMP(3);
        for (int i = 0; i < n_units; i += B) {
#pragma unroll
            for (int s = 0; s < B; ++s) {
                wait_unit(st[s]);
                compute(st[s]);
                __builtin_amdgcn_sched_barrier(0);
                slot(st[s], i + B + s);
                __builtin_amdgcn_sched_barrier(0);
            }
        }
        asm volatile("s_waitcnt vmcnt(0)" ::: "memory");
#pragma unroll
        for (int s = 0; s < B; ++s) {
#pragma unroll
            for (int t = 0; t < NT; ++t) asm volatile("" : "+v"(st[s].w[t]));
#pragma unroll
            for (int f = 0; f < NF; ++f) asm volatile("" : "+v"(st[s].x[f]));
        }
    }
    PBN_WSTAMP(4);

    if constexpr (!KSPLIT) {
#pragma unroll
        for (int f = 0; f < NF; ++f) {
            const int p = row0 + wave * RW + f * 16 + rl;
            if (p >= n) continue;
            const int orow = a.row_perm ? a.row_perm[p] : p;
#pragma unroll
            for (int t = 0; t < NT; ++t) epilogue_store<T>(a, acc[f][t], orow, (tile0 + t) * 16 + g * 4);
        }
    } else {
        constexpr int RP = NTB * 16;
        constexpr int RPP = ksplit_red_pitch(NTB);
        T* out = reinterpret_cast<T*>(a.out);
        const T* res = reinterpret_cast<const T*>(a.residual);
#pragma unroll
        for (int t0 = 0; t0 < NT; t0 += NTB) {
#pragma unroll
            for (int f = 0; f < NF; ++f)
#pragma unroll
                for (int tt = 0; tt < NTB; ++tt) {
                    const f32x4 v = acc[f][t0 + tt];
                    *reinterpret_cast<float4*>(s_red + ((size_t)(wave * TM + f * 16 + rl) * RPP + tt * 16 + g * 4)) =
                        make_float4(v[0], v[1], v[2], v[3]);
                }
            __syncthreads();
            if (t0 == 0) { PBN_WSTAMP(5); }
            for (int e = tid; e < TM * (RP / 4); e += TPB) {
                const int r = e / (RP / 4), q = e - r * (RP / 4);
                const int p = row0 + r;
                if (p >= n) continue;
                const int orow = a.row_perm ? a.row_perm[p] : p;
                const int cl = t0 * 16 + q * 4;
                f32x4 rv = f32x4{0.f, 0.f, 0.f, 0.f};
                if (res) rv = load4<T>(res + (size_t)orow * a.ld_res + tile0 * 16 + cl);
                f32x4 v = f32x4{0.f, 0.f, 0.f, 0.f};
#pragma unroll
                for (int w = 0; w < KW; ++w) {
                    const float4 s = *reinterpret_cast<const float4*>(s_red + ((size_t)(w * TM + r) * RPP + q * 4));
                    v[0] += s.x; v[1] += s.y; v[2] += s.z; v[3] += s.w;
                }
                if (a.scale) {
                    const float4 sc = *reinterpret_cast<const float4*>(s_ss + cl);
                    v[0] *= sc.x; v[1] *= sc.y; v[2] *= sc.z; v[3] *= sc.w;
                }
                if (a.shift) {
                    const float4 sh = *reinterpret_cast<const float4*>(s_ss + NT * 16 + cl);
                    v[0] += sh.x; v[1] += sh.y; v[2] += sh.z; v[3] += sh.w;
                }
                v += rv;
                if (a.relu) {
                    v[0] = fmaxf(v[0], 0.f); v[1] = fmaxf(v[1], 0.f); v[2] = fmaxf(v[2], 0.f); v[3] = fmaxf(v[3], 0.f);
                }
                store4<T>(out + (size_t)orow * a.ld_out + tile0 * 16 + cl, v);
            }
            if (t0 + NTB < NT) __syncthreads();
        }
    }
    PBN_WSTAMP(6);
}

template <typename T, int NF, int NT, int KW, bool KSPLIT, bool KLIST = false>
int launch_cfg(ConvArgs a, hipStream_t stream) {
    constexpr int RW = NF * 16;
    constexpr int TM = KSPLIT ? RW : KW * RW;
    constexpr int NTB = ksplit_round_tiles(KW, TM, NT);
    if (a.ntiles_total % NT) return PBN_ERR_UNSUPPORTED;
    const int KS = a.K | 1;
    size_t lds = sizeof(int) * (size_t)((TM * KS + 3) & ~3);
    if (KSPLIT) lds += 16 + sizeof(float) * ((size_t)2 * NT * 16 + (size_t)KW * TM * ksplit_red_pitch(NTB));
    if (!KSPLIT || KLIST) lds += (KSPLIT ? 0 : 16) + sizeof(unsigned) * (size_t)((KW * (a.n_steps + 2 * MAX_DEPTH + (KLIST ? 64 : 0)) + 3) & ~3);
    if (lds > 160 * 1024 || a.K > 128 || a.n_steps > 0xfffe) return PBN_ERR_UNSUPPORTED;
    auto kern = k_spconv_wave<T, NF, NT, KW, KSPLIT, KLIST>;
    if (lds > 64 * 1024)
        PBN_HIP_CHECK(hipFuncSetAttribute((const void*)kern, hipFuncAttributeMaxDynamicSharedMemorySize, (int)lds));
    const int row_tiles = cdiv(a.n_out, TM), groups = a.ntiles_total / NT;
    static const int wmajor_env = getenv("PBN_WAVE_WMAJOR") ? atoi(getenv("PBN_WAVE_WMAJOR")) : 2;
    const bool shape_ok = groups >= 8 ? (groups % 8 == 0) : (groups == 1 || groups == 2 || groups == 4);
    a.wmajor = (wmajor_env == 1 || (wmajor_env == 2 && a.w_bytes > a.in_bytes)) && shape_ok && groups > 1 ? 1 : 0;
    int blocks = row_tiles * groups;
    if (a.wmajor && groups < 8) blocks = 8 * cdiv(row_tiles, 8 / groups);
    hipLaunchKernelGGL(kern, dim3(blocks), dim3(KW * 64), lds, stream, a);
    PBN_LAUNCH_CHECK();
    return PBN_OK;
}

template <typename T>
int launch_by_cfg(const ConvArgs& a, int cfg, hipStream_t stream) {
    switch (cfg) {
        case 401: return launch_cfg<T, 4, 1, 4, false>(a, stream);
        case 402: return launch_cfg<T, 4, 2, 4, false>(a, stream);
        case 404: return launch_cfg<T, 4, 4, 4, false>(a, stream);
        case 406: return launch_cfg<T, 4, 6, 4, false>(a, stream);
        case 408: return launch_cfg<T, 4, 8, 4, false>(a, stream);
        case 204: return launch_cfg<T, 2, 4, 4, false>(a, stream);
        case 206: return launch_cfg<T, 2, 6, 4, false>(a, stream);
        case 208: return launch_cfg<T, 2, 8, 4, false>(a, stream);
        case 1401: return launch_cfg<T, 4, 1, 8, true>(a, stream);
        case 1402: return launch_cfg<T, 4, 2, 8, true>(a, stream);
        case 1404: return launch_cfg<T, 4, 4, 8, true>(a, stream);
        case 1201: return launch_cfg<T, 2, 1, 8, true>(a, stream);
        case 1202: return launch_cfg<T, 2, 2, 8, true>(a, stream);
        case 1204: return launch_cfg<T, 2, 4, 8, true>(a, stream);
        case 1208: return launch_cfg<T, 2, 8, 8, true>(a, stream);
        case 1408: return launch_cfg<T, 4, 8, 8, true>(a, stream);
        case 2202: return launch_cfg<T, 2, 2, 8, true, true>(a, stream);
        case 2201: return launch_cfg<T, 2, 1, 8, true, true>(a, stream);
        default: return PBN_ERR_UNSUPPORTED;
    }
}

int pick_cfg(const ConvArgs& a) {
    const int ntt = a.ntiles_total;
    const long long rows = a.n_sel;
    if (a.vpo <= 2 && a.K >= 64 && ntt % 2 == 0) return 1202;
    static const int klist = getenv("PBN_WAVE_KLIST") ? atoi(getenv("PBN_WAVE_KLIST")) : 0;
    if (a.vpo <= 8 && a.K >= 64 && ntt % 2 == 0) return (klist && a.vpo >= 8) ? 2202 : 1202;
    int best = 0;
    long long best_wgs = -1;
    for (int cfg : {1404, 1204, 1402, 1202, 1401, 1201}) {
        const int nf = (cfg / 100) % 10, nt = cfg % 100;
        if (ntt % nt) continue;
        const long long wgs = ((rows + nf * 16 - 1) / (nf * 16)) * (ntt / nt);
        if (wgs >= 180) return cfg;
        if (wgs > best_wgs) { best_wgs = wgs; best = cfg; }
    }
    return best ? best : 1201;
}

template <typename T>
int launch_t(const ConvArgs& a, int force_cfg, hipStream_t stream) {
    int cfg = force_cfg > 0 ? force_cfg : pick_cfg(a);
    int rc = launch_by_cfg<T>(a, cfg, stream);
    if (rc == PBN_ERR_UNSUPPORTED && force_cfg <= 0) {
        for (int alt : {1202, 1201, 204}) {
            rc = launch_by_cfg<T>(a, alt, stream);
            if (rc != PBN_ERR_UNSUPPORTED) break;
        }
    }
    return rc;
}

}

#ifdef PBN_CONV_TIMING
}
extern "C" int pbn_wave_timing_read(unsigned long long* host) {
    PBN_HIP_CHECK(hipDeviceSynchronize());
    PBN_HIP_CHECK(hipMemcpyFromSymbol(host, HIP_SYMBOL(pbn::g_wave_timing), sizeof(unsigned long long) * (pbn::WT_BLOCKS * 64 + 8)));
    return PBN_OK;
}
namespace pbn {
#endif

int launch_wave(const ConvArgs& a, int dtype, int force_cfg, hipStream_t stream) {
    switch (dtype) {
        case PBN_F32: return launch_t<float>(a, force_cfg, stream);
        case PBN_BF16: return launch_t<__hip_bfloat16>(a, force_cfg, stream);
        case PBN_F16: return launch_t<__half>(a, force_cfg, stream);
        default: return PBN_ERR_ARG;
    }
}

void describe_launch(const ConvArgs& a, int dtype, LaunchDesc* d) {
    d->wave_family = 0; d->nt = 0; d->groups = 0; d->wmajor = 0;
    if (!wave_family_wanted(a, dtype)) return;
    static const int force_cfg = getenv("PBN_WAVE_CFG") ? atoi(getenv("PBN_WAVE_CFG")) : 0;
    const int cfg = force_cfg > 0 ? force_cfg : pick_cfg(a);
    const int nt = cfg % 100;
    if (nt <= 0 || a.ntiles_total % nt) return;
    d->wave_family = 1;
    d->nt = nt;
    d->groups = a.ntiles_total / nt;
    const bool shape_ok = d->groups >= 8 ? (d->groups % 8 == 0) : (d->groups == 1 || d->groups == 2 || d->groups == 4);
    static const int wmajor_env = getenv("PBN_WAVE_WMAJOR") ? atoi(getenv("PBN_WAVE_WMAJOR")) : 2;
    d->wmajor = (cfg >= 1000 && (wmajor_env == 1 || (wmajor_env == 2 && a.w_bytes > a.in_bytes)) && shape_ok && d->groups > 1) ? 1 : 0;
}

bool wave_family_wanted(const ConvArgs& a, int dtype) {
    (void)dtype;
    static const int fam = getenv("PBN_CONV_FAMILY") ? atoi(getenv("PBN_CONV_FAMILY")) : 2;
    static const int max_rows = getenv("PBN_WAVE_MAX_ROWS") ? atoi(getenv("PBN_WAVE_MAX_ROWS")) : 30000;
    static const double max_macs = getenv("PBN_WAVE_MAX_GMACS") ? atof(getenv("PBN_WAVE_MAX_GMACS")) * 1e9 : 1.0e10;
    if (a.K > 128) return false;
    if (fam == 0) return false;
    if (fam == 1) return true;
    if (a.vpo <= 8 && a.K >= 64 && !a.row_perm) return true;
    const double elems_per_step = 4.0 * (dtype == PBN_F32 ? 4.0 : 8.0);
    const double dense = (double)a.n_sel * a.n_steps * elems_per_step * a.ntiles_total * 16.0;
    return a.n_sel < max_rows && dense <= max_macs;
}

}
```

### pbnet_amd/network/mink_unet.py

```python
import ctypes
import operator
import os

import torch
import torch.nn as nn

from .. import _native as N
from .. import stage_ops
from .. import MinkowskiEngine as ME
from ..MinkowskiEngine.conv import spconv_forward, pack_weight, _pad_vec, _vpo, _workspace
from ..MinkowskiEngine.modules.resnet_block import BasicBlock
from ..MinkowskiEngine.fused_train import conv_bn_act
from ..prof import section

SPECS = {
    "MinkUNet14A": ((1,) * 8, (32, 64, 128, 256, 128, 128, 96, 96)),
    "MinkUNet14B": ((1,) * 8, (32, 64, 128, 256, 128, 128, 128, 128)),
    "MinkUNet14C": ((1,) * 8, (32, 64, 128, 256, 192, 192, 128, 128)),
    "MinkUNet14D": ((1,) * 8, (32, 64, 128, 256, 384, 384, 384, 384)),
    "MinkUNet18A": ((2,) * 8, (32, 64, 128, 256, 128, 128, 96, 96)),
    "MinkUNet18B": ((2,) * 8, (32, 64, 128, 256, 128, 128, 128, 128)),
    "MinkUNet18D": ((2,) * 8, (32, 64, 128, 256, 384, 384, 384, 384)),
    "MinkUNet34A": ((2, 3, 4, 6, 2, 2, 2, 2), (32, 64, 128, 256, 256, 128, 64, 64)),
    "MinkUNet34B": ((2, 3, 4, 6, 2, 2, 2, 2), (32, 64, 128, 256, 256, 128, 64, 32)),
# ... 122 lines not shown

    def forward(self, x):
        if self.FUSE_EVAL and not self.training and not torch.is_grad_enabled():
            return self._forward_fused(x)
        return self._forward_modules(x)

    def _forward_modules(self, x):
        from .train_engine import forward_body
        body = forward_body(self, x)
        if body is not None:
            return self.final_sematic(body)
        out = conv_bn_act(self.conv0p1s1, self.bn0, x)
        skips = [out]
        for i in range(4):
            out = conv_bn_act(getattr(self, _DOWN[i]), getattr(self, _DOWN_BN[i]), out)
            out = getattr(self, "block%d" % (i + 1))(out)
            if i < 3:
                skips.append(out)
        for i in range(4):
            out = conv_bn_act(getattr(self, _UP[i]), getattr(self, _UP_BN[i]), out)
            out = ME.cat(out, skips[3 - i])
            out = getattr(self, "block%d" % (i + 5))(out)
        return self.final_sematic(out)

    def _fold(self, bn, cout_p):
        b = bn.bn
        key = (id(bn), b.weight._version, b.bias._version, b.running_mean._version, b.running_var._version, cout_p)
        hit = self._fold_cache.get(id(bn))
        if hit is None or hit[0] != key:
            scale = b.weight.detach().float() / torch.sqrt(b.running_var.float() + b.eps)
            shift = b.bias.detach().float() - b.running_mean.float() * scale
            hit = (key, _pad_vec(scale, cout_p, 1.0), _pad_vec(shift, cout_p, 0.0))
            self._fold_cache[id(bn)] = hit
        return hit[1], hit[2]

    def _cbr(self, conv, bn, feats, nbr, n_out, relu=True, residual=None, out=None):
        packed = conv._cache.get(conv.kernel, feats.dtype)
        scale, shift = self._fold(bn, packed[3])
        return spconv_forward(feats, nbr, n_out, packed, scale=scale, shift=shift, residual=residual, relu=relu, out=out)

    def _build_plan(self, dtype):
        keep, ops, bufs, true_io, folded_io = [], [], [(0, 0)], [], []

        def new_buf(level, width):
            bufs.append((level, width))
            return len(bufs) - 1

        def slab(level, up, skip):
            b = new_buf(level, up + skip)
            return (b, 0), (b, up), (b, 0)

        def emit(map_kind, lin, lout, src, res, out, packed, scale, shift, relu, src2=(-1, 0), vpo2=0):
            w, vpo, n_steps, cout_p = packed
            keep.extend([w, scale, shift])
            if out is None:
                out = (new_buf(lout, cout_p), 0)
            op = N.UnetOp()
            op.map_kind, op.level_in, op.level_out = map_kind, lin, lout
            op.in_buf, op.in_col = src
            op.res_buf, op.res_col = res if res is not None else (-1, 0)
            op.out_buf, op.out_col = out
            op.vpo, op.n_steps, op.cout_p, op.relu = vpo, n_steps, cout_p, int(relu)
            op.in2_buf, op.in2_col = src2
            op.vpo2 = vpo2
            op.w = w.data_ptr()
            op.scale = scale.data_ptr() if scale is not None else None
            op.shift = shift.data_ptr() if shift is not None else None
            ops.append(op)
            return out

        def add(conv, bn, map_kind, lin, lout, src, res, out, relu):
            packed = conv._cache.get(conv.kernel, dtype)
            if bn is not None:
                scale, shift = self._fold(bn, packed[3])
            else:
                scale = None
                shift = _pad_vec(conv.bias.detach(), packed[3], 0.0) if conv.bias is not None else None
            true_io.append((int(conv.kernel.shape[-2]), int(conv.kernel.shape[-1])))
            return emit(map_kind, lin, lout, src, res, out, packed, scale, shift, relu)

        def add_folded(blk, h, cur, l, out):
            conv2, convd = blk.conv2, blk.downsample[0]
            if not (self.FOLD_SHORTCUT and _vpo(int(conv2.kernel.shape[-2]), dtype) % 4 == 0
                    and _vpo(int(convd.kernel.shape[-2]), dtype) % 4 == 0 and self._fold_is_safe(blk, dtype)):
                return None
            cout = int(conv2.kernel.shape[-1])
            cout_p = (cout + 15) // 16 * 16
            s2, b2 = self._fold(blk.norm2, cout_p)
            sd, bd = self._fold(blk.downsample[1], cout_p)
            k2 = conv2.kernel.detach().float() * s2[:cout]
            kd = convd.kernel.detach().float()
            kd = (kd if kd.dim() == 3 else kd.unsqueeze(0)) * sd[:cout]
            w2, vpo, n_main, cp2 = pack_weight(k2, dtype)
            wd, vpo2, n2, cpd = pack_weight(kd, dtype)
            assert cp2 == cpd == cout_p and vpo % 4 == 0 and vpo2 % 4 == 0
            cg = _group_steps(vpo // 4)
            pad = (-n2) % cg
            parts = [w2, wd] + ([torch.zeros(pad, *wd.shape[1:], dtype=wd.dtype, device=wd.device)] if pad else [])
            w = torch.cat(parts, 0).contiguous()
            true_io.append((int(conv2.kernel.shape[-2]), cout))
            folded_io.append((len(ops), int(kd.shape[-2]), cout))
            return emit(1, l, l, h, None, out, (w, vpo, n_main + n2 + pad, cout_p), None, (b2 + bd).contiguous(), True, cur, vpo2)

        cur = walk_body(self, (0, 0), slab, add, add_folded)
        final = add(self.final_sematic, None, 0, 0, 0, cur, None, None, False)
        cin_p = self.conv0p1s1._cache.get(self.conv0p1s1.kernel, dtype)[1] * (16 // torch.empty(0, dtype=dtype).element_size())
        bufs[0] = (0, cin_p)
        ops_arr = (N.UnetOp * len(ops))(*ops)
        bufs_arr = (N.UnetBuf * len(bufs))(*[N.UnetBuf(lv, w) for lv, w in bufs])
        return dict(ops=ops_arr, n_ops=len(ops), bufs=bufs_arr, n_bufs=len(bufs), out_buf=final[0], cin_p=cin_p,
                    out_width=bufs[final[0]][1], keep=keep, true_io=true_io, folded_io=folded_io)

    def _forget_state_tensors(self):
        self.__dict__.pop("_state_tensors", None)
        self.__dict__.pop("_train_plans", None)
        self.__dict__.pop("_train_engine_ok", None)
        self.__dict__.pop("_train_engine_norms", None)
        self._plans.clear()

    def _apply(self, fn, *args, **kwargs):
        self._forget_state_tensors()
        return super()._apply(fn, *args, **kwargs)

    def _plan(self, dtype):
        tensors = self.__dict__.get("_state_tensors")
        if tensors is None:
            tensors = list(self.parameters()) + list(self.buffers())
            self.__dict__["_state_tensors"] = tensors
        ver = sum(map(_VERSION_OF, tensors))
        hit = self._plans.get(dtype)
        if hit is None or hit[0] != ver:
            hit = (ver, self._build_plan(dtype))
            self._plans[dtype] = hit
        return hit[1]

    def _output_rows(self, plan, arena, offs, n, dtype):
        out = arena_rows(arena, offs[plan["out_buf"]], n, plan["out_width"], dtype)
        cout = self.final_sematic.kernel.shape[-1]
        return out if out.shape[1] == cout else out[:, :cout]

    def _forward_fused(self, x):
        cm = x.coordinate_manager
        assert x.tensor_stride == 1
        sv = cm.sorted() if self.MORTON else None
        pyr = sv.pyramid if sv is not None else cm.plain()
        dt, dev = x.F.dtype, x.F.device
        plan = self._plan(dt)
        feats = input_slab(x.F, plan["cin_p"], None if sv is None else sv.perm)
        rows = list(pyr.n)
        arena, nbytes, offs, n_rows = alloc_arena(plan["bufs"], plan["n_bufs"], rows, dt, dev)
        lib = N.lib()
        vp = ctypes.c_void_p
        ws = _workspace(dev)
        args = (plan["ops"], plan["n_ops"], plan["bufs"], plan["n_bufs"], n_rows, vp(feats.data_ptr()), feats.stride(0)) \
            + pyr.native_tables() + (vp(arena.data_ptr()), nbytes, N.DT[dt], vp(ws.data_ptr()), ws.numel(), N.current_stream())
        if MinkUNet.OP_TIMING_SINK is None:
            rc = lib.pbn_unet_forward(*args)
        else:
            op_ms = (ctypes.c_float * plan["n_ops"])()
            rc = lib.pbn_unet_forward_timed(*(args + (op_ms,)))
            MinkUNet.OP_TIMING_SINK(self, plan, rows, pyr, feats.element_size(), list(op_ms))
        N.check(rc, "pbn_unet_forward")
        out = self._output_rows(plan, arena, offs, rows[0], dt)
        if sv is not None:
            return ME.SparseTensor._from_stored_rows(out, sv.inv_perm, cm)
        return ME.SparseTensor(out, coordinate_manager=cm, tensor_stride=1)

    def _forward_fused_py(self, x):
        cm = x.coordinate_manager
        assert x.tensor_stride == 1
        dt, dev = x.F.dtype, x.F.device
        n = [cm.num_rows(1 << l) for l in range(5)]

        def slab(level, up, skip):
            t = torch.empty(n[level], up + skip, dtype=dt, device=dev)
            return t[:, :up], t[:, up:], t

        def conv(conv, bn, map_kind, lin, lout, src, res, out, relu):
            return self._cbr(conv, bn, src, MAP_KINDS[map_kind][2](cm, lin, lout), n[lout], relu=relu, residual=res, out=out)

        cur = walk_body(self, x.F, slab, conv)
        fs = self.final_sematic
        packed = fs._cache.get(fs.kernel, dt)
        out = spconv_forward(cur, None, n[0], packed, shift=_pad_vec(fs.bias, packed[3], 0.0))
        cout = fs.kernel.shape[-1]
        return ME.SparseTensor(out if out.shape[1] == cout else out[:, :cout], coordinate_manager=cm, tensor_stride=1)


def input_slab(feats, cin_p, perm=None, perm2=None, n=None, n_dev=None):
    es, width = feats.element_size(), int(feats.shape[1])
    assert width <= cin_p, "input rows of %d channels for a network of at most %d" % (width, cin_p)
    if perm is None and n_dev is None and width == cin_p and feats.stride(1) == 1 and (feats.stride(0) * es) % 16 == 0 \
            and feats.data_ptr() % 16 == 0:
        return feats
    if feats.stride(1) == 1 and (width * es) % 4 == 0 and (feats.stride(0) * es) % 4 == 0 and feats.data_ptr() % 4 == 0:
        return stage_ops.gather_pad_rows(feats, cin_p, perm, perm2, n, n_dev)
    assert perm2 is None and n_dev is None, "rows the padding launch cannot address have no capacity form"
    padded = torch.zeros(feats.shape[0], cin_p, dtype=feats.dtype, device=feats.device)
    padded[:, :width] = feats if perm is None else feats[perm]
    return padded


def alloc_arena(bufs, n_bufs, rows, dtype, device):
    n_rows = (ctypes.c_int32 * 5)(*[int(v) for v in rows])
    offs = (ctypes.c_int64 * n_bufs)()
    nbytes = N.lib().pbn_unet_arena_bytes(bufs, n_bufs, n_rows, N.DT[dtype], offs)
    return torch.empty(max(nbytes, 16), dtype=torch.uint8, device=device), nbytes, offs, n_rows


def arena_rows(arena, offset, n, width, dtype):
    return arena[offset:offset + n * width * torch.empty(0, dtype=dtype).element_size()].view(dtype).view(n, width)


def _variant(name):
    def init(self, in_channels, out_channels, D=3):
        MinkUNet.__init__(self, in_channels, out_channels, D, arch=name)
    return type(name, (MinkUNet,), {"__init__": init})


for _n in SPECS:
    globals()[_n] = _variant(_n)


def Mink_unet(in_channels=3, out_channels=20, D=3, arch="MinkUNet18A"):
    if arch not in SPECS:
        raise Exception("architecture not supported yet: {}".format(arch))
    return globals()[arch](in_channels, out_channels, D)
```

Measured before the change: 383.2.

## Derive stem 5x5x5 neighbour map on the fly from k3 parent tables

```diff
diff --git a/include/pbnet_hip.h b/include/pbnet_hip.h
--- a/include/pbnet_hip.h
+++ b/include/pbnet_hip.h
@@ -79,6 +79,12 @@
                             int relu, void* out_feat, int ld_out, int dtype, int rows_per_wave, void* workspace,
                             size_t workspace_bytes, const void* in2_feat, int ld_in2, int n_in2, int vecs_second,
                             pbn_stream_t stream);
+
+int pbn_spconv_forward_k5_derived(const void* in_feat, int ld_in, int n_in, const int32_t* k3_parent, const int32_t* child_table,
+                                  const int32_t* up_table, int n_parent, int x_fastest, const int32_t* n_out_dev, int n_out,
+                                  const void* w_packed, int vecs_per_offset, int n_steps, int cout_padded, const float* scale,
+                                  const float* shift, const void* residual, int ld_res, int relu, void* out_feat, int ld_out,
+                                  int dtype, int rows_per_wave, pbn_stream_t stream);
 
 int pbn_spconv_family(int n_out, int n_offsets, int vecs_per_offset, int n_steps, int cout_padded, int dtype, int has_map);
 
@@ -367,6 +373,9 @@
 int pbn_coords_prepare_hash(const int32_t* coords, const int32_t* n_dev, int n_cap, int want_k5, int x_fastest, void* arena,
                             size_t arena_bytes, const pbn_prepare_layout* layout, pbn_stream_t stream);
 
+int pbn_coords_k5_map(const int32_t* k3_parent, const int32_t* child_table, const int32_t* up_table, int n, int n_parent,
+                      int x_fastest, int32_t* k5, pbn_stream_t stream);
+
 int pbn_morton_keys(const int32_t* coords, const int32_t* n_dev, int n_max, int64_t* keys, pbn_stream_t stream);
 
 typedef struct {
diff --git a/pbnet_amd/MinkowskiEngine/core.py b/pbnet_amd/MinkowskiEngine/core.py
--- a/pbnet_amd/MinkowskiEngine/core.py
+++ b/pbnet_amd/MinkowskiEngine/core.py
@@ -1,4 +1,5 @@
 import ctypes
+import os
 
 import torch
 
@@ -13,6 +14,7 @@
 
 
 _OFFSETS = {}
+STEM_DERIVED = int(os.environ.get("PBN_STEM_DERIVED", "1") or 0) != 0
 _RANGE_ERROR = ("coordinates cannot be indexed: batch must be in [0,65534], x/y/z in [-32768,32767], and the bounding box of one "
                 "call must fit 44 Z-order key bits (3 x bits of the largest extent + bits of the batch range); also raised when a "
                 "coordinate table was found full or corrupted")
@@ -88,7 +90,17 @@
         if kernel_size == 3:
             return self._map_view(("k3", l), lambda: self.view(self.layout.k3[l], self.n[l] * 27, torch.int32, (self.n[l], 27)))
         assert kernel_size == 5 and stride == 1
+        if self.layout.k5 < 0:
+            return self._map_view(("k5",), self._k5_from_tables)
         return self._map_view(("k5",), lambda: self.view(self.layout.k5, self.n[0] * 125, torch.int32, (self.n[0], 125)))
+
+    def _k5_from_tables(self):
+        L = self.layout
+        nbr = torch.empty(max(self.n[0], 1), 125, dtype=torch.int32, device=self.device)
+        rc = N.lib().pbn_coords_k5_map(N.c_vp(self.ptr(L.k3[1])), N.c_vp(self.ptr(L.nbr_down[0])), N.c_vp(self.ptr(L.up[0])),
+                                       self.n[0], self.n[1], int(CV.X_FASTEST), N.ptr(nbr), N.current_stream())
+        N.check(rc, "pbn_coords_k5_map")
+        return nbr[:self.n[0]]
 
     def down_map(self, stride_in):
         self.finalize()
@@ -101,14 +113,16 @@
         l = self.level_index(stride_in) - 1
         return self._map_view(("up", l), lambda: self.view(self.layout.up[l], self.n[l] * 8, torch.int32, (self.n[l], 8)))
 
-    def native_tables(self):
-        self.finalize()
-        return table_arrays(self.ptr(0), self.layout)
-
-
-def table_arrays(base, L):
+    def native_tables(self, derived_ok=False):
+        self.finalize()
+        if self.layout.k5 >= 0:
+            return table_arrays(self.ptr(0), self.layout)
+        return table_arrays(self.ptr(0), self.layout, None if derived_ok else self.kernel_map(1, 5).data_ptr())
+
+
+def table_arrays(base, L, k5=-1):
     vp = ctypes.c_void_p
-    return ((vp * 5)(*[base + L.k3[l] for l in range(5)]), vp(base + L.k5),
+    return ((vp * 5)(*[base + L.k3[l] for l in range(5)]), vp(base + L.k5 if k5 == -1 else k5),
             (vp * 4)(*[base + L.nbr_down[l] for l in range(4)]), (vp * 4)(*[base + L.up[l] for l in range(4)]))
 
 
@@ -140,10 +154,11 @@
             prepare = ("plain" if torch.is_grad_enabled() else "sorted") if build_maps else "unique"
         self._native = None
         if prepare == "sorted" and n > 0:
+            self._want_k5 = want_k5 = 0 if (STEM_DERIVED and CV.X_FASTEST and not torch.is_grad_enabled()) else 1
             P = N.PrepareLayout()
-            nbytes = lib.pbn_coords_prepare_bytes(n, 1, ctypes.byref(P))
+            nbytes = lib.pbn_coords_prepare_bytes(n, want_k5, ctypes.byref(P))
             arena = torch.empty(nbytes, dtype=torch.uint8, device=dev)
-            rc = lib.pbn_coords_prepare(N.ptr(coords), n, 1, int(CV.X_FASTEST), N.ptr(arena), nbytes, ctypes.byref(P),
+            rc = lib.pbn_coords_prepare(N.ptr(coords), n, want_k5, int(CV.X_FASTEST), N.ptr(arena), nbytes, ctypes.byref(P),
                                         N.current_stream())
             N.check(rc, "pbn_coords_prepare")
             self._native = (arena, P)
@@ -200,7 +215,7 @@
             counts = pyr.counts_dev.tolist()
             if min(counts) < 0 and self.__dict__.get("_prepare_input") is not None:
                 coords = self._prepare_input
-                rc = N.lib().pbn_coords_prepare_hash(N.ptr(coords), None, self.n_input, 1, int(CV.X_FASTEST), N.ptr(arena),
+                rc = N.lib().pbn_coords_prepare_hash(N.ptr(coords), None, self.n_input, self._want_k5, int(CV.X_FASTEST), N.ptr(arena),
                                                      arena.numel(), ctypes.byref(P), N.current_stream())
                 N.check(rc, "pbn_coords_prepare_hash")
                 counts = pyr.counts_dev.tolist()
diff --git a/pbnet_amd/_native.py b/pbnet_amd/_native.py
--- a/pbnet_amd/_native.py
+++ b/pbnet_amd/_native.py
@@ -129,6 +129,9 @@
                                    c_f32p, c_f32p, c_vp, c_int, c_int, c_vp, c_int, c_int, c_int, c_vp, c_size, c_vp]),
     "pbn_spconv_forward_dual": (c_int, [c_vp, c_int, c_int, c_i32p, c_int, c_i32p, c_int, c_vp, c_int, c_int, c_int, c_f32p, c_f32p,
                                         c_vp, c_int, c_int, c_vp, c_int, c_int, c_int, c_vp, c_size, c_vp, c_int, c_int, c_int, c_vp]),
+    "pbn_spconv_forward_k5_derived": (c_int, [c_vp, c_int, c_int, c_i32p, c_i32p, c_i32p, c_int, c_int, c_i32p, c_int, c_vp, c_int,
+                                              c_int, c_int, c_f32p, c_f32p, c_vp, c_int, c_int, c_vp, c_int, c_int, c_int, c_vp]),
+    "pbn_coords_k5_map": (c_int, [c_i32p, c_i32p, c_i32p, c_int, c_int, c_int, c_i32p, c_vp]),
     "pbn_spconv_family": (c_int, [c_int, c_int, c_int, c_int, c_int, c_int, c_int]),
     "pbn_spconv_wgrad_workspace_bytes": (c_size, [c_int, c_int, c_int]),
     "pbn_spconv_wgrad": (c_int, [c_vp, c_int, c_vp, c_int, c_int, c_vp, c_vp, c_i32p, c_i32p, c_int, c_int, c_int, c_int, c_int,
diff --git a/pbnet_amd/csrc/executor.hip b/pbnet_amd/csrc/executor.hip
--- a/pbnet_amd/csrc/executor.hip
+++ b/pbnet_amd/csrc/executor.hip
@@ -181,6 +181,19 @@
     return coords_prepare_impl(coords, n_dev, n_cap, want_k5, x_fastest, arena, arena_bytes, P, stream, true);
 }
 
+extern "C" int pbn_coords_k5_map(const int32_t* k3_parent, const int32_t* child_table, const int32_t* up_table, int n, int n_parent,
+                                 int x_fastest, int32_t* k5, pbn_stream_t stream) {
+    if (n < 0 || n_parent < 0) return PBN_ERR_ARG;
+    if (n == 0) return PBN_OK;
+    if (!k3_parent || !child_table || !up_table || !k5 || ((uintptr_t)up_table & 15)) return PBN_ERR_ARG;
+    return coords_k5_from_tables(k3_parent, child_table, up_table, n, n_parent, x_fastest, k5, (hipStream_t)stream);
+}
+
+static bool stem_derived(const pbn_unet_op& o, const MapTables& T) {
+    static const int env = getenv("PBN_STEM_DERIVED") ? atoi(getenv("PBN_STEM_DERIVED")) : 1;
+    return env && o.map_kind == 2 && !T.k5 && T.k3 && T.k3[1] && T.down && T.down[0] && T.up && T.up[0];
+}
+
 extern "C" size_t pbn_unet_arena_bytes(const pbn_unet_buf* bufs, int n_bufs, const int32_t* n_rows, int dtype,
                                        int64_t* buf_offsets) {
     if (!bufs || !n_rows || n_bufs < 1) return 0;
@@ -198,7 +211,7 @@
                                 int dtype, int mode) {
     if (!op_index_ok(q.in_buf, q.res_buf, q.out_buf, q.level_in, q.level_out, n_bufs) || !q.w) return {};
     const OpTables m = op_tables(q.map_kind, q.level_in, q.level_out, T);
-    const ConvArgs nx = shape_args(n_rows[q.level_out], m.K, q.vpo, q.n_steps, q.cout_p, m.fwd != nullptr,
+    const ConvArgs nx = shape_args(n_rows[q.level_out], m.K, q.vpo, q.n_steps, q.cout_p, m.fwd != nullptr || stem_derived(q, T),
                                    (unsigned)((unsigned long long)q.n_steps * (q.cout_p / 16) * 1024ull),
                                    (unsigned)((unsigned long long)n_rows[q.level_in] * B.ld(q.in_buf) * esize(dtype)));
     LaunchDesc d;
@@ -221,7 +234,8 @@
         const pbn_unet_op& o = ops[i];
         if (!op_index_ok(o.in_buf, o.res_buf, o.out_buf, o.level_in, o.level_out, n_bufs)) return PBN_ERR_ARG;
         const OpTables m = op_tables(o.map_kind, o.level_in, o.level_out, T);
-        if (!m.ok) return PBN_ERR_ARG;
+        const bool derived = stem_derived(o, T);
+        if (!m.ok && !derived) return PBN_ERR_ARG;
         const bool dual = o.in2_buf >= 0;
         ConvHints hints;
         if (rows_expected && n_rows_dev) hints.rows_expected = rows_expected[o.level_out];
@@ -238,7 +252,9 @@
                                       .out_feat = B.at(o.out_buf, o.out_col), .ld_out = B.ld(o.out_buf), .dtype = dtype,
                                       .workspace = splitk_ws, .workspace_bytes = splitk_bytes,
                                       .in2_feat = dual ? B.at(o.in2_buf, o.in2_col) : nullptr, .ld_in2 = dual ? B.ld(o.in2_buf) : 0,
-                                      .n_in2 = dual ? n_rows[o.level_out] : 0, .vecs_second = dual ? o.vpo2 : 0},
+                                      .n_in2 = dual ? n_rows[o.level_out] : 0, .vecs_second = dual ? o.vpo2 : 0,
+                                      .k3_parent = derived ? T.k3[1] : nullptr, .child_table = derived ? T.down[0] : nullptr,
+                                      .up_table = derived ? T.up[0] : nullptr, .n_parent = derived ? n_rows[1] : 0},
                                      hints, (hipStream_t)stream);
         if (rc != PBN_OK) return rc;
         if (events) PBN_HIP_CHECK(hipEventRecord(events[2 * i + 1], (hipStream_t)stream));
diff --git a/pbnet_amd/csrc/pbn_common.h b/pbnet_amd/csrc/pbn_common.h
--- a/pbnet_amd/csrc/pbn_common.h
+++ b/pbnet_amd/csrc/pbn_common.h
@@ -57,6 +57,30 @@
     return (uint32_t)k;
 }
 
+__device__ __forceinline__ void cube_offset(int k, int ksize, int x_fastest, int& dx, int& dy, int& dz) {
+    const int c0 = (ksize & 1) ? ksize / 2 : 0;
+    const int a = k % ksize - c0, b = (k / ksize) % ksize - c0, c = k / (ksize * ksize) - c0;
+    dx = x_fastest ? a : c; dy = b; dz = x_fastest ? c : a;
+}
+
+__device__ __forceinline__ void child_neighbour_slot(int ck, int k, int ksize, int x_fastest, int& kp3, int& cb) {
+    int dx, dy, dz;
+    cube_offset(k, ksize, x_fastest, dx, dy, dz);
+    const int tx = (ck & 1) + dx, ty = ((ck >> 1) & 1) + dy, tz = ((ck >> 2) & 1) + dz;
+    const int px = tx >> 1, py = ty >> 1, pz = tz >> 1;
+    kp3 = x_fastest ? (px + 1) + 3 * (py + 1) + 9 * (pz + 1) : (pz + 1) + 3 * (py + 1) + 9 * (px + 1);
+    cb = (tx & 1) + 2 * (ty & 1) + 4 * (tz & 1);
+}
+
+__device__ __forceinline__ void parent_of_up_row(const int* up, int row, int& parent, int& ck) {
+    const int4 lo = reinterpret_cast<const int4*>(up)[2 * (size_t)row], hi = reinterpret_cast<const int4*>(up)[2 * (size_t)row + 1];
+    const int u[8] = {lo.x, lo.y, lo.z, lo.w, hi.x, hi.y, hi.z, hi.w};
+    parent = -1; ck = 0;
+#pragma unroll
+    for (int s = 0; s < 8; ++s)
+        if (u[s] >= 0) { parent = u[s]; ck = s; }
+}
+
 constexpr int SCAN_THREADS = 256;
 constexpr int SCAN_ITEMS = 8;
 constexpr int SCAN_TILE = SCAN_THREADS * SCAN_ITEMS;
@@ -103,6 +127,8 @@
 size_t pyramid_scratch_bytes(int n);
 int coords_prepare_sorted(const int32_t* coords, const int32_t* n_dev, int n, int want_k5, int x_fastest, void* arena,
                           const pbn_prepare_layout* P, hipStream_t stream);
+int coords_k5_from_tables(const int32_t* k3_parent, const int32_t* child_table, const int32_t* up, int n, int n_parent,
+                          int x_fastest, int32_t* k5, hipStream_t stream);
 constexpr int RADIX_U32_DIGIT_BITS = 11, RADIX_U32_PASSES = 3;
 size_t radix_sort_u32_scratch_bytes(int n);
 int radix_sort_u32(unsigned long long* keys_a, unsigned long long* keys_b, int32_t* vals_a, int32_t* vals_b, int n,
diff --git a/pbnet_amd/csrc/pyramid.hip b/pbnet_amd/csrc/pyramid.hip
--- a/pbnet_amd/csrc/pyramid.hip
+++ b/pbnet_amd/csrc/pyramid.hip
@@ -522,12 +522,6 @@
     }
 }
 
-__device__ __forceinline__ void cube_offset(int k, int ksize, int x_fastest, int& dx, int& dy, int& dz) {
-    const int c0 = (ksize & 1) ? ksize / 2 : 0;
-    const int a = k % ksize - c0, b = (k / ksize) % ksize - c0, c = k / (ksize * ksize) - c0;
-    dx = x_fastest ? a : c; dy = b; dz = x_fastest ? c : a;
-}
-
 struct TopJobs { const int* coords[3]; const u64* lkeys[3]; int* nbr[3]; const int* counts; int n_max, x_fastest; };
 __global__ __launch_bounds__(TPB) void k_maps_top(const TopJobs jb, const int* __restrict__ plan) {
     const KeyPlan kp = key_plan(plan);
@@ -588,13 +582,9 @@
             if (row >= 0) { if (first < 0) first = row; cks |= (unsigned)ck << (3 * nchild); ++nchild; }
         }
         auto entry = [&](int j, int k, int ksize) -> int {
-            const int ck = (int)(cks >> (3 * j)) & 7;
-            int dx, dy, dz;
-            cube_offset(k, ksize, jb.x_fastest, dx, dy, dz);
-            const int tx = (ck & 1) + dx, ty = ((ck >> 1) & 1) + dy, tz = ((ck >> 2) & 1) + dz;
-            const int px = tx >> 1, py = ty >> 1, pz = tz >> 1;
-            const int kp3 = jb.x_fastest ? (px + 1) + 3 * (py + 1) + 9 * (pz + 1) : (pz + 1) + 3 * (py + 1) + 9 * (px + 1);
-            return tab[kp3 * 8 + ((tx & 1) + 2 * (ty & 1) + 4 * (tz & 1))];
+            int kp3, cb;
+            child_neighbour_slot((int)(cks >> (3 * j)) & 7, k, ksize, jb.x_fastest, kp3, cb);
+            return tab[kp3 * 8 + cb];
         };
         for (int e = lane; e < nchild * 27; e += 64) {
             const int j = e / 27;
@@ -606,6 +596,23 @@
                 jb.k5[(size_t)first * 125 + e] = entry(j, e - j * 125, 5);
             }
         __builtin_amdgcn_wave_barrier();
+    }
+}
+
+__global__ __launch_bounds__(TPB) void k_k5_from_tables(const int* __restrict__ k3_parent, const int* __restrict__ child_table,
+                                                        const int* __restrict__ up, int n, int n_parent, int x_fastest,
+                                                        int* __restrict__ k5) {
+    const long long total = (long long)n * 125;
+    for (long long e = (long long)blockIdx.x * TPB + threadIdx.x; e < total; e += (long long)gridDim.x * TPB) {
+        const int row = (int)(e / 125), k = (int)(e - (long long)row * 125);
+        int par, ck, kp3, cb, v = -1;
+        parent_of_up_row(up, row, par, ck);
+        if (par >= 0 && par < n_parent) {
+            child_neighbour_slot(ck, k, 5, x_fastest, kp3, cb);
+            const int q = k3_parent[(size_t)par * 27 + kp3];
+            if (q >= 0 && q < n_parent) v = child_table[(size_t)q * 8 + cb];
+        }
+        k5[e] = v;
     }
 }
 
@@ -718,6 +725,17 @@
     return PBN_OK;
 }
 
+int coords_k5_from_tables(const int32_t* k3_parent, const int32_t* child_table, const int32_t* up, int n, int n_parent,
+                          int x_fastest, int32_t* k5, hipStream_t st) {
+    if (n <= 0) return PBN_OK;
+    long long blocks = cdiv((long long)n * 125, TPB * 4);
+    if (blocks > 16384) blocks = 16384;
+    hipLaunchKernelGGL(k_k5_from_tables, dim3((unsigned)blocks), dim3(TPB), 0, st, k3_parent, child_table, up, n, n_parent,
+                       x_fastest, k5);
+    PBN_LAUNCH_CHECK();
+    return PBN_OK;
+}
+
 static_assert(RADIX_U32_DIGIT_BITS == RADIX_BITS, "radix_sort_u32 runs sort_pass_body<8>: 11-bit digits");
 
 size_t radix_sort_u32_scratch_bytes(int n) {
diff --git a/pbnet_amd/csrc/spconv.hip b/pbnet_amd/csrc/spconv.hip
--- a/pbnet_amd/csrc/spconv.hip
+++ b/pbnet_amd/csrc/spconv.hip
@@ -508,7 +508,11 @@
         if ((c.vecs_per_offset & 3) || c.vecs_second < 4 || (c.vecs_second & 3) || !c.nbr || c.row_perm || c.n_in2 < c.n_out) return PBN_ERR_ARG;
         if (c.n_steps < n_main + (c.vecs_second >> 2) || c.n_steps > n_main + (c.vecs_second >> 2) + 3) return PBN_ERR_ARG;
     } else if (c.n_steps != n_main) return PBN_ERR_ARG;
-    if (!c.nbr && c.n_offsets != 1) return PBN_ERR_ARG;
+    const bool derived = !c.nbr && c.k3_parent;
+    if (derived && (c.n_offsets != 125 || !c.child_table || !c.up_table || c.n_parent < 0 || c.row_perm || c.in2_feat ||
+                    ((uintptr_t)c.up_table & 15) || c.rows_per_wave >= 10000 || (c.rows_per_wave > 0 && c.rows_per_wave < 100)))
+        return PBN_ERR_ARG;
+    if (!c.nbr && !derived && c.n_offsets != 1) return PBN_ERR_ARG;
     if (c.n_out == 0) return PBN_OK;
     if (!c.in_feat || !c.w_packed || !c.out_feat) return PBN_ERR_ARG;
     const int dtype = c.dtype, esz = dtype == PBN_F32 ? 4 : 2;
@@ -520,7 +524,7 @@
     const unsigned long long in_extent = (unsigned long long)c.n_in * (unsigned long long)c.ld_in * (unsigned long long)esz;
     const unsigned long long w_extent = (unsigned long long)c.n_steps * (unsigned long long)(c.cout_padded / 16) * 1024ull;
     if (in_extent >= 0x80000000ull || w_extent >= 0x80000000ull) return PBN_ERR_RANGE;
-    if (!c.nbr && c.n_in < c.n_out) return PBN_ERR_ARG;
+    if (!c.nbr && !derived && c.n_in < c.n_out) return PBN_ERR_ARG;
     ConvArgs a;
     a.in_bytes = (unsigned)in_extent; a.w_bytes = (unsigned)w_extent;
     a.in = c.in_feat; a.nbr = c.nbr; a.row_perm = c.row_perm; a.n_out_dev = c.n_out_dev; a.w = c.w_packed; a.scale = c.scale;
@@ -533,6 +537,18 @@
     a.pf_w = hints.next.w; a.pf_steps = hints.next.steps; a.pf_ntt = hints.next.ntt; a.pf_nt = hints.next.nt; a.pf_groups = hints.next.groups;
     static const int dbg_env = getenv("PBN_CONV_DBG") ? atoi(getenv("PBN_CONV_DBG")) : 0;
     a.dbg = dbg_env;
+    a.dk_k3 = derived ? c.k3_parent : nullptr; a.dk_child = derived ? c.child_table : nullptr; a.dk_up = derived ? c.up_table : nullptr;
+    a.dk_n_parent = c.n_parent; a.dk_x_fastest = c.x_fastest;
+    if (derived) {
+        if (c.rows_per_wave >= 100) return launch_wave(a, dtype, c.rows_per_wave, stream);
+        static const int no_neighbour = -1;
+        ConvArgs with_map = a;
+        with_map.nbr = &no_neighbour;
+        int family = 0;
+        for (const Family& f : FAMILIES)
+            if (f.wanted(with_map, dtype)) { family = f.id; break; }
+        return family == 1 ? launch_wave_auto(a, dtype, 0, stream) : PBN_ERR_UNSUPPORTED;
+    }
     int rows_per_wave = c.rows_per_wave;
     if (rows_per_wave >= 10000) {
         const int cfg = rows_per_wave - 10000;
@@ -597,6 +613,22 @@
                          ConvHints{}, (hipStream_t)stream);
 }
 
+extern "C" int pbn_spconv_forward_k5_derived(const void* in_feat, int ld_in, int n_in, const int32_t* k3_parent,
+                                             const int32_t* child_table, const int32_t* up_table, int n_parent, int x_fastest,
+                                             const int32_t* n_out_dev, int n_out, const void* w_packed, int vecs_per_offset,
+                                             int n_steps, int cout_padded, const float* scale, const float* shift,
+                                             const void* residual, int ld_res, int relu, void* out_feat, int ld_out, int dtype,
+                                             int rows_per_wave, pbn_stream_t stream) {
+    if (!k3_parent) return PBN_ERR_ARG;
+    return spconv_launch({.in_feat = in_feat, .ld_in = ld_in, .n_in = n_in, .nbr = nullptr, .n_offsets = 125, .n_out_dev = n_out_dev,
+                          .n_out = n_out, .w_packed = w_packed, .vecs_per_offset = vecs_per_offset, .n_steps = n_steps,
+                          .cout_padded = cout_padded, .scale = scale, .shift = shift, .residual = residual, .ld_res = ld_res,
+                          .relu = relu, .out_feat = out_feat, .ld_out = ld_out, .dtype = dtype, .rows_per_wave = rows_per_wave,
+                          .k3_parent = k3_parent, .child_table = child_table, .up_table = up_table, .n_parent = n_parent,
+                          .x_fastest = x_fastest != 0},
+                         ConvHints{}, (hipStream_t)stream);
+}
+
 #ifdef PBN_CONV_TIMING
 extern "C" int pbn_conv_timing_read(unsigned* host) {
     PBN_HIP_CHECK(hipDeviceSynchronize());
diff --git a/pbnet_amd/csrc/spconv_common.h b/pbnet_amd/csrc/spconv_common.h
--- a/pbnet_amd/csrc/spconv_common.h
+++ b/pbnet_amd/csrc/spconv_common.h
@@ -37,6 +37,8 @@
     unsigned in2_bytes;
     const void* pf_w;
     int pf_steps, pf_ntt, pf_nt, pf_groups;
+    const int* dk_k3; const int* dk_child; const int* dk_up;
+    int dk_n_parent, dk_x_fastest;
 };
 
 struct LaunchDesc { int wave_family, nt, groups, wmajor; };
@@ -50,6 +52,8 @@
     void* out_feat; int ld_out; int dtype; int rows_per_wave = 0;
     void* workspace = nullptr; size_t workspace_bytes = 0;
     const void* in2_feat = nullptr; int ld_in2 = 0; int n_in2 = 0; int vecs_second = 0;
+    const int32_t* k3_parent = nullptr; const int32_t* child_table = nullptr; const int32_t* up_table = nullptr;
+    int n_parent = 0; int x_fastest = 1;
 };
 struct ConvHints { int rows_expected = 0; NextWeights next = {}; };
 int spconv_launch(const ConvCall& c, const ConvHints& hints, hipStream_t stream);
diff --git a/pbnet_amd/csrc/spconv_wave.hip b/pbnet_amd/csrc/spconv_wave.hip
--- a/pbnet_amd/csrc/spconv_wave.hip
+++ b/pbnet_amd/csrc/spconv_wave.hip
@@ -25,6 +25,8 @@
 #ifndef PBN_WAVE_XCOAL
 #define PBN_WAVE_XCOAL 1
 #endif
+constexpr bool derived_fill_built(bool ksplit, int nt) { return ksplit && nt <= 4; }
+
 constexpr int pipe_depth(int nf, int nt) {
     (void)nf; (void)nt;
     return PBN_WAVE_DEPTH;
@@ -180,7 +182,34 @@
     if (row0 >= n) { prefetch_drain(pf_sink); return; }
     if (tid == 0) *s_none = -1;
 
-    if (a.nbr && !a.row_perm && row0 + TM <= n && KS == K && ((TM * K) & 3) == 0) {
+    if (derived_fill_built(KSPLIT, NT) && !a.nbr && a.dk_k3) {
+        static_assert(TPB % TM == 0, "whole threads per tile row");
+        constexpr int TPR = TPB / TM;
+        const int r = tid / TPR, j = tid - r * TPR;
+        int par = -1, ck = 0;
+        if (row0 + r < n) parent_of_up_row(a.dk_up, row0 + r, par, ck);
+        if (par >= a.dk_n_parent) par = -1;
+        for (int k0 = j; k0 < 125; k0 += 8 * TPR) {
+            int q[8], cb[8];
+#pragma unroll
+            for (int i = 0; i < 8; ++i) {
+                const int k = k0 + i * TPR;
+                int kp3 = 0;
+                cb[i] = 0;
+                q[i] = -1;
+                if (k < 125 && par >= 0) {
+                    child_neighbour_slot(ck, k, 5, a.dk_x_fastest, kp3, cb[i]);
+                    q[i] = a.dk_k3[(size_t)par * 27 + kp3];
+                }
+            }
+#pragma unroll
+            for (int i = 0; i < 8; ++i) {
+                const int k = k0 + i * TPR;
+                const int v = (q[i] >= 0 && q[i] < a.dk_n_parent) ? a.dk_child[(size_t)q[i] * 8 + cb[i]] : -1;
+                if (k < 125) s_nbr[r * KS + k] = v;
+            }
+        }
+    } else if (a.nbr && !a.row_perm && row0 + TM <= n && KS == K && ((TM * K) & 3) == 0) {
         const int4* src = reinterpret_cast<const int4*>(a.nbr + (size_t)row0 * K);
         int4* dst = reinterpret_cast<int4*>(s_nbr);
         for (int e = tid; e < (TM * K) >> 2; e += TPB) dst[e] = src[e];
@@ -431,6 +460,7 @@
     constexpr int TM = KSPLIT ? RW : KW * RW;
     constexpr int NTB = ksplit_round_tiles(KW, TM, NT);
     if (a.ntiles_total % NT) return PBN_ERR_UNSUPPORTED;
+    if (!a.nbr && a.dk_k3 && !derived_fill_built(KSPLIT, NT)) return PBN_ERR_UNSUPPORTED;
     const int KS = a.K | 1;
     size_t lds = sizeof(int) * (size_t)((TM * KS + 3) & ~3);
     if (KSPLIT) lds += 16 + sizeof(float) * ((size_t)2 * NT * 16 + (size_t)KW * TM * ksplit_red_pitch(NTB));
diff --git a/pbnet_amd/network/mink_unet.py b/pbnet_amd/network/mink_unet.py
--- a/pbnet_amd/network/mink_unet.py
+++ b/pbnet_amd/network/mink_unet.py
@@ -298,8 +298,10 @@
         lib = N.lib()
         vp = ctypes.c_void_p
         ws = _workspace(dev)
+        stem = plan["ops"][0]
+        derived_ok = stem.map_kind == 2 and lib.pbn_spconv_family(rows[0], 125, stem.vpo, stem.n_steps, stem.cout_p, N.DT[dt], 1) == 1
         args = (plan["ops"], plan["n_ops"], plan["bufs"], plan["n_bufs"], n_rows, vp(feats.data_ptr()), feats.stride(0)) \
-            + pyr.native_tables() + (vp(arena.data_ptr()), nbytes, N.DT[dt], vp(ws.data_ptr()), ws.numel(), N.current_stream())
+            + pyr.native_tables(derived_ok=derived_ok) + (vp(arena.data_ptr()), nbytes, N.DT[dt], vp(ws.data_ptr()), ws.numel(), N.current_stream())
         if MinkUNet.OP_TIMING_SINK is None:
             rc = lib.pbn_unet_forward(*args)
         else:
```

Result: slower. 374.1 (-2.4%).
